# GDMCF/GDMCF

Hardware: AMD Instinct MI355X
Metric: training users/sec (higher is better)
Workload: dtype f32; 1 GPU; yelp-shape synthetic rows, batch=400/GPU, dims=[1000], T=5, noise_scale=0.01, linear-var, mean_type=x0, reweight, AdamW lr=1e-5 (BASELINE configs[1]); n_items=34395, global_batch=400, parallelism=dp1, batch_rows=device CSR rows (CsrBatch)

## Files before the change

### gdmcf_amd/_lib.py

```python
import ctypes
import os
import re
from ctypes import c_char_p, c_double, c_float, c_int, c_int64, c_size_t, c_uint64, c_void_p

_HERE = os.path.dirname(os.path.abspath(__file__))
LIB_PATH = os.path.join(_HERE, "csrc", "libgdmcf_hip.so")
HEADER_PATH = os.path.normpath(os.path.join(_HERE, "..", "include", "gdmcf_hip.h"))

P = c_void_p
_CTYPES = {"int": c_int, "int64_t": c_int64, "uint64_t": c_uint64, "size_t": c_size_t, "float": c_float, "double": c_double}


def _uncomment(text):
    return re.sub(r"/\*.*?\*/", " ", text, flags=re.S)


def _code(text):
    return re.sub(r'^[ \t]*(#.*|extern\s+"C"\s*\{|\})[ \t]*$', "", _uncomment(text), flags=re.M)


def _ctype(ctype, where):
    words = re.sub(r"\bconst\b", " ", ctype).replace("*", " * ").split()
    if "*" in words:
        return c_char_p if words == ["char", "*"] else c_void_p
    if " ".join(words) not in _CTYPES:
        raise ImportError(f"gdmcf_hip.h: no ctypes type for '{' '.join(ctype.split())}' in the declaration of {where}")
    return _CTYPES[" ".join(words)]


def _declarator(decl, where):
    m = re.fullmatch(r"\s*(.*[\s*])(\w+)\s*", decl, flags=re.S)
    if not m:
        raise ImportError(f"gdmcf_hip.h: cannot read '{decl.strip()}' in the declaration of {where}")
    return m.groups()


def parse_functions(text):
    code = _code(text)
    out = {}
    for ret, name, params in re.findall(r"([\w\s*]+?)\b(gdmcf_\w+)\s*\(([^()]*)\)\s*;", code):
        params = [] if params.strip() in ("", "void") else params.split(",")
        out[name] = (_ctype(ret, name), [_ctype(_declarator(p, name)[0], name) for p in params])
    mentioned = re.findall(r"(gdmcf_\w+)\s*\(", code)
    if len(mentioned) != len(out):
        raise ImportError(f"gdmcf_hip.h: {len(mentioned)} gdmcf_*( but {len(out)} declarations read; unreadable: "
                          f"{sorted(set(mentioned) - set(out)) or 'none, a name is repeated'}")
    return out


def parse_constants(text):
    text = _uncomment(text)
    out = {n: int(v) for n, v in re.findall(r"^\s*#\s*define\s+(GDMCF_\w+)\s+\(?\s*(-?\d+)\s*\)?\s*$", text, flags=re.M)}
    for body in re.findall(r"\benum\s*\{([^}]*)\}", text):
        for member in filter(str.strip, body.split(",")):
            m = re.fullmatch(r"\s*(\w+)\s*=\s*(-?\d+)\s*", member)
            if not m:
                raise ImportError(f"gdmcf_hip.h: enum member '{member.strip()}' is not `NAME = integer`")
            out[m.group(1)] = int(m.group(2))
    return out


def parse_structs(text):
    out = {}
    for name, body in re.findall(r"\btypedef\s+struct\s+(\w+)\s*\{([^}]*)\}\s*\1\s*;", _code(text)):
        out[name] = []
        for line in filter(str.strip, body.split(";")):
            first, *more = line.split(",")
            ctype, member = _declarator(first, "struct " + name)
            if more and "*" in line:
                raise ImportError(f"gdmcf_hip.h: struct {name}: '{line.strip()}' must declare one pointer member per line")
            out[name] += [(m.strip(), _ctype(ctype, "struct " + name)) for m in [member] + more]
    return out


try:
    with open(HEADER_PATH) as _f:
        _HEADER = _f.read()
except OSError as e:
    raise ImportError(f"{HEADER_PATH} is missing: gdmcf_amd._lib derives its ctypes binding from the C header, which sits "
                      "beside the package in the source tree.") from e
_SIGNATURES = parse_functions(_HEADER)
EXPORTED_SYMBOLS = tuple(_SIGNATURES)
CONSTANTS = parse_constants(_HEADER)
GDMCF_OK, E_SHAPE, E_ARG, E_UNSUPPORTED, E_HIP, E_WORKSPACE, N_TABLES = (
    CONSTANTS["GDMCF_" + n] for n in ("OK", "E_SHAPE", "E_ARG", "E_UNSUPPORTED", "E_HIP", "E_WORKSPACE", "N_TABLES"))
TABLE_NAMES = (
    "betas", "alphas_cumprod", "alphas_cumprod_prev", "alphas_cumprod_next", "sqrt_alphas_cumprod",
    "sqrt_one_minus_alphas_cumprod", "log_one_minus_alphas_cumprod", "sqrt_recip_alphas_cumprod",
    "sqrt_recipm1_alphas_cumprod", "posterior_variance", "posterior_log_variance_clipped",
    "posterior_mean_coef1", "posterior_mean_coef2",
)


class GdDwAdamw(ctypes.Structure):
    _fields_ = parse_structs(_HEADER)["GdDwAdamw"]


class GdKnTail(ctypes.Structure):
    _fields_ = parse_structs(_HEADER)["GdKnTail"]


_lib = None


def load():
    global _lib
    if _lib is not None:
        return _lib
    if not os.path.exists(LIB_PATH):
        raise ImportError(
            f"{LIB_PATH} is missing: build it with `python -m gdmcf_amd.build` (hipcc, gfx950). "
            "gdmcf_amd has no CPU / PyTorch fallback.")
    lib = ctypes.CDLL(LIB_PATH)
    for name, (res, args) in _SIGNATURES.items():
        fn = getattr(lib, name)
        fn.restype = res
        fn.argtypes = args
    if lib.gdmcf_version() != 1:
        raise ImportError("libgdmcf_hip.so ABI version mismatch; rebuild with `python -m gdmcf_amd.build --force`")
    _lib = lib
    return lib


_EXC = {E_SHAPE: AssertionError, E_ARG: ValueError, E_UNSUPPORTED: NotImplementedError, E_HIP: RuntimeError,
        E_WORKSPACE: RuntimeError}


def check(rc):
    if rc != GDMCF_OK:
        msg = load().gdmcf_last_error().decode(errors="replace")
        raise _EXC.get(rc, RuntimeError)(msg or f"gdmcf error {rc}")


def ptr(t):
    return None if t is None else t.data_ptr()


def require_gpu(t, what):
    if not t.is_cuda:
        raise RuntimeError(f"gdmcf_amd: {what} must live on the MI355X (got device '{t.device}'); "
                           "the HIP path has no CPU fallback")


def shadow_info(data_ptr):
    p16 = ctypes.c_void_p()
    rows, cols, ld = ctypes.c_int64(), ctypes.c_int64(), ctypes.c_int64()
    if not load().gdmcf_bf16_shadow_info(data_ptr, ctypes.byref(p16), ctypes.byref(rows), ctypes.byref(cols), ctypes.byref(ld)):
        return None
    return int(p16.value), int(rows.value), int(cols.value), int(ld.value)


def stream_ptr():
    import torch
    return torch.cuda.current_stream().cuda_stream


def philox_randn(shape, device, seed, offset, stream_id=4, out=None):
    import torch
    rows, cols = int(shape[0]), int(shape[1])
    if out is None:
        out = torch.empty(rows, cols, dtype=torch.float32, device=device)
    require_gpu(out, "philox_randn output")
    check(load().gdmcf_randn_f32(out.data_ptr(), out.stride(0), rows, cols, int(stream_id), int(seed) & (2 ** 64 - 1),
                                 int(offset) & (2 ** 64 - 1), stream_ptr()))
    return out


def schedule_tables(kind, noise_scale, noise_min, noise_max, steps, beta_fixed=True):
    import numpy as np
    out = np.zeros((N_TABLES, steps), dtype=np.float64)
    rc = load().gdmcf_schedule_build(kind, float(noise_scale), float(noise_min), float(noise_max), int(steps),
                                     int(bool(beta_fixed)), out.ctypes.data_as(c_void_p))
    check(rc)
    return out


class Bf16Shadow:

    def __init__(self, t, sync=True):
        import weakref

        import torch
        require_gpu(t, "bf16 shadow source")
        if t.dim() != 2 or t.dtype != torch.float32 or t.stride(1) != 1:
            raise RuntimeError("gdmcf_amd: a bf16 shadow needs a 2-D float32 tensor with unit column stride")
        self.rows, self.cols = t.shape
        self.ptr = t.data_ptr()
        self.ld = t.stride(0)
        self.buf = torch.zeros((self.rows + 63) // 64 * 64, (self.cols + 63) // 64 * 64, dtype=torch.bfloat16,
                               device=t.device)
        self._lib = load()
        self._fin = weakref.finalize(self, self._lib.gdmcf_bf16_shadow_clear, self.ptr)
        self.register()
        if sync:
            self.sync()

    def register(self):
        check(self._lib.gdmcf_bf16_shadow_set(self.ptr, self.buf.data_ptr(), self.rows, self.cols, self.buf.stride(0)))

    def unregister(self):
        self._lib.gdmcf_bf16_shadow_clear(self.ptr)

    def sync(self):
        check(self._lib.gdmcf_bf16_shadow_sync(self.ptr, self.ld, stream_ptr()))

    def close(self):
        self._fin()
```

### gdmcf_amd/csrc/gemm_dr_kn.hip

```cpp
#include <stdlib.h>

#include "gemm_dr.h"
#include "tail_job.h"

namespace {

#ifndef GD_KN_EVERY
#define GD_KN_EVERY 4
#endif
template <int NL>
__global__ __launch_bounds__(256, 1) void dr_kn_kernel(const DrArgs d, const GdTailJob job) {
    constexpr int TMB = 5;
    const GdGemm& g = d.g;
    const int lane = threadIdx.x & 63;
    const int wave = __builtin_amdgcn_readfirstlane(threadIdx.x >> 6);
    const int r = lane & 15, q = lane >> 4;
    const int nblk = gridDim.x, per = nblk >> 3;
    const int slot = (nblk & 7) == 0 ? ((int)(blockIdx.x & 7) * per + (int)(blockIdx.x >> 3)) : (int)blockIdx.x;
    const int wl = slot * 4 + wave;
    const int n_waves = nblk * 4;
    const int ntiles = d.tiles_m * d.tiles_n;
    const int CPS = d.ksp;
    const int total_chunks = (g.K + 15) >> 4;
    const int ntasks = ntiles * g.splits;
    if (job.on && slot == (ntasks + 3) >> 2) {
        extern __shared__ __attribute__((aligned(16))) unsigned char kn_lds[];
        gd_tail_job_run(job, kn_lds);
        return;
    }
    const __amdgpu_buffer_rsrc_t srdA = __builtin_amdgcn_make_buffer_rsrc(const_cast<float*>(g.A), 0, (int)(((int64_t)(g.M - 1) * g.lda + g.K) * 4), 0x00020000);
    const __amdgpu_buffer_rsrc_t srdB = __builtin_amdgcn_make_buffer_rsrc(const_cast<float*>(g.B), 0, (int)(((int64_t)(g.K - 1) * g.ldb + g.N) * 4), 0x00020000);
    const uint32_t ldb16 = (uint32_t)g.ldb * 64u;
    for (int task = wl; task < ntasks; task += n_waves) {
        const int split = task / ntiles, tile = task - split * ntiles;
        const int tm = tile % d.tiles_m, tn = tile / d.tiles_m;
        const int m0 = tm * (16 * TMB), n0 = tn * (64 * NL);
        const int c_lo = split * CPS;
        uint32_t offA[TMB], offB[4][NL];
#pragma unroll
        for (int a = 0; a < TMB; ++a) offA[a] = (uint32_t)(((int64_t)min(m0 + 16 * a + r, g.M - 1) * g.lda + 4 * q) * 4);
#pragma unroll
        for (int s = 0; s < 4; ++s)
#pragma unroll
            for (int l = 0; l < NL; ++l) {
                const int n = n0 + 64 * l + 4 * r;
                offB[s][l] = n < g.N ? (uint32_t)(((int64_t)(4 * q + s) * g.ldb + n) * 4) : 0x80000000u;
            }
        f32x4 acc[TMB][NL][4];
#pragma unroll
        for (int a = 0; a < TMB; ++a)
#pragma unroll
            for (int l = 0; l < NL; ++l)
#pragma unroll
                for (int e = 0; e < 4; ++e) acc[a][l][e] = f32x4{0.f, 0.f, 0.f, 0.f};
        f32x4 xa[2][TMB], xb[2][4][NL];
        {
            const uint32_t ka = (uint32_t)c_lo * 64u, kb = (uint32_t)c_lo * ldb16;
#pragma unroll
            for (int a = 0; a < TMB; ++a) xa[0][a] = __builtin_bit_cast(f32x4, __builtin_amdgcn_raw_buffer_load_b128(srdA, offA[a], ka, 0));
#pragma unroll
            for (int s = 0; s < 4; ++s)
#pragma unroll
                for (int l = 0; l < NL; ++l)
                    xb[0][s][l] = __builtin_bit_cast(f32x4, __builtin_amdgcn_raw_buffer_load_b128(srdB, offB[s][l], kb, 0));
        }
#define GD_KN_CHUNK(PAR, c)                                                                                            \
        {                                                                                                              \
            const bool more = (c) + 1 < c_lo + CPS && (c) + 1 < total_chunks;                                          \
            const uint32_t ka = more ? (uint32_t)((c) + 1) * 64u : 0x80000000u;                                        \
            const uint32_t kb = more ? (uint32_t)((c) + 1) * ldb16 : 0x80000000u;                                      \
            if ((c) * 16 + 15 >= g.K) {  \
                _Pragma("unroll") for (int e = 0; e < 4; ++e) {                                                        \
                    const bool keep = (c) * 16 + 4 * q + e < g.K;                                                      \
                    _Pragma("unroll") for (int a = 0; a < TMB; ++a) xa[PAR][a][e] = keep ? xa[PAR][a][e] : 0.f;        \
                }                                                                                                      \
            }                                                                                                          \
                    \
            _Pragma("unroll") for (int a = 0; a < TMB; ++a) asm volatile("" : "+v"(xa[PAR][a]));                       \
            _Pragma("unroll") for (int s = 0; s < 4; ++s)                                                              \
                _Pragma("unroll") for (int l = 0; l < NL; ++l) asm volatile("" : "+v"(xb[PAR][s][l]));                 \
            __builtin_amdgcn_sched_barrier(0);                                                                         \
            _Pragma("unroll") for (int s = 0; s < 4; ++s) {                                                            \
                _Pragma("unroll") for (int n = 0; n < TMB * NL * 4; ++n) {                                             \
                    const int a = n / (NL * 4), l = (n / 4) % NL, e = n % 4;                                           \
                    acc[a][l][e] = __builtin_amdgcn_mfma_f32_16x16x4f32(xa[PAR][a][s], xb[PAR][s][l][e], acc[a][l][e], 0, 0, 0); \
                    const int idx = s * (TMB * NL * 4) + n;                                                            \
                    if (idx % GD_KN_EVERY == 2 && idx / GD_KN_EVERY < TMB + 4 * NL) {                                  \
                        const int ld = idx / GD_KN_EVERY;                                                              \
                        __builtin_amdgcn_sched_barrier(0);                                                             \
                        if (ld < TMB)                                                                                  \
                            xa[(PAR) ^ 1][ld] = __builtin_bit_cast(f32x4, __builtin_amdgcn_raw_buffer_load_b128(srdA, offA[ld], ka, 0)); \
                        else                                                                                           \
                            xb[(PAR) ^ 1][(ld - TMB) / NL][(ld - TMB) % NL] = __builtin_bit_cast(                      \
                                f32x4, __builtin_amdgcn_raw_buffer_load_b128(srdB, offB[(ld - TMB) / NL][(ld - TMB) % NL], kb, 0)); \
                        __builtin_amdgcn_sched_barrier(0);                                                             \
                    }                                                                                                  \
                }                                                                                                      \
                __builtin_amdgcn_sched_barrier(0);                                                                     \
            }                                                                                                          \
        }
        for (int c = c_lo; c < c_lo + CPS && c < total_chunks; c += 2) {
            GD_KN_CHUNK(0, c);
            GD_KN_CHUNK(1, c + 1);
        }
#undef GD_KN_CHUNK
        float* __restrict__ slab = g.C + (int64_t)split * g.slab_stride;
#pragma unroll
        for (int a = 0; a < TMB; ++a)
#pragma unroll
            for (int t = 0; t < 4; ++t) {
                const int m = m0 + 16 * a + 4 * q + t;
                if (m >= g.M) continue;
#pragma unroll
                for (int l = 0; l < NL; ++l) {
                    const int n = n0 + 64 * l + 4 * r;
                    const f32x4 v = {acc[a][l][0][t], acc[a][l][1][t], acc[a][l][2][t], acc[a][l][3][t]};
                    if (n + 3 < g.ldc) {
                        *reinterpret_cast<f32x4*>(slab + (int64_t)m * g.ldc + n) = v;
                    } else {
                        for (int e = 0; e < 4; ++e)
                            if (n + e < g.N) slab[(int64_t)m * g.ldc + n + e] = v[e];
                    }
                }
            }
    }
}

}

int gd_dr_kn_splits(int M, int N, int K) {
    if (!dr_routes().kn || M < 16 || N < 64 || K < 4096) return 0;
    const long tiles = (long)gd_cdiv(M, 80) * gd_cdiv(N, 128);
    if ((long)gd_cdiv(M, 80) * 80 * 100 > (long)M * 112) return 0;
    if ((long)gd_cdiv(N, 128) * 128 * 100 > (long)N * 112) return 0;
    const long slots = 4L * dr_cu_count();
    if (tiles > slots) return 0;
    int splits = (int)(slots / tiles);
    const int total_chunks = gd_cdiv(K, 16);
    if (splits > total_chunks / 8) splits = total_chunks / 8;
    if (splits < 2 || splits > 64) return splits > 64 ? 64 : 0;
    return splits;
}

static bool kn_idle_workgroup(int ntasks, int n_cu) { return gd_cdiv(ntasks, 4) < n_cu; }

#ifndef GD_KN_TAIL_DEFAULT
#define GD_KN_TAIL_DEFAULT 1
#endif

static int kn_launch(GdGemm& g, const GdTailJob* job, hipStream_t s) {
    if (!dr_routes().kn) return GD_DR_NOT_TAKEN;
    const int splits = gd_dr_kn_splits(g.M, g.N, g.K);
    const size_t need = (size_t)splits * g.M * g.ldc * sizeof(float);
    const bool ok = splits > 0 && g.ldc >= g.N && (g.ldc & 3) == 0 && g.ws_cap >= need && g.slab_stride >= (int64_t)g.M * g.ldc &&
                (int64_t)g.M * g.lda * 4 < ((int64_t)1 << 31) && (int64_t)g.K * g.ldb * 4 < ((int64_t)1 << 31) && g.lda >= g.K && g.ldb >= g.N &&
                (reinterpret_cast<uintptr_t>(g.B) & 15) == 0 && (g.ldb & 3) == 0 && (reinterpret_cast<uintptr_t>(g.C) & 15) == 0;
    if (!ok) return GD_DR_NOT_TAKEN;
    DrArgs d = {};
    const int n_cu = dr_cu_count();
    const int total_chunks = gd_cdiv(g.K, 16);
    const int cps = (gd_cdiv(total_chunks, splits) + 1) & ~1;
    const int real_splits = gd_cdiv(total_chunks, cps);
    d.tiles_m = gd_cdiv(g.M, 80);
    d.tiles_n = gd_cdiv(g.N, 128);
    d.ksp = cps;
    GdTailJob none = {};
    size_t lds = 0;
    if (job) {
        const char* env = getenv("GDMCF_KN_TAIL");
        const bool tail_on = env ? atoi(env) != 0 : GD_KN_TAIL_DEFAULT != 0;
        lds = lt_lds_bytes(job->T, job->H, job->B);
        if (!tail_on || !job->on || !kn_idle_workgroup(d.tiles_m * d.tiles_n * real_splits, n_cu) || lds > GD_LT_LDS_MAX)
            return GD_DR_NOT_TAKEN;
        static bool attr_set = false;
        if (!gd_allow_big_lds(dr_kn_kernel<2>, lds, &attr_set, "gemm_dr_kn")) return GDMCF_E_HIP;
    }
    g.splits = real_splits;
    g.kchunk = cps * 16;
    g.tiles_m = d.tiles_m;
    g.tiles_n = d.tiles_n;
    d.g = g;
    {
        GdProfScope prof(g.prof_tag, 2.0 * g.M * g.N * g.K, s);
        hipLaunchKernelGGL((dr_kn_kernel<2>), dim3(n_cu), dim3(256), lds, s, d, job ? *job : none);
    }
    t_gd_last_gemm = 5;
    return gd_launch_status("gemm_dr_kn");
}

int gd_dr_kn_launch(GdGemm& g, hipStream_t s) { return kn_launch(g, nullptr, s); }
int gd_dr_kn_launch_tail(GdGemm& g, const GdTailJob& job, hipStream_t s) { return kn_launch(g, &job, s); }

int gdmcf_debug_kn_tail_rides(int M, int N, int K) {
    const int splits = gd_dr_kn_splits(M, N, K);
    if (splits <= 0) return 0;
    const int total_chunks = gd_cdiv(K, 16);
    const int cps = (gd_cdiv(total_chunks, splits) + 1) & ~1;
    return kn_idle_workgroup(gd_cdiv(M, 80) * gd_cdiv(N, 128) * gd_cdiv(total_chunks, cps), dr_cu_count()) ? 1 : 0;
}
```

### gdmcf_amd/csrc/linear.hip

```cpp
#include <stdlib.h>

#include "common.h"
#include "tail_job.h"

int gd_splitk_reduce(const float* slabs, int64_t slab_stride, int splits, int64_t ld_slab, int M, int N, int mode,
                     const float* bias, const float* rowscale, const float* aact, int64_t ldact, int act, float* out,
                     int64_t ldo, hipStream_t s);
int gd_colsum(const float* dZ, int64_t ld, const float* rs, int M, int N, float* db, hipStream_t s);
int gd_rowpart_reduce(const float* rowpart, int ld, int M, int nt, float* rowsum, hipStream_t s);

namespace {

static const int TARGET_WGS = getenv("GDMCF_TARGET_WGS") ? atoi(getenv("GDMCF_TARGET_WGS")) : 760;

thread_local int t_gemm_prec = GDMCF_GEMM_F32;
thread_local int t_loss_parts = 0;

int pick_class(int M, int N, bool fused, int prec) {
    if (prec == GDMCF_GEMM_BF16 && M > 128) {
        const long pad = (long)gd_cdiv(M, 208) * 208;
        const long tiles = (pad / 208) * gd_cdiv(N, 256);
        const long rounds = (tiles + 255) / 256;
        if (pad * 10 <= (long)M * 11 && pad / 208 <= 2 && (!fused || tiles * 100 >= rounds * 256 * 85)) return 3;
    }
    if (prec == GDMCF_GEMM_F32X3 && M > 128 && N >= 128) {
        const long pad = (long)gd_cdiv(M, 208) * 208;
        if (pad * 10 <= (long)M * 11) return 4;
    }
    return gd_pick_shape_class(M, N);
}

int pick_class_dw(int M, int N, int prec, bool fused_adamw = false) {
    static const int forced = getenv("GDMCF_BF16_DW_CLASS") ? atoi(getenv("GDMCF_BF16_DW_CLASS")) : -1;
    if (prec == GDMCF_GEMM_BF16 && forced >= 0) return forced;
    if (prec == GDMCF_GEMM_BF16 && fused_adamw && M >= 160 && N >= 256) return 0;
    if (prec == GDMCF_GEMM_BF16 && M >= 416 && N >= 512) {
        const long tiles = (long)gd_cdiv(M, 208) * gd_cdiv(N, 256);
        const long rounds = (tiles + 255) / 256;
        if (tiles * 100 >= rounds * 256 * 85) return 3;
    }
    return gd_pick_shape_class(M, N);
}

void attach_result_shadow(GdGemm& g) {
    GdShadow c;
    if (g.bf16 == 1 && gd_shadow_lookup(g.C, &c) && c.rows == g.M && c.cols >= g.N) {
        g.C16 = c.p16;
        g.ldc16 = c.ld16;
    }
}

void attach_shadows(GdGemm& g, int layA, int layB) {
    if (g.bf16 != 1) return;
    GdShadow a, b;
    if (!gd_shadow_lookup(g.A, &a) || !gd_shadow_lookup(g.B, &b)) return;
    const bool okA = layA == GD_LAY_KC ? (a.rows == g.M && a.cols == g.K) : (a.rows == g.K && a.cols == g.M);
    const bool okB = layB == GD_LAY_KC ? (b.rows == g.N && b.cols == g.K) : (b.rows == g.K && b.cols == g.N);
    if (!okA || !okB) return;
    g.A16 = a.p16; g.lda16 = a.ld16;
    g.B16 = b.p16; g.ldb16 = b.ld16;
}

int pick_splits(int M, int N, int K, int cls, int prec) {
    const int bk = prec == GDMCF_GEMM_BF16 ? 64 : 32;
    const int tiles = gd_cdiv(M, gd_gemm_tile_m(cls)) * gd_cdiv(N, gd_gemm_tile_n(cls));
    int s = (cls >= 3 ? 256 : TARGET_WGS) / tiles;
    const int max_by_k = K / (8 * bk);
    if (s > max_by_k) s = max_by_k;
    if (s < 1) s = 1;
    if (s > 64) s = 64;
    return s;
}

inline int64_t round4(int64_t x) { return (x + 3) & ~(int64_t)3; }

float* bias_col_request(int a_scale_col, int64_t lda, const float* rowscale, int K, float* db) {
    static const int on = getenv("GDMCF_BIAS_COL") ? atoi(getenv("GDMCF_BIAS_COL")) : 1;
    if (!on || !a_scale_col || db == nullptr || t_gemm_prec != GDMCF_GEMM_F32 || lda <= K) return nullptr;
    return db;
}

int dw_adamw_setup(const GdDwAdamw& e, GdGemm& g, int& cls) {
    GD_CHECK_SHAPE(e.M > 0 && e.N > 0 && e.K > 0 && e.lddz >= e.N && e.lda >= e.K && e.ldw >= e.K, "linear_bwd_weight_adamw: bad shape");
    GD_CHECK_ARG(e.W && e.exp_avg && e.exp_avg_sq && e.step >= 1, "linear_bwd_weight_adamw: optimizer state missing");
    const int M = e.M, N = e.N, K = e.K;
    cls = pick_class_dw(N, K, t_gemm_prec, true);
    g = GdGemm{};
    g.bf16 = t_gemm_prec;
    g.A = e.dZ; g.lda = e.lddz; g.B = e.A; g.ldb = e.lda; g.M = N; g.N = K; g.K = M; g.splits = 1;
    g.m_fastest = gd_cdiv(N, gd_gemm_tile_m(cls)) <= gd_cdiv(K, gd_gemm_tile_n(cls));
    g.C = e.W; g.ldc = e.ldw; g.aux = e.exp_avg; g.aux2 = e.exp_avg_sq; g.prof_tag = 5;
    g.adam = gd_adam_hyper(e.lr, e.beta1, e.beta2, e.eps, e.weight_decay, e.step, e.grad_scale);
    g.adam_dev = t_gd_step_state ? &t_gd_step_state->hyper : nullptr;
    attach_result_shadow(g);
    attach_shadows(g, GD_LAY_MC, GD_LAY_MC);
    g.out2 = bias_col_request(e.a_scale_col, e.lda, e.rowscale, K, e.db);
    return GDMCF_OK;
}

int dw_adamw_finish(const GdDwAdamw& e, bool asked, const GdGemm& g, hipStream_t s) {
    if (asked && g.out2 == nullptr) return GDMCF_OK;
    if (e.db) return gd_colsum(e.dZ, e.lddz, e.rowscale, e.M, e.N, e.db, s);
    return GDMCF_OK;
}

}

extern "C" {

int gdmcf_gemm_precision(int mode) {
    const int prev = t_gemm_prec;
    if (mode == GDMCF_GEMM_F32 || mode == GDMCF_GEMM_BF16 || mode == GDMCF_GEMM_F32X3) t_gemm_prec = mode;
    return prev;
}

size_t gdmcf_linear_ws_bytes(int M, int N, int K) {
    if (M <= 0 || N <= 0 || K <= 0) return 0;
    size_t need = 0;
    for (int prec = GDMCF_GEMM_F32; prec <= GDMCF_GEMM_F32X3; ++prec) {
        const int cf = pick_class(M, N, false, prec), cb = pick_class(M, K, false, prec);
        size_t f = (size_t)pick_splits(M, N, K, cf, prec) * M * round4(N);
        if (prec == GDMCF_GEMM_F32) {
            const size_t fk = (size_t)gd_dr_kn_splits(M, N, K) * M * round4(N);
            f = f > fk ? f : fk;
            const size_t ff = (size_t)gd_dr_fat_slab_plan(M, N, K, nullptr, nullptr) * M * round4(N);
            f = f > ff ? f : ff;
        }
        size_t b = (size_t)pick_splits(M, K, N, cb, prec) * M * round4(K);
        if (prec == GDMCF_GEMM_F32) {
            const size_t bk = (size_t)gd_dr_kn_splits(M, K, N) * M * round4(K);
            b = b > bk ? b : bk;
        }
        need = need > f ? need : f;
        need = need > b ? need : b;
    }
    return need * sizeof(float) + 256;
}

int gdmcf_debug_fat_slab_plan(int M, int N, int K, int* nb, int* splits, int* cps) {
    int nb_ = 0, cps_ = 0;
    const int sp = (t_gemm_prec == GDMCF_GEMM_F32 && M > 0 && N > 0 && K > 0) ? gd_dr_fat_slab_plan(M, N, K, &nb_, &cps_) : 0;
    if (nb) *nb = nb_;
    if (splits) *splits = sp;
    if (cps) *cps = cps_;
    return sp > 0;
}

int gdmcf_loss_tiles(int N) { return gd_cdiv(N, 16); }

int gdmcf_linear_fwd_f32(const float* A, int64_t lda, const float* W, int64_t ldw, const float* bias, int act, int M,
                         int N, int K, float* C, int64_t ldc, void* ws, size_t ws_bytes, void* stream) {
    GD_CHECK_SHAPE(M > 0 && N > 0 && K > 0 && lda >= K && ldw >= K && ldc >= N, "linear_fwd: bad shape");
    GD_CHECK_ARG(act == 0 || act == 1, "linear_fwd: bad activation");
    hipStream_t s = (hipStream_t)stream;
    const int cls = pick_class(M, N, false, t_gemm_prec);
    const int splits = pick_splits(M, N, K, cls, t_gemm_prec);
    GdGemm g = {};
    g.bf16 = t_gemm_prec;
    g.A = A; g.lda = lda; g.B = W; g.ldb = ldw; g.M = M; g.N = N; g.K = K;
    g.m_fastest = gd_cdiv(M, gd_gemm_tile_m(cls)) <= gd_cdiv(N, gd_gemm_tile_n(cls));
    g.bias = bias; g.act = act; g.prof_tag = 1;
    if (splits == 1) {
        g.splits = 1; g.C = C; g.ldc = ldc;
        attach_result_shadow(g);
        attach_shadows(g, GD_LAY_KC, GD_LAY_KC);
        return gd_gemm_launch(GD_LAY_KC, GD_LAY_KC, GD_EPI_BIAS_ACT, cls, g, s);
    }
    const int64_t lds_ = round4(N);
    const size_t need = (size_t)splits * M * lds_ * sizeof(float);
    if (ws == nullptr || ws_bytes < need) {
        gdmcf_set_error("linear_fwd: workspace %zu < %zu bytes", ws_bytes, need);
        return GDMCF_E_WORKSPACE;
    }
    g.splits = splits; g.C = (float*)ws; g.ldc = lds_; g.slab_stride = (int64_t)M * lds_;
    g.ws_cap = ws_bytes;
    attach_shadows(g, GD_LAY_KC, GD_LAY_KC);
    int rc = gd_gemm_launch(GD_LAY_KC, GD_LAY_KC, GD_EPI_SLAB, cls, g, s);
    if (rc) return rc;
    const int real_splits = gd_cdiv(K, g.kchunk);
    return gd_splitk_reduce((const float*)ws, g.slab_stride, real_splits, lds_, M, N, 0, bias, nullptr, nullptr, 0,
                            act, C, ldc, s);
}

int gdmcf_linear_fwd_wt_f32(const float* A, int64_t lda, const float* Wt, int64_t ldwt, const float* bias, int act, int M, int N,
                            int K, float* C, int64_t ldc, void* ws, size_t ws_bytes, void* stream) {
    GD_CHECK_SHAPE(M > 0 && N > 0 && K > 0 && lda >= K && ldwt >= N && ldc >= N, "linear_fwd_wt: bad shape");
    GD_CHECK_ARG(act == 0 || act == 1, "linear_fwd_wt: bad activation");
    if (t_gemm_prec != GDMCF_GEMM_F32) {
        gdmcf_set_error("linear_fwd_wt: float32 GEMM mode only (the bf16 / f32x3 modes keep the weight in its own orientation)");
        return GDMCF_E_UNSUPPORTED;
    }
    hipStream_t s = (hipStream_t)stream;
    const int cls = pick_class(M, N, false, t_gemm_prec);
    const int splits = pick_splits(M, N, K, cls, t_gemm_prec);
    const int64_t lds_ = round4(N);
    const size_t need = (size_t)splits * M * lds_ * sizeof(float);
    if (ws == nullptr || ws_bytes < need) {
        gdmcf_set_error("linear_fwd_wt: workspace %zu < %zu bytes", ws_bytes, need);
        return GDMCF_E_WORKSPACE;
    }
    GdGemm g = {};
    g.A = A; g.lda = lda; g.B = Wt; g.ldb = ldwt; g.M = M; g.N = N; g.K = K;
    g.m_fastest = gd_cdiv(M, gd_gemm_tile_m(cls)) <= gd_cdiv(N, gd_gemm_tile_n(cls));
    g.splits = splits; g.C = (float*)ws; g.ldc = lds_; g.slab_stride = (int64_t)M * lds_; g.prof_tag = 1;
    g.ws_cap = ws_bytes;
    int rc = gd_gemm_launch(GD_LAY_KC, GD_LAY_MC, GD_EPI_SLAB, cls, g, s);
    if (rc) return rc;
    const int real_splits = gd_cdiv(K, g.kchunk);
    return gd_splitk_reduce((const float*)ws, g.slab_stride, real_splits, lds_, M, N, 0, bias, nullptr, nullptr, 0, act, C, ldc, s);
}

int gdmcf_linear_loss_fwd_f32(const float* A, int64_t lda, const float* W, int64_t ldw, const float* bias,
                              const float* target, int64_t ldt, const float* alpha, int M, int N, int K, float* out,
                              int64_t ldo, float* diff, int64_t ldd, float* rowpart, float* rowsum, void* stream) {
    GD_CHECK_SHAPE(M > 0 && N > 0 && K > 0 && lda >= K && ldw >= K && ldt >= N && ldd >= N, "linear_loss_fwd: bad shape");
    GD_CHECK_SHAPE(out == nullptr || ldo >= N, "linear_loss_fwd: ldo < N");
    hipStream_t s = (hipStream_t)stream;
    const int cls = pick_class(M, N, true, t_gemm_prec);
    GdGemm g = {};
    g.bf16 = t_gemm_prec;
    g.A = A; g.lda = lda; g.B = W; g.ldb = ldw; g.M = M; g.N = N; g.K = K; g.splits = 1;
    g.m_fastest = gd_cdiv(M, gd_gemm_tile_m(cls)) <= gd_cdiv(N, gd_gemm_tile_n(cls));
    g.bias = bias; g.aux = target; g.ldaux = ldt; g.r0 = alpha; g.out2 = out; g.ldout2 = ldo;
    g.prof_tag = 2;
    g.C = diff; g.ldc = ldd; g.rowpart = rowpart; g.ld_rowpart = gdmcf_loss_tiles(N);
    attach_result_shadow(g);
    attach_shadows(g, GD_LAY_KC, GD_LAY_KC);
    int rc = gd_gemm_launch(GD_LAY_KC, GD_LAY_KC, GD_EPI_LOSS, cls, g, s);
    if (rc) return rc;
    t_loss_parts = g.tiles_n;
    if (rowsum == nullptr) return GDMCF_OK;
    return gd_rowpart_reduce(rowpart, g.ld_rowpart, M, g.tiles_n, rowsum, s);
}

int gdmcf_linear_loss_fwd_bits_f32(const float* A, int64_t lda, const float* W, int64_t ldw, const float* bias,
                                   const uint32_t* target_bits, int64_t ldbits, const float* alpha, int M, int N, int K,
                                   float* out, int64_t ldo, float* diff, int64_t ldd, float* rowpart, float* rowsum,
                                   void* stream) {
    GD_CHECK_SHAPE(M > 0 && N > 0 && K > 0 && lda >= K && ldw >= K && ldd >= N, "linear_loss_fwd_bits: bad shape");
    GD_CHECK_SHAPE(out == nullptr || ldo >= N, "linear_loss_fwd_bits: ldo < N");
    GD_CHECK_ARG(target_bits && ldbits >= (N + 31) / 32, "linear_loss_fwd_bits: target bitmap missing / ldbits < ceil(N/32)");
    hipStream_t s = (hipStream_t)stream;
    const int cls = pick_class(M, N, true, t_gemm_prec);
    GdGemm g = {};
    g.bf16 = t_gemm_prec;
    g.A = A; g.lda = lda; g.B = W; g.ldb = ldw; g.M = M; g.N = N; g.K = K; g.splits = 1;
    g.m_fastest = gd_cdiv(M, gd_gemm_tile_m(cls)) <= gd_cdiv(N, gd_gemm_tile_n(cls));
    g.bias = bias; g.aux = nullptr; g.ldaux = 0; g.aux_bits = target_bits; g.ldbits = ldbits; g.r0 = alpha; g.out2 = out;
    g.ldout2 = ldo; g.prof_tag = 2;
    g.C = diff; g.ldc = ldd; g.rowpart = rowpart; g.ld_rowpart = gdmcf_loss_tiles(N);
    attach_result_shadow(g);
    attach_shadows(g, GD_LAY_KC, GD_LAY_KC);
    int rc = gd_gemm_launch(GD_LAY_KC, GD_LAY_KC, GD_EPI_LOSS, cls, g, s);
    if (rc) return rc;
    t_loss_parts = g.tiles_n;
    if (rowsum == nullptr) return GDMCF_OK;
    return gd_rowpart_reduce(rowpart, g.ld_rowpart, M, g.tiles_n, rowsum, s);
}

int gdmcf_linear_posterior_fwd_f32(const float* A, int64_t lda, const float* W, int64_t ldw, const float* bias,
                                   const float* x_t, int64_t ldxt, const float* c1, const float* c2, const float* r1,
                                   const float* r2, const float* sigma, const float* z, int64_t ldz, int M, int N,
                                   int K, float* x_next, int64_t ldxn, float* pred_out, int64_t ldp, void* stream) {
    GD_CHECK_SHAPE(M > 0 && N > 0 && K > 0 && lda >= K && ldw >= K && ldxt >= N && ldxn >= N, "linear_posterior_fwd: bad shape");
    GD_CHECK_ARG(c1 && c2, "linear_posterior_fwd: c1/c2 missing");
    GD_CHECK_ARG((r1 == nullptr) == (r2 == nullptr), "linear_posterior_fwd: r1/r2 must both be set or both NULL");
    GD_CHECK_ARG(z == nullptr || (sigma != nullptr && ldz >= N), "linear_posterior_fwd: sigma missing");
    hipStream_t s = (hipStream_t)stream;
    const int cls = pick_class(M, N, true, t_gemm_prec);
    GdGemm g = {};
    g.bf16 = t_gemm_prec;
    g.A = A; g.lda = lda; g.B = W; g.ldb = ldw; g.M = M; g.N = N; g.K = K; g.splits = 1;
    g.m_fastest = gd_cdiv(M, gd_gemm_tile_m(cls)) <= gd_cdiv(N, gd_gemm_tile_n(cls));
    g.bias = bias; g.aux = x_t; g.ldaux = ldxt; g.aux2 = z; g.ldaux2 = ldz;
    g.r0 = c1; g.r1 = c2; g.r2 = r1; g.r3 = r2; g.r4 = sigma;
    g.out2 = pred_out; g.ldout2 = ldp; g.C = x_next; g.ldc = ldxn; g.prof_tag = 3;
    attach_result_shadow(g);
    attach_shadows(g, GD_LAY_KC, GD_LAY_KC);
    return gd_gemm_launch(GD_LAY_KC, GD_LAY_KC, GD_EPI_POST, cls, g, s);
}

int gdmcf_linear_bwd_input_f32(const float* dZ, int64_t lddz, const float* W, int64_t ldw, const float* rowscale,
                               const float* Aact, int64_t ldact, int act, int M, int N, int K, float* dA,
                               int64_t ldda, void* ws, size_t ws_bytes, void* stream) {
    GD_CHECK_SHAPE(M > 0 && N > 0 && K > 0 && lddz >= N && ldw >= K && ldda >= K, "linear_bwd_input: bad shape");
    GD_CHECK_ARG(act == 0 || (act == 1 && Aact && ldact >= K), "linear_bwd_input: activation output missing");
    hipStream_t s = (hipStream_t)stream;
    const int cls = pick_class(M, K, false, t_gemm_prec);
    const int splits = pick_splits(M, K, N, cls, t_gemm_prec);
    const int64_t lds_ = round4(K);
    const size_t need = (size_t)splits * M * lds_ * sizeof(float);
    if (ws == nullptr || ws_bytes < need) {
        gdmcf_set_error("linear_bwd_input: workspace %zu < %zu bytes", ws_bytes, need);
        return GDMCF_E_WORKSPACE;
    }
    GdGemm g = {};
    g.bf16 = t_gemm_prec;
    g.A = dZ; g.lda = lddz; g.B = W; g.ldb = ldw; g.M = M; g.N = K; g.K = N;
    g.m_fastest = gd_cdiv(M, gd_gemm_tile_m(cls)) <= gd_cdiv(K, gd_gemm_tile_n(cls));
    g.splits = splits; g.C = (float*)ws; g.ldc = lds_; g.slab_stride = (int64_t)M * lds_; g.prof_tag = 4;
    g.ws_cap = ws_bytes;
    attach_shadows(g, GD_LAY_KC, GD_LAY_MC);
    int rc = gd_gemm_launch(GD_LAY_KC, GD_LAY_MC, GD_EPI_SLAB, cls, g, s);
    if (rc) return rc;
    const int real_splits = gd_cdiv(N, g.kchunk);
    return gd_splitk_reduce((const float*)ws, g.slab_stride, real_splits, lds_, M, K, 1, nullptr, rowscale, Aact,
                            ldact, act, dA, ldda, s);
}

int gdmcf_loss_parts_last(void) { return t_loss_parts; }

int gdmcf_kn_tail_run(const GdKnTail* tail, int M, void* stream) {
    GD_CHECK_ARG(tail != nullptr, "kn_tail_run: tail missing");
    const GdKnTail& t = *tail;
    GD_CHECK_SHAPE(M > 0 && t.nt > 0 && t.ld_rowpart >= t.nt, "kn_tail_run: bad shape");
    GD_CHECK_ARG(t.rowpart && t.rowsum, "kn_tail_run: null pointer");
    int rc = gd_rowpart_reduce(t.rowpart, t.ld_rowpart, M, t.nt, t.rowsum, (hipStream_t)stream);
    if (rc) return rc;
    rc = gdmcf_row_loss_finish_mean_f64(t.rowsum, t.rowdiv, t.alpha, t.ts, t.weight_t, t.pt, M, t.T, t.H, t.Lt_history, t.Lt_count,
                                        t.update_history, t.loss_unscaled, t.loss, t.gradcoef, t.loss_mean, t.rowscale_mean, stream);
    if (rc) return rc;
    return gdmcf_rowscale_f32(t.A, t.lda, t.rowscale, M, t.Ka, t.out, t.ldo, stream);
}

int gdmcf_linear_bwd_input_tail_f32(const float* dZ, int64_t lddz, const float* W, int64_t ldw, const float* rowscale,
                                    const float* Aact, int64_t ldact, int act, int M, int N, int K, float* dA, int64_t ldda,
                                    void* ws, size_t ws_bytes, const GdKnTail* tail, void* stream) {
    GD_CHECK_SHAPE(M > 0 && N > 0 && K > 0 && lddz >= N && ldw >= K && ldda >= K, "linear_bwd_input_tail: bad shape");
    GD_CHECK_ARG(act == 0 || (act == 1 && Aact && ldact >= K), "linear_bwd_input_tail: activation output missing");
    GD_CHECK_ARG(tail != nullptr, "linear_bwd_input_tail: tail missing");
    const GdKnTail& t = *tail;
    GD_CHECK_SHAPE(t.nt > 0 && t.ld_rowpart >= t.nt && t.T > 0 && t.H > 0 && t.Ka > 0 && t.lda >= t.Ka && t.ldo >= t.Ka,
                   "linear_bwd_input_tail: bad tail shape");
    GD_CHECK_ARG(t.rowpart && t.rowsum && t.rowdiv && t.ts && t.weight_t && t.pt && t.loss_unscaled && t.loss && t.A && t.rowscale && t.out,
                 "linear_bwd_input_tail: null pointer");
    GD_CHECK_ARG(!t.update_history || (t.Lt_history && t.Lt_count), "linear_bwd_input_tail: update_history without the history");
    GD_CHECK_ARG(!t.rowscale_mean || t.gradcoef, "linear_bwd_input_tail: rowscale_mean needs gradcoef");
    GD_CHECK_ARG(lt_lds_bytes(t.T, t.H, M) <= GD_LT_LDS_MAX, "linear_bwd_input_tail: T*H and B too large for the LDS-resident FIFO update (150 KiB)");
    hipStream_t s = (hipStream_t)stream;
    const int64_t lds_ = round4(K);
    if (t_gemm_prec == GDMCF_GEMM_F32 && ws != nullptr) {
        GdGemm g = {};
        g.A = dZ; g.lda = lddz; g.B = W; g.ldb = ldw; g.M = M; g.N = K; g.K = N;
        g.C = (float*)ws; g.ldc = lds_; g.slab_stride = (int64_t)M * lds_; g.prof_tag = 4;
        g.ws_cap = ws_bytes;
        GdShadow sh;
        const bool has16 = gd_shadow_lookup(t.out, &sh) && sh.rows == M && sh.cols == t.Ka;
        GdTailJob j = {};
        j.on = 1; j.B = M;
        j.rowpart = t.rowpart; j.ld_rowpart = t.ld_rowpart; j.nt = t.nt; j.rowsum = t.rowsum;
        j.rowdiv = t.rowdiv; j.alpha = t.alpha; j.gradcoef = t.gradcoef; j.ts = t.ts; j.weight_t = t.weight_t; j.pt = t.pt;
        j.T = t.T; j.H = t.H; j.update = t.update_history; j.hist = t.Lt_history; j.cnt = t.Lt_count; j.lu = t.loss_unscaled;
        j.loss = t.loss; j.loss_mean = t.loss_mean; j.rowscale_mean = t.rowscale_mean; j.inv_b = 1.0f / (float)M;
        j.K = t.Ka; j.A = t.A; j.lda = t.lda; j.rs = t.rowscale; j.out = t.out; j.ldo = t.ldo;
        j.out16 = has16 ? (unsigned short*)sh.p16 : nullptr; j.ldo16 = has16 ? sh.ld16 : 0; j.bias_col = t.ldo > t.Ka;
        const int rc = gd_dr_kn_launch_tail(g, j, s);
        if (rc != GD_DR_NOT_TAKEN) {
            if (rc) return rc;
            return gd_splitk_reduce((const float*)ws, g.slab_stride, gd_cdiv(N, g.kchunk), lds_, M, K, 1, nullptr, rowscale, Aact, ldact,
                                    act, dA, ldda, s);
        }
    }
    const int rc = gdmcf_kn_tail_run(tail, M, stream);
    if (rc) return rc;
    return gdmcf_linear_bwd_input_f32(dZ, lddz, W, ldw, rowscale, Aact, ldact, act, M, N, K, dA, ldda, ws, ws_bytes, stream);
}

int gdmcf_linear_bwd_weight_f32(const float* dZ, int64_t lddz, const float* A, int64_t lda, const float* rowscale,
                                int a_scale_col, int M, int N, int K, float* dW, int64_t lddw, float* db, int accumulate,
                                void* stream) {
    GD_CHECK_SHAPE(M > 0 && N > 0 && K > 0 && lddz >= N && lda >= K && lddw >= K, "linear_bwd_weight: bad shape");
    hipStream_t s = (hipStream_t)stream;
    const int cls = pick_class_dw(N, K, t_gemm_prec);
    GdGemm g = {};
    g.bf16 = t_gemm_prec;
    g.A = dZ; g.lda = lddz; g.B = A; g.ldb = lda; g.M = N; g.N = K; g.K = M; g.splits = 1;
    g.m_fastest = gd_cdiv(N, gd_gemm_tile_m(cls)) <= gd_cdiv(K, gd_gemm_tile_n(cls));
    g.C = dW; g.ldc = lddw; g.accumulate = accumulate; g.prof_tag = 5;
    attach_shadows(g, GD_LAY_MC, GD_LAY_MC);
    g.out2 = bias_col_request(a_scale_col, lda, rowscale, K, db);
    const bool asked = g.out2 != nullptr;
    int rc = gd_gemm_launch(GD_LAY_MC, GD_LAY_MC, GD_EPI_STORE, cls, g, s);
    if (rc) return rc;
    if (asked && g.out2 == nullptr) return GDMCF_OK;
    if (db) return gd_colsum(dZ, lddz, rowscale, M, N, db, s);
    return GDMCF_OK;
}

int gdmcf_linear_bwd_weight_adamw_f32(const float* dZ, int64_t lddz, const float* A, int64_t lda, const float* rowscale,
                                      int a_scale_col, int M, int N, int K, float* W, int64_t ldw, float* exp_avg, float* exp_avg_sq,
                                      float* db, float lr, float beta1, float beta2, float eps, float weight_decay,
                                      int step, float grad_scale, void* stream) {
    const GdDwAdamw e = {dZ, lddz, A, lda, rowscale, a_scale_col, M, N, K, W, ldw, exp_avg, exp_avg_sq, db,
                         lr, beta1, beta2, eps, weight_decay, step, grad_scale};
    GdGemm g;
    int cls;
    int rc = dw_adamw_setup(e, g, cls);
    if (rc) return rc;
    const bool asked = g.out2 != nullptr;
    rc = gd_gemm_launch(GD_LAY_MC, GD_LAY_MC, GD_EPI_ADAMW, cls, g, (hipStream_t)stream);
    if (rc) return rc;
    return dw_adamw_finish(e, asked, g, (hipStream_t)stream);
}

int gdmcf_linear_bwd_weight_adamw_multi_f32(const GdDwAdamw* list, int n, void* stream) {
    GD_CHECK_ARG(n >= 0 && (n == 0 || list), "linear_bwd_weight_adamw_multi: bad list");
    hipStream_t s = (hipStream_t)stream;
    constexpr int MAXN = 4;
    for (int i0 = 0; i0 < n; i0 += MAXN) {
        const int k = n - i0 < MAXN ? n - i0 : MAXN;
        GdGemm g[MAXN];
        bool asked[MAXN];
        int cls;
        for (int j = 0; j < k; ++j) {
            const int rc = dw_adamw_setup(list[i0 + j], g[j], cls);
            if (rc) return rc;
            asked[j] = g[j].out2 != nullptr;
        }
        int rc = gd_gemm_dr_adamw_multi(g, k, s);
        if (rc == GD_DR_NOT_TAKEN) {
            for (int j = 0; j < k; ++j) {
                const GdDwAdamw& e = list[i0 + j];
                rc = gdmcf_linear_bwd_weight_adamw_f32(e.dZ, e.lddz, e.A, e.lda, e.rowscale, e.a_scale_col, e.M, e.N, e.K, e.W,
                                                       e.ldw, e.exp_avg, e.exp_avg_sq, e.db, e.lr, e.beta1, e.beta2, e.eps,
                                                       e.weight_decay, e.step, e.grad_scale, stream);
                if (rc) return rc;
            }
            continue;
        }
        if (rc) return rc;
        for (int j = 0; j < k; ++j) {
            rc = dw_adamw_finish(list[i0 + j], asked[j], g[j], s);
            if (rc) return rc;
        }
    }
    return GDMCF_OK;
}

}
```

### gdmcf_amd/csrc/reduce.hip

```cpp
#include "tail_job.h"

namespace {

__global__ __launch_bounds__(256) void splitk_reduce_kernel(const float* __restrict__ slabs, int64_t slab_stride,
                                                            int splits, int64_t ld_slab, int M, int N, int mode,
                                                            const float* __restrict__ bias,
                                                            const float* __restrict__ rowscale,
                                                            const float* __restrict__ aact, int64_t ldact, int act,
                                                            float* __restrict__ out, int64_t ldo,
                                                            unsigned short* __restrict__ out16, int64_t ldo16, int vec) {
    const int m = blockIdx.y;
    const int n0 = (blockIdx.x * 256 + threadIdx.x) * 4;
    if (n0 >= N) return;
    float sv[4] = {0.f, 0.f, 0.f, 0.f};
    const float* p = slabs + (int64_t)m * ld_slab + n0;
    if (vec && n0 + 3 < N) {
        for (int k0 = 0; k0 < splits; k0 += 8) {
            f32x4 t[8];
#pragma unroll
            for (int u = 0; u < 8; ++u)
                t[u] = (k0 + u < splits) ? *reinterpret_cast<const f32x4*>(p + (int64_t)(k0 + u) * slab_stride)
                                         : f32x4{0.f, 0.f, 0.f, 0.f};
#pragma unroll
            for (int u = 0; u < 8; ++u)
                if (k0 + u < splits) { sv[0] += t[u].x; sv[1] += t[u].y; sv[2] += t[u].z; sv[3] += t[u].w; }
        }
    } else {
        for (int k = 0; k < splits; ++k)
            for (int j = 0; j < 4; ++j)
                if (n0 + j < N) sv[j] += p[(int64_t)k * slab_stride + j];
    }
    const float rs = (mode != 0 && rowscale) ? rowscale[m] : 1.f;
#pragma unroll
    for (int j = 0; j < 4; ++j) {
        const int n = n0 + j;
        if (n >= N) break;
        float s = sv[j];
        if (mode == 0) {
            if (bias) s += bias[n];
            if (act == 1) s = tanhf(s);
        } else {
            if (rowscale) s *= rs;
            if (act == 1) {
                const float h = aact[(int64_t)m * ldact + n];
                s *= (1.f - h * h);
            }
        }
        out[(int64_t)m * ldo + n] = s;
        if (out16) out16[(int64_t)m * ldo16 + n] = gd_bf16_bits(s);
    }
}

__global__ __launch_bounds__(256) void rowscale_kernel(const float* __restrict__ A, int64_t lda,
                                                       const float* __restrict__ rs, int M, int K,
                                                       float* __restrict__ out, int64_t ldo,
                                                       unsigned short* __restrict__ out16, int64_t ldo16, int bias_col) {
    gd_rowscale_rows<1>(A, lda, rs, M, K, out, ldo, out16, ldo16, bias_col, blockIdx.x, gridDim.x, blockIdx.y, gridDim.y);
}

__global__ __launch_bounds__(256) void colsum_kernel(const float* __restrict__ dZ, int64_t ld,
                                                     const float* __restrict__ rs, int M, int N,
                                                     float* __restrict__ db) {
    __shared__ float part[4][64];
    const int lane = threadIdx.x & 63, wave = threadIdx.x >> 6;
    const int n = blockIdx.x * 64 + lane;
    const int nc = min(n, N - 1);
    float s = 0.f;
    int m = wave;
    for (; m + 28 < M; m += 32) {
        float v[8];
#pragma unroll
        for (int j = 0; j < 8; ++j) v[j] = dZ[(int64_t)(m + 4 * j) * ld + nc] * (rs ? rs[m + 4 * j] : 1.f);
#pragma unroll
        for (int j = 0; j < 8; ++j) s += v[j];
    }
    for (; m < M; m += 4) s += dZ[(int64_t)m * ld + nc] * (rs ? rs[m] : 1.f);
    part[wave][lane] = s;
    __syncthreads();
    if (wave == 0 && n < N) db[n] = ((part[0][lane] + part[1][lane]) + part[2][lane]) + part[3][lane];
}

__global__ __launch_bounds__(256) void rowpart_reduce_kernel(const float* __restrict__ rowpart, int ld, int M, int nt,
                                                             float* __restrict__ rowsum) {
    gd_rowpart_reduce_rows<1>(rowpart, ld, M, nt, rowsum, blockIdx.x, gridDim.x);
}

typedef __bf16 gd_bf16x2 __attribute__((ext_vector_type(2)));
__device__ __forceinline__ unsigned gd_pack_bf16(float lo, float hi) {
    gd_bf16x2 v;
    v[0] = (__bf16)lo;
    v[1] = (__bf16)hi;
    return __builtin_bit_cast(unsigned, v);
}
typedef unsigned int gd_u32x4 __attribute__((ext_vector_type(4)));

__global__ __launch_bounds__(256) void cast_bf16_kernel(const float* __restrict__ src, int64_t ld, unsigned short* __restrict__ dst,
                                                        int64_t ld16, int64_t rows, int64_t cols) {
    const int64_t groups = (cols + 7) / 8;
    const int64_t total = rows * groups;
    for (int64_t u = (int64_t)blockIdx.x * blockDim.x + threadIdx.x; u < total; u += (int64_t)gridDim.x * blockDim.x) {
        const int64_t r = u / groups, c = (u - r * groups) * 8;
        const float* p = src + r * ld + c;
        float e[8];
#pragma unroll
        for (int i = 0; i < 8; ++i) e[i] = (c + i < cols) ? p[i] : 0.f;
        gd_u32x4 w;
        w.x = gd_pack_bf16(e[0], e[1]);
        w.y = gd_pack_bf16(e[2], e[3]);
        w.z = gd_pack_bf16(e[4], e[5]);
        w.w = gd_pack_bf16(e[6], e[7]);
        *reinterpret_cast<gd_u32x4*>(dst + r * ld16 + c) = w;
    }
}
}

extern "C" {

int gdmcf_rowscale_f32(const float* A, int64_t lda, const float* rowscale, int M, int K, float* out, int64_t ldo,
                       void* stream) {
    GD_CHECK_SHAPE(M > 0 && K > 0 && lda >= K && ldo >= K, "rowscale: bad shape");
    GdShadow sh;
    const bool has16 = gd_shadow_lookup(out, &sh) && sh.rows == M && sh.cols == K;
    const int bias_col = ldo > K;
    hipLaunchKernelGGL(rowscale_kernel, dim3(gd_cdiv(K, 1024), M), dim3(256), 0, (hipStream_t)stream, A, lda,
                       rowscale, M, K, out, ldo, has16 ? (unsigned short*)sh.p16 : nullptr, has16 ? sh.ld16 : 0, bias_col);
    return gd_launch_status("rowscale");
}

}

int gd_splitk_reduce(const float* slabs, int64_t slab_stride, int splits, int64_t ld_slab, int M, int N, int mode,
                     const float* bias, const float* rowscale, const float* aact, int64_t ldact, int act, float* out,
                     int64_t ldo, hipStream_t s) {
    GdShadow sh;
    const bool has16 = gd_shadow_lookup(out, &sh) && sh.rows == M && sh.cols == N;
    const int vec = (ld_slab % 4 == 0) && (slab_stride % 4 == 0) && gd_aligned16(slabs);
    hipLaunchKernelGGL(splitk_reduce_kernel, dim3(gd_cdiv(N, 1024), M), dim3(256), 0, s, slabs, slab_stride,
                       splits, ld_slab, M, N, mode, bias, rowscale, aact, ldact, act, out, ldo,
                       has16 ? (unsigned short*)sh.p16 : nullptr, has16 ? sh.ld16 : 0, vec);
    return gd_launch_status("splitk_reduce");
}

int gd_colsum(const float* dZ, int64_t ld, const float* rs, int M, int N, float* db, hipStream_t s) {
    hipLaunchKernelGGL(colsum_kernel, dim3(gd_cdiv(N, 64)), dim3(256), 0, s, dZ, ld, rs, M, N, db);
    return gd_launch_status("colsum");
}

int gd_rowpart_reduce(const float* rowpart, int ld, int M, int nt, float* rowsum, hipStream_t s) {
    hipLaunchKernelGGL(rowpart_reduce_kernel, dim3(gd_cdiv(M, 4)), dim3(256), 0, s, rowpart, ld, M, nt, rowsum);
    return gd_launch_status("rowpart_reduce");
}

int gd_cast_bf16(const float* src, int64_t ld, void* dst, int64_t ld16, int64_t rows, int64_t cols, hipStream_t s) {
    const int64_t total = rows * ((cols + 7) / 8);
    const int64_t blocks = (total + 255) / 256;
    hipLaunchKernelGGL(cast_bf16_kernel, dim3((unsigned)(blocks < 16384 ? blocks : 16384)), dim3(256), 0, s, src, ld,
                       (unsigned short*)dst, ld16, rows, cols);
    return gd_launch_status("cast_bf16");
}
```

### gdmcf_amd/csrc/rows.hip

```cpp
#include "common.h"

namespace {

__device__ __forceinline__ float block_sum_256(float v, float* red) {
#pragma unroll
    for (int o = 32; o > 0; o >>= 1) v += __shfl_down(v, o, 64);
    __syncthreads();
    if ((threadIdx.x & 63) == 0) red[threadIdx.x >> 6] = v;
    __syncthreads();
    return red[0] + red[1] + red[2] + red[3];
}

__global__ __launch_bounds__(256) void row_norms_kernel(const float* __restrict__ X, int64_t ld, int cols,
                                                       float* __restrict__ norm, float* __restrict__ inv_norm) {
    __shared__ float red[4];
    const float* x = X + (int64_t)blockIdx.x * ld;
    float ss = 0.f;
    const int c4 = cols & ~3;
    for (int c = threadIdx.x * 4; c < c4; c += 1024) {
        const f32x4 t = *reinterpret_cast<const f32x4_u4*>(x + c);
        ss += t.x * t.x + t.y * t.y + t.z * t.z + t.w * t.w;
    }
    if (threadIdx.x < cols - c4) ss += x[c4 + threadIdx.x] * x[c4 + threadIdx.x];
    const float n = sqrtf(block_sum_256(ss, red));
    if (threadIdx.x == 0) {
        if (norm) norm[blockIdx.x] = n;
        if (inv_norm) inv_norm[blockIdx.x] = 1.f / n;
    }
}

template <bool ADAM_>
__global__ __launch_bounds__(256) void normalize_rows_bwd_kernel(const float* __restrict__ dY, int64_t lddy,
                                                                const float* __restrict__ Y, int64_t ldy,
                                                                const float* __restrict__ inv_norm, int cols,
                                                                float* __restrict__ dX, int64_t lddx,
                                                                float* __restrict__ exp_avg, float* __restrict__ exp_avg_sq,
                                                                GdAdamHyper h, const GdStepState* step_state) {
    __shared__ float red[4];
    if (ADAM_ && step_state) h = step_state->hyper;
    const float* dy = dY + (int64_t)blockIdx.x * lddy;
    const float* y = Y + (int64_t)blockIdx.x * ldy;
    float* dx = dX + (int64_t)blockIdx.x * lddx;
    float* mr = ADAM_ ? exp_avg + (int64_t)blockIdx.x * lddx : nullptr;
    float* vr = ADAM_ ? exp_avg_sq + (int64_t)blockIdx.x * lddx : nullptr;
    const float rn = inv_norm[blockIdx.x];
    if (cols <= 4096 && (cols & 3) == 0) {
        f32x4 a[4], b[4];
        float dot = 0.f;
#pragma unroll
        for (int k = 0; k < 4; ++k) {
            const int c = (threadIdx.x + 256 * k) * 4;
            a[k] = b[k] = f32x4{0.f, 0.f, 0.f, 0.f};
            if (c < cols) {
                a[k] = *reinterpret_cast<const f32x4_u4*>(dy + c);
                b[k] = *reinterpret_cast<const f32x4_u4*>(y + c);
            }
            dot += a[k].x * b[k].x + a[k].y * b[k].y + a[k].z * b[k].z + a[k].w * b[k].w;
        }
        dot = block_sum_256(dot, red);
#pragma unroll
        for (int k = 0; k < 4; ++k) {
            const int c = (threadIdx.x + 256 * k) * 4;
            if (c >= cols) continue;
            const f32x4 g = (a[k] - b[k] * dot) * rn;
            if (!ADAM_) {
                *reinterpret_cast<f32x4_u4*>(dx + c) = g;
                continue;
            }
            f32x4 pp = *reinterpret_cast<const f32x4_u4*>(dx + c);
            f32x4 mm = *reinterpret_cast<const f32x4_u4*>(mr + c);
            f32x4 vv = *reinterpret_cast<const f32x4_u4*>(vr + c);
#pragma unroll
            for (int j = 0; j < 4; ++j) {
                float pj = pp[j], mj = mm[j], vj = vv[j];
                gd_adam_elem(pj, g[j], mj, vj, h);
                pp[j] = pj;
                mm[j] = mj;
                vv[j] = vj;
            }
            *reinterpret_cast<f32x4_u4*>(dx + c) = pp;
            *reinterpret_cast<f32x4_u4*>(mr + c) = mm;
            *reinterpret_cast<f32x4_u4*>(vr + c) = vv;
        }
        return;
    }
    float dot = 0.f;
    for (int c = threadIdx.x; c < cols; c += 256) dot += dy[c] * y[c];
    dot = block_sum_256(dot, red);
    for (int c = threadIdx.x; c < cols; c += 256) {
        const float g = (dy[c] - y[c] * dot) * rn;
        if (ADAM_)
            gd_adam_elem(dx[c], g, mr[c], vr[c], h);
        else
            dx[c] = g;
    }
}

__global__ __launch_bounds__(256) void tanh_bwd_kernel(const float* __restrict__ dA, int64_t ldd, const float* __restrict__ A,
                                                      int64_t lda, const float* __restrict__ extra, int64_t lde,
                                                      const float* __restrict__ scale, int N, float* __restrict__ out,
                                                      int64_t ldo) {
    const int m = blockIdx.y, n = blockIdx.x * 256 + threadIdx.x;
    if (n >= N) return;
    float g = dA[(int64_t)m * ldd + n];
    if (extra) g += scale[0] * extra[(int64_t)m * lde + n];
    const float a = A[(int64_t)m * lda + n];
    out[(int64_t)m * ldo + n] = g * (1.f - a * a);
}

__global__ __launch_bounds__(256) void gather_rows_kernel(const float* __restrict__ src, int64_t lds,
                                                         const int64_t* __restrict__ index, int cols,
                                                         float* __restrict__ dst, int64_t ldd) {
    const float* s = src + index[blockIdx.x] * lds;
    float* d = dst + (int64_t)blockIdx.x * ldd;
    for (int c = threadIdx.x; c < cols; c += 256) d[c] = s[c];
}

__global__ __launch_bounds__(256) void scatter_add_rows_kernel(const float* __restrict__ src, int64_t lds,
                                                              const int64_t* __restrict__ index, int cols,
                                                              float* __restrict__ dst, int64_t ldd) {
    const float* s = src + (int64_t)blockIdx.x * lds;
    float* d = dst + index[blockIdx.x] * ldd;
    for (int c = threadIdx.x; c < cols; c += 256) atomicAdd(d + c, s[c]);
}

constexpr int SCATTER_ADAM_ROWS = 16;

__global__ __launch_bounds__(256) void scatter_rows_adamw_kernel(const float* __restrict__ src, int64_t lds,
                                                                const int64_t* __restrict__ index, int n, int rows, int cols,
                                                                float* __restrict__ W, int64_t ldw, float* __restrict__ exp_avg,
                                                                float* __restrict__ exp_avg_sq, GdAdamHyper h,
                                                                const GdStepState* step_state) {
    __shared__ int slot[SCATTER_ADAM_ROWS];
    if (step_state) h = step_state->hyper;
    const int64_t r0 = (int64_t)blockIdx.x * SCATTER_ADAM_ROWS;
    if (threadIdx.x < SCATTER_ADAM_ROWS) slot[threadIdx.x] = -1;
    __syncthreads();
    for (int j = threadIdx.x; j < n; j += 256) {
        const int64_t r = index[j] - r0;
        if (r >= 0 && r < SCATTER_ADAM_ROWS) slot[r] = j;
    }
    __syncthreads();
    const int nr = (int)min((int64_t)SCATTER_ADAM_ROWS, rows - r0);
    const bool vec = ((cols | ldw | lds) & 3) == 0 &&
                     ((reinterpret_cast<uintptr_t>(W) | reinterpret_cast<uintptr_t>(exp_avg) |
                       reinterpret_cast<uintptr_t>(exp_avg_sq) | reinterpret_cast<uintptr_t>(src)) & 15u) == 0;
    if (vec) {
        const int c4 = cols >> 2;
        for (int it = threadIdx.x; it < nr * c4; it += 256) {
            const int rr = it / c4, c = (it - rr * c4) * 4;
            const int j = slot[rr];
            const int64_t o = (r0 + rr) * ldw + c;
            f32x4 gg = {0.f, 0.f, 0.f, 0.f};
            if (j >= 0) gg = gg + *reinterpret_cast<const f32x4*>(src + (int64_t)j * lds + c);
            f32x4 pp = __builtin_nontemporal_load(reinterpret_cast<f32x4*>(W + o));
            f32x4 mm = __builtin_nontemporal_load(reinterpret_cast<f32x4*>(exp_avg + o));
            f32x4 vv = __builtin_nontemporal_load(reinterpret_cast<f32x4*>(exp_avg_sq + o));
#pragma unroll
            for (int q = 0; q < 4; ++q) {
                float pq = pp[q], mq = mm[q], vq = vv[q];
                gd_adam_elem(pq, gg[q], mq, vq, h);
                pp[q] = pq;
                mm[q] = mq;
                vv[q] = vq;
            }
            __builtin_nontemporal_store(pp, reinterpret_cast<f32x4*>(W + o));
            __builtin_nontemporal_store(mm, reinterpret_cast<f32x4*>(exp_avg + o));
            __builtin_nontemporal_store(vv, reinterpret_cast<f32x4*>(exp_avg_sq + o));
        }
        return;
    }
    for (int it = threadIdx.x; it < nr * cols; it += 256) {
        const int rr = it / cols, c = it - rr * cols;
        const int j = slot[rr];
        const int64_t o = (r0 + rr) * ldw + c;
        float g = 0.f;
        if (j >= 0) g = g + src[(int64_t)j * lds + c];
        gd_adam_elem(W[o], g, exp_avg[o], exp_avg_sq[o], h);
    }
}

__global__ __launch_bounds__(256) void emb_gather_w_kernel(const float* __restrict__ W1, int64_t ldw, int I, int E, int N,
                                                           float* __restrict__ W1e) {
    const int idx = blockIdx.x * 256 + threadIdx.x;
    if (idx < N * E) W1e[idx] = W1[(int64_t)(idx / E) * ldw + I + (idx % E)];
}

__global__ __launch_bounds__(256) void emb_bwd_demb_kernel(const float* __restrict__ dZ1, int64_t lddz,
                                                           const float* __restrict__ W1e, int E, int N,
                                                           float* __restrict__ demb) {
    const int m = blockIdx.x;
    const int lane = threadIdx.x & 63, wave = threadIdx.x >> 6;
    for (int e = wave; e < E; e += 4) {
        float s = 0.f;
        for (int n = lane; n < N; n += 64) s += dZ1[(int64_t)m * lddz + n] * W1e[(int64_t)n * E + e];
        for (int o = 32; o > 0; o >>= 1) s += __shfl_xor(s, o);
        if (lane == 0) demb[(int64_t)m * E + e] = s;
    }
}

__global__ __launch_bounds__(64) void emb_bwd_w_kernel(const float* __restrict__ demb, const float* __restrict__ temb,
                                                       int M, int E, float* __restrict__ dWe,
                                                       float* __restrict__ dbe) {
    const int idx = blockIdx.x, lane = threadIdx.x;
    float s = 0.f;
    if (idx < E * E) {
        const int e = idx / E, f = idx % E;
        for (int m = lane; m < M; m += 64) s += demb[(int64_t)m * E + e] * temb[(int64_t)m * E + f];
    } else {
        const int e = idx - E * E;
        for (int m = lane; m < M; m += 64) s += demb[(int64_t)m * E + e];
    }
    for (int o = 32; o > 0; o >>= 1) s += __shfl_xor(s, o);
    if (lane == 0) {
        if (idx < E * E) dWe[idx] = s;
        else dbe[idx - E * E] = s;
    }
}

__global__ __launch_bounds__(256) void densify_rows_kernel(const int64_t* __restrict__ indptr,
                                                           const int32_t* __restrict__ indices,
                                                           const float* __restrict__ values,
                                                           const int64_t* __restrict__ row_ids, int I,
                                                           float* __restrict__ out, int64_t ldo) {
    const int b = blockIdx.x;
    float* row = out + (int64_t)b * ldo;
    const bool al = ((reinterpret_cast<uintptr_t>(row) & 15u) == 0);
    if (al) {
        for (int i = threadIdx.x * 4; i + 3 < I; i += 1024) *reinterpret_cast<f32x4*>(row + i) = f32x4{0.f, 0.f, 0.f, 0.f};
        for (int i = (I & ~3) + threadIdx.x; i < I; i += 256) row[i] = 0.f;
    } else {
        for (int i = threadIdx.x; i < I; i += 256) row[i] = 0.f;
    }
    __syncthreads();
    const int64_t u = row_ids ? row_ids[b] : b;
    for (int64_t j = indptr[u] + threadIdx.x; j < indptr[u + 1]; j += 256) {
        const int c = indices[j];
        if (c >= 0 && c < I) row[c] = values ? values[j] : 1.f;
    }
}

__global__ __launch_bounds__(256) void scale_kernel(const float* __restrict__ a, int64_t n, float s,
                                                    float* __restrict__ out) {
    const int64_t i = (int64_t)blockIdx.x * 256 + threadIdx.x;
    if (i < n) out[i] = a[i] * s;
}

}

extern "C" {

int gdmcf_row_norms_f32(const float* X, int64_t ld, int rows, int cols, float* norm, float* inv_norm, void* stream) {
    GD_CHECK_SHAPE(rows > 0 && cols > 0 && ld >= cols, "row_norms: bad shape");
    GD_CHECK_ARG(X && (norm || inv_norm), "row_norms: null pointer");
    hipLaunchKernelGGL(row_norms_kernel, dim3(rows), dim3(256), 0, (hipStream_t)stream, X, ld, cols, norm, inv_norm);
    return gd_launch_status("row_norms");
}

int gdmcf_normalize_rows_bwd_f32(const float* dY, int64_t lddy, const float* Y, int64_t ldy, const float* inv_norm, int rows,
                                 int cols, float* dX, int64_t lddx, void* stream) {
    GD_CHECK_SHAPE(rows > 0 && cols > 0 && lddy >= cols && ldy >= cols && lddx >= cols, "normalize_rows_bwd: bad shape");
    GD_CHECK_ARG(dY && Y && inv_norm && dX, "normalize_rows_bwd: null pointer");
    hipLaunchKernelGGL(normalize_rows_bwd_kernel<false>, dim3(rows), dim3(256), 0, (hipStream_t)stream, dY, lddy, Y, ldy,
                       inv_norm, cols, dX, lddx, nullptr, nullptr, GdAdamHyper{}, nullptr);
    return gd_launch_status("normalize_rows_bwd");
}

int gdmcf_normalize_rows_bwd_adamw_f32(const float* dY, int64_t lddy, const float* Y, int64_t ldy, const float* inv_norm,
                                       int rows, int cols, float* X, int64_t ldx, float* exp_avg, float* exp_avg_sq, float lr,
                                       float beta1, float beta2, float eps, float weight_decay, int step, float grad_scale,
                                       void* stream) {
    GD_CHECK_SHAPE(rows > 0 && cols > 0 && lddy >= cols && ldy >= cols && ldx >= cols, "normalize_rows_bwd_adamw: bad shape");
    GD_CHECK_ARG(dY && Y && inv_norm && X && exp_avg && exp_avg_sq && step >= 1, "normalize_rows_bwd_adamw: null pointer");
    const GdAdamHyper h = gd_adam_hyper(lr, beta1, beta2, eps, weight_decay, step, grad_scale);
    {
        GdProfScope prof(6, 32.0 * (double)rows * cols, (hipStream_t)stream);
        hipLaunchKernelGGL(normalize_rows_bwd_kernel<true>, dim3(rows), dim3(256), 0, (hipStream_t)stream, dY, lddy, Y, ldy,
                           inv_norm, cols, X, ldx, exp_avg, exp_avg_sq, h, t_gd_step_state);
    }
    return gd_launch_status("normalize_rows_bwd_adamw");
}

int gdmcf_tanh_bwd_f32(const float* dA, int64_t ldd, const float* A, int64_t lda, const float* extra, int64_t lde,
                       const float* scale, int M, int N, float* out, int64_t ldo, void* stream) {
    GD_CHECK_SHAPE(M > 0 && N > 0 && ldd >= N && lda >= N && ldo >= N && (!extra || lde >= N), "tanh_bwd: bad shape");
    GD_CHECK_ARG(dA && A && out && (!extra || scale), "tanh_bwd: null pointer");
    hipLaunchKernelGGL(tanh_bwd_kernel, dim3(gd_cdiv(N, 256), M), dim3(256), 0, (hipStream_t)stream, dA, ldd, A, lda, extra, lde,
                       scale, N, out, ldo);
    return gd_launch_status("tanh_bwd");
}

int gdmcf_gather_rows_f32(const float* src, int64_t lds, const int64_t* index, int n, int cols, float* dst, int64_t ldd,
                          void* stream) {
    GD_CHECK_SHAPE(n > 0 && cols > 0 && lds >= cols && ldd >= cols, "gather_rows: bad shape");
    GD_CHECK_ARG(src && index && dst, "gather_rows: null pointer");
    hipLaunchKernelGGL(gather_rows_kernel, dim3(n), dim3(256), 0, (hipStream_t)stream, src, lds, index, cols, dst, ldd);
    return gd_launch_status("gather_rows");
}

int gdmcf_scatter_add_rows_f32(const float* src, int64_t lds, const int64_t* index, int n, int cols, float* dst, int64_t ldd,
                               void* stream) {
    GD_CHECK_SHAPE(n > 0 && cols > 0 && lds >= cols && ldd >= cols, "scatter_add_rows: bad shape");
    GD_CHECK_ARG(src && index && dst, "scatter_add_rows: null pointer");
    hipLaunchKernelGGL(scatter_add_rows_kernel, dim3(n), dim3(256), 0, (hipStream_t)stream, src, lds, index, cols, dst, ldd);
    return gd_launch_status("scatter_add_rows");
}

int gdmcf_scatter_rows_adamw_f32(const float* src, int64_t lds, const int64_t* index, int n, int rows, int cols, float* W,
                                 int64_t ldw, float* exp_avg, float* exp_avg_sq, float lr, float beta1, float beta2, float eps,
                                 float weight_decay, int step, float grad_scale, void* stream) {
    GD_CHECK_SHAPE(n >= 0 && rows > 0 && cols > 0 && ldw >= cols && (n == 0 || lds >= cols), "scatter_rows_adamw: bad shape");
    GD_CHECK_ARG(W && exp_avg && exp_avg_sq && (n == 0 || (src && index)) && step >= 1, "scatter_rows_adamw: null pointer");
    const GdAdamHyper h = gd_adam_hyper(lr, beta1, beta2, eps, weight_decay, step, grad_scale);
    {
        GdProfScope prof(6, 24.0 * (double)rows * cols, (hipStream_t)stream);
        hipLaunchKernelGGL(scatter_rows_adamw_kernel, dim3(gd_cdiv(rows, SCATTER_ADAM_ROWS)), dim3(256), 0, (hipStream_t)stream,
                           src, lds, index, n, rows, cols, W, ldw, exp_avg, exp_avg_sq, h, t_gd_step_state);
    }
    return gd_launch_status("scatter_rows_adamw");
}

int gdmcf_emb_bwd_f32(const float* dZ1, int64_t lddz, const float* W1, int64_t ldw, int I, int E, const float* temb,
                      int M, int N, float* demb_ws, float* dWe, float* dbe, void* stream) {
    GD_CHECK_SHAPE(M > 0 && N > 0 && E > 0 && I >= 0 && ldw >= I + E && lddz >= N, "emb_bwd: bad shape");
    GD_CHECK_ARG(dZ1 && W1 && temb && demb_ws && dWe && dbe, "emb_bwd: null pointer");
    hipStream_t s = (hipStream_t)stream;
    float* W1e = demb_ws + (size_t)M * E;
    hipLaunchKernelGGL(emb_gather_w_kernel, dim3(gd_cdiv(N * E, 256)), dim3(256), 0, s, W1, ldw, I, E, N, W1e);
    hipLaunchKernelGGL(emb_bwd_demb_kernel, dim3(M), dim3(256), 0, s, dZ1, lddz, W1e, E, N, demb_ws);
    hipLaunchKernelGGL(emb_bwd_w_kernel, dim3(E * E + E), dim3(64), 0, s, demb_ws, temb, M, E, dWe, dbe);
    return gd_launch_status("emb_bwd");
}

int gdmcf_densify_rows_f32(const int64_t* indptr, const int32_t* indices, const float* values, const int64_t* row_ids,
                           int B, int I, float* out, int64_t ldo, void* stream) {
    GD_CHECK_SHAPE(B > 0 && I > 0 && ldo >= I, "densify_rows: bad shape");
    GD_CHECK_ARG(indptr && indices && out, "densify_rows: null pointer");
    hipLaunchKernelGGL(densify_rows_kernel, dim3(B), dim3(256), 0, (hipStream_t)stream, indptr, indices, values, row_ids,
                       I, out, ldo);
    return gd_launch_status("densify_rows");
}

int gdmcf_scale_f32(const float* acc, int64_t n, float scale, float* out, void* stream) {
    GD_CHECK_SHAPE(n > 0, "scale: empty");
    GD_CHECK_ARG(acc && out, "scale: null pointer");
    hipLaunchKernelGGL(scale_kernel, dim3((unsigned)((n + 255) / 256)), dim3(256), 0, (hipStream_t)stream, acc, n,
                       scale, out);
    return gd_launch_status("scale");
}

}
```

### gdmcf_amd/csrc/tail_job.h

```cpp
#pragma once

#include "common.h"

namespace {

template <int U>
__device__ __forceinline__ void gd_rowpart_reduce_rows(const float* __restrict__ rowpart, int ld, int M, int nt,
                                                       float* __restrict__ rowsum, int blk, int nblk) {
    const int lane = threadIdx.x & 63, step = nblk * 4;
    for (int m0 = blk * 4 + (int)(threadIdx.x >> 6); m0 < M; m0 += step * U) {
        float s[U];
#pragma unroll
        for (int u = 0; u < U; ++u) s[u] = 0.f;
        for (int j = lane; j < nt; j += 64) {
#pragma unroll
            for (int u = 0; u < U; ++u) s[u] += rowpart[(int64_t)min(m0 + u * step, M - 1) * ld + j];
        }
#pragma unroll
        for (int u = 0; u < U; ++u) {
            for (int o = 32; o > 0; o >>= 1) s[u] += __shfl_xor(s[u], o);
            if (lane == 0 && m0 + u * step < M) rowsum[m0 + u * step] = s[u];
        }
    }
}

template <int U>
__device__ __forceinline__ void gd_rowscale_rows(const float* __restrict__ A, int64_t lda, const float* __restrict__ rs, int M, int K,
                                                 float* __restrict__ out, int64_t ldo, unsigned short* __restrict__ out16,
                                                 int64_t ldo16, int bias_col, int bx, int nbx, int by, int nby) {
    for (int kb = bx; kb * 1024 < K; kb += nbx) {
        const int k = (kb * 256 + (int)threadIdx.x) * 4;
        for (int m0 = by; m0 < M; m0 += nby * U) {
            float r[U];
            f32x4 t[U];
#pragma unroll
            for (int u = 0; u < U; ++u) {
                const int m = min(m0 + u * nby, M - 1);
                r[u] = rs[m];
                const float* a = A + (int64_t)m * lda + k;
                if (k + 3 < K) {
                    t[u] = *reinterpret_cast<const f32x4_u4*>(a);
                } else {
                    for (int j = 0; j < 4; ++j) t[u][j] = k + j < K ? a[j] : 0.f;
                }
            }
#pragma unroll
            for (int u = 0; u < U; ++u) {
                const int m = m0 + u * nby;
                if (m >= M) break;
                if (bias_col && kb == 0 && threadIdx.x == 0) out[(int64_t)m * ldo + K] = r[u];
                if (k >= K) continue;
                float* o = out + (int64_t)m * ldo + k;
                const float v[4] = {t[u].x * r[u], t[u].y * r[u], t[u].z * r[u], t[u].w * r[u]};
                if (k + 3 < K) {
                    *reinterpret_cast<f32x4_u4*>(o) = f32x4{v[0], v[1], v[2], v[3]};
                } else {
                    for (int j = 0; j < 4; ++j)
                        if (k + j < K) o[j] = v[j];
                }
                if (out16)
                    for (int j = 0; j < 4; ++j)
                        if (k + j < K) out16[(int64_t)m * ldo16 + k + j] = gd_bf16_bits(v[j]);
            }
        }
    }
}

__device__ __forceinline__ void lt_history_parallel(const int64_t* __restrict__ ts, const double* __restrict__ lu, int B, int T, int H,
                                                    double* hist, int64_t* cnt, unsigned char* lds_raw) {
    double* old = reinterpret_cast<double*>(lds_raw);
    int* n_t = reinterpret_cast<int*>(old + (size_t)T * H);
    int* c0 = n_t + T;
    int* tsl = c0 + T;
    const int tid = threadIdx.x, nth = blockDim.x;
    for (int i = tid; i < T * H; i += nth) old[i] = hist[i];
    for (int t = tid; t < T; t += nth) {
        n_t[t] = 0;
        c0[t] = (int)cnt[t];
    }
    for (int b = tid; b < B; b += nth) tsl[b] = (int)ts[b];
    __syncthreads();
    for (int b = tid; b < B; b += nth) atomicAdd(&n_t[tsl[b]], 1);
    __syncthreads();
    for (int i = tid; i < T * H; i += nth) {
        const int t = i / H, j = i % H;
        const int drop = max(0, c0[t] + n_t[t] - H);
        if (j < c0[t] && j - drop >= 0) hist[(int64_t)t * H + (j - drop)] = old[i];
    }
    for (int b = tid; b < B; b += nth) {
        const int t = tsl[b];
        int rank = 0;
        for (int p = 0; p < b; ++p) rank += (tsl[p] == t);
        const int drop = max(0, c0[t] + n_t[t] - H);
        const int pos = c0[t] + rank - drop;
        if (pos >= 0) hist[(int64_t)t * H + pos] = lu[b];
    }
    for (int t = tid; t < T; t += nth) cnt[t] = (int64_t)min(H, c0[t] + n_t[t]);
}

__device__ __forceinline__ void gd_row_loss_finish_block(const float* __restrict__ rowsum, const float* __restrict__ rowdiv,
                                                         const float* __restrict__ alpha, float* __restrict__ gradcoef,
                                                         const int64_t* __restrict__ ts, const double* __restrict__ weight_t,
                                                         const double* __restrict__ pt, int B, int T, int H, double* hist,
                                                         int64_t* cnt, int update, double* __restrict__ lu, double* __restrict__ loss,
                                                         double* __restrict__ loss_mean, float* __restrict__ rowscale_mean,
                                                         float inv_b, unsigned char* fin_lds) {
    double part = 0.0;
    for (int b = threadIdx.x; b < B; b += 256) {
        const float mse = rowsum[b] / rowdiv[b];
        const double l = weight_t[ts[b]] * (double)mse;
        lu[b] = l;
        const double lb = l / pt[b];
        loss[b] = lb;
        part += lb;
        if (gradcoef) {
            const float gc = (float)(2.0 * (alpha ? (double)alpha[b] : 1.0) * weight_t[ts[b]] / (pt[b] * (double)rowdiv[b]));
            gradcoef[b] = gc;
            if (rowscale_mean) rowscale_mean[b] = gc * inv_b;
        }
    }
    if (loss_mean) {
        double* s_part = reinterpret_cast<double*>(fin_lds);
        for (int o = 32; o > 0; o >>= 1) part += __shfl_xor(part, o);
        if ((threadIdx.x & 63) == 0) s_part[threadIdx.x >> 6] = part;
        __syncthreads();
        if (threadIdx.x == 0) *loss_mean = (((s_part[0] + s_part[1]) + s_part[2]) + s_part[3]) / (double)B;
    }
    __syncthreads();
    if (update) lt_history_parallel(ts, lu, B, T, H, hist, cnt, fin_lds);
}

}

struct GdTailJob {
    int on;
    int B;
    const float* rowpart;
    int ld_rowpart, nt;
    float* rowsum;
    const float* rowdiv;
    const float* alpha;
    float* gradcoef;
    const int64_t* ts;
    const double* weight_t;
    const double* pt;
    int T, H, update;
    double* hist;
    int64_t* cnt;
    double* lu;
    double* loss;
    double* loss_mean;
    float* rowscale_mean;
    float inv_b;
    int K;
    const float* A;
    int64_t lda;
    const float* rs;
    float* out;
    int64_t ldo;
    unsigned short* out16;
    int64_t ldo16;
    int bias_col;
};

namespace {

__device__ __forceinline__ void gd_tail_job_run(const GdTailJob& j, unsigned char* lds) {
    gd_rowpart_reduce_rows<8>(j.rowpart, j.ld_rowpart, j.B, j.nt, j.rowsum, 0, 1);
    __syncthreads();
    gd_row_loss_finish_block(j.rowsum, j.rowdiv, j.alpha, j.gradcoef, j.ts, j.weight_t, j.pt, j.B, j.T, j.H, j.hist, j.cnt, j.update,
                             j.lu, j.loss, j.loss_mean, j.rowscale_mean, j.inv_b, lds);
    __syncthreads();
    gd_rowscale_rows<8>(j.A, j.lda, j.rs, j.B, j.K, j.out, j.ldo, j.out16, j.ldo16, j.bias_col, 0, 1, 0, 1);
}

inline size_t lt_lds_bytes(int T, int H, int B) { return (size_t)T * H * 8 + (size_t)T * 8 + (size_t)B * 4 + 16; }
constexpr size_t GD_LT_LDS_MAX = 150 * 1024;

template <class K>
bool gd_allow_big_lds(K* kernel, size_t lds, bool* done, const char* who) {
    if (*done || lds <= 48 * 1024) return true;
    *done = hipFuncSetAttribute(reinterpret_cast<const void*>(kernel), hipFuncAttributeMaxDynamicSharedMemorySize, 160 * 1024) == hipSuccess;
    if (!*done) gdmcf_set_error("%s: hipFuncSetAttribute failed", who);
    return *done;
}

}

int gd_dr_kn_launch_tail(GdGemm& g, const GdTailJob& job, hipStream_t s);
```

### gdmcf_amd/engine.py

```python

import ctypes
import os

import torch

from . import _lib
from . import engine_core as core
from .engine_core import EngineBase, _Bufs, _ceil64, with_precision


class DenoiserEngine(EngineBase):
    def __init__(self, model):
        super().__init__(model)
        self._wshadow = {}
        self.input_grad_first = False
        self.weight_waiters = {}
        self.static_grads = False
        self._grad_bufs = {}
        self._gemm_side = os.environ.get("GDMCF_GEMM_SIDE", "0") == "1"
        self._side2 = None
        self._side2_used = False
        self._wt_on = os.environ.get("GDMCF_FWD_WT", "1") == "1"
        self.defer_tail = False
        self._pending_tail = None

    def _grad_like(self, p):
        if not self.static_grads:
            return torch.empty_like(p)
        g = self._grad_bufs.get(id(p))
        if g is None or g.shape != p.shape or g.device != p.device:
            g = self._grad_bufs[id(p)] = torch.empty_like(p)
        return g

    def _use_weight(self, w):
        fn = self.weight_waiters.pop(id(w), None) if self.weight_waiters else None
        if fn is not None:
            fn()
            rec = self._wshadow.get(id(w))
            if rec is not None and rec[1] != w._version:
                rec[0].sync()
                rec[1] = w._version

    def flush_weight_waiters(self):
        self._flush_tail()
        while self.weight_waiters:
            self.weight_waiters.popitem()[1]()

    def _defers_tail(self, spec, layers, B):
        if not self.defer_tail or type(self) is not DenoiserEngine or self.gemm_dtype != "f32" or spec["eps_mode"]:
            return False
        if (self.grad_sink is not None and not self.input_grad_first) or len(layers) < 2:
            return False
        n, k = layers[-1][0].shape
        return bool(self.lib.gdmcf_debug_kn_tail_rides(B, k, n))

    def _flush_tail(self):
        pend, self._pending_tail = self._pending_tail, None
        if pend is not None:
            core.tail_job_run(self.lib, pend[0], pend[1], _lib.stream_ptr())

    def _shadows_on(self, bufs, layers):
        if self.gemm_dtype != "bf16":
            if bufs.shadows is not None:
                for sh in bufs.shadows:
                    sh.close()
                bufs.shadows = None
                bufs.sh_xin2 = None
            for sh, _ in self._wshadow.values():
                sh.close()
            self._wshadow = {}
            return
        if bufs.shadows is None:
            I, E = self.I, self.E
            mk = lambda t, cols: _lib.Bf16Shadow(t[:, :cols], sync=False)
            sh = [mk(bufs.xin, I + E), mk(bufs.diff, I)]
            for (w, _, _), a, d in zip(layers[:-1], bufs.acts, bufs.dzs):
                sh += [mk(a, w.shape[0]), mk(d, w.shape[0])]
            sh.append(mk(bufs.hs, layers[-1][0].shape[1]))
            bufs.shadows = sh
            bufs.sh_xin = sh[0]
        live = {id(w) for w, _, _ in layers}
        for key in [k for k in self._wshadow if k not in live]:
            self._wshadow.pop(key)[0].close()
        for w, _, _ in layers:
            rec = self._wshadow.get(id(w))
            if rec is None or rec[0].ptr != w.data_ptr():
                self._use_weight(w)
                if rec is not None:
                    rec[0].close()
                self._wshadow[id(w)] = [_lib.Bf16Shadow(w.detach()), w._version]
            elif id(w) in self.weight_waiters:
                continue
            elif rec[1] != w._version:
                rec[0].sync()
                rec[1] = w._version

    def _layers(self):
        layers = self.model.layer_list()
        self._check_params(layers)
        return layers

    def buffers(self, B, device):
        key = (B, str(device))
        b = self._bufs.get(key)
        if b is not None:
            return b
        layers = self.model.layer_list()
        f32 = dict(dtype=torch.float32, device=device)
        b = _Bufs()
        b.ldk = _ceil64(self.I + self.E)
        b.xin = torch.zeros(B, b.ldk, **f32)
        b.xin2 = None
        b.acts = [torch.zeros(B, _ceil64(w.shape[0]), **f32) for (w, _, _) in layers[:-1]]
        b.dzs = [torch.zeros(B, _ceil64(w.shape[0]), **f32) for (w, _, _) in layers[:-1]]
        b.hs = torch.zeros(B, _ceil64(layers[-1][0].shape[1]), **f32)
        b.shadows = None
        self._shared_buffers(b, B, device, layers[-1][0].shape[0], layers[0][0].shape[0], [w for w, _, _ in layers])
        self._bufs[key] = b
        return b

    def _prep(self, bufs, x, ts, ca, cb, noise, drop_mask, training, xt_out=None, xin=None):
        xin = bufs.xin if xin is None else xin
        keepalive = self._prep_input(bufs, x, self.I, xin, ts, ca, cb, noise, drop_mask, training, xt_out=xt_out)
        if xin is bufs.xin:
            bufs.xin_ones = True
        return keepalive

    def _train_input(self, bufs, spec, xt_out):
        return self._prep(bufs, spec["x_start"], spec["ts"], spec["ca"], spec["cb"], spec["noise"], spec["drop_mask"],
                          self.model.training, xt_out=xt_out)

    def _prep_csr(self, bufs, batch, ts, ca, cb, noise, drop_mask, training):
        m = self.model
        B, I = batch.shape
        if getattr(bufs, "x0bits", None) is None:
            bufs.x0bits = torch.zeros(B, (I + 31) // 32, dtype=torch.int32, device=batch.device)
        self.offset += 1
        keepalive = core.prep_input_csr(self.lib, batch, ts, ca, cb, noise, drop_mask, float(m.drop.p), training, self.seed,
                                        self.offset, m.emb_layer, self.E, bufs.xin, bufs.temb, bufs.x0bits, _lib.stream_ptr())
        bufs.xin_ones = True
        return keepalive

    def _train_input_csr(self, bufs, spec):
        return self._prep_csr(bufs, spec["csr"], spec["ts"], spec["ca"], spec["cb"], spec["noise"], spec["drop_mask"],
                              self.model.training)

    def _hidden_forward(self, bufs, layers, B, xin=None, frozen=False, csr=None):
        lib, st = self.lib, _lib.stream_ptr()
        A = bufs.xin if xin is None else xin
        for li, (w, bias, act) in enumerate(layers[:-1]):
            N, K = w.shape
            out = bufs.acts[li]
            self._use_weight(w)
            if li == 0 and csr is not None:
                self._gather_first_layer(bufs, csr, w, bias, act, A, B, out, st)
            elif frozen and self._wt_on and self.gemm_dtype == "f32" and K >= 4096 and w.numel() >= (1 << 20):
                wt = self._transposed(w)
                _lib.check(lib.gdmcf_linear_fwd_wt_f32(A.data_ptr(), A.stride(0), wt.data_ptr(), wt.stride(0), bias.data_ptr(), act, B, N, K,
                                                       out.data_ptr(), out.stride(0), bufs.ws.data_ptr(), bufs.ws_bytes, st))
            else:
                core.linear_fwd(lib, bufs, A, w, bias, act, B, N, K, out, st)
            A = out
        return A

    @with_precision
    def train_forward(self, spec):
        self._flush_tail()
        x0, ts = spec["x_start"], spec["ts"]
        csr = spec.get("csr")
        B, dev = (csr.shape[0], csr.device) if csr is not None else (x0.shape[0], x0.device)
        layers = self._layers()
        bufs = self.buffers(B, dev)
        self._shadows_on(bufs, layers)
        lib, st = self.lib, _lib.stream_ptr()
        self.version += 1
        eps_mode = spec["eps_mode"]
        xt_out = None
        if eps_mode:
            if bufs.xt is None:
                bufs.xt = torch.zeros(B, bufs.ldi, dtype=torch.float32, device=dev)
            xt_out = bufs.xt
        if csr is not None:
            keepalive = self._train_input_csr(bufs, spec)
        else:
            keepalive = self._train_input(bufs, spec, xt_out)
        x0c = keepalive[0]
        alpha = None
        if eps_mode:
            target, alpha, rowdiv = self._eps_target(bufs, spec, ts, x0c, keepalive[1])
        else:
            target = x0c
            rowdiv = bufs.rowdiv_mse
        A = self._hidden_forward(bufs, layers, B)
        w, bias, _ = layers[-1]
        N, K = w.shape
        self._use_weight(w)
        defer = self._defers_tail(spec, layers, B)
        if csr is not None:
            nt = core.loss_layer_bits(lib, bufs, A, w, bias, bufs.x0bits, None, B, N, K, st, reduce=not defer)
        else:
            nt = core.loss_layer(lib, bufs, A, w, bias, target, alpha, B, N, K, st, reduce=not defer)
        tail = None
        if defer:
            loss, self.last_loss_mean, tail = core.loss_tail_job(lib, bufs, spec, B, rowdiv, alpha, nt, A, K)
            self._pending_tail = (tail, B)
        else:
            loss, self.last_loss_mean = core.loss_tail(lib, bufs, spec, B, rowdiv, alpha, st, mean=True)
        self._saved = dict(kind="train", B=B, bufs=bufs, layers=layers, tail=tail,
                           keepalive=(keepalive, target, alpha, rowdiv, spec["pt"]))
        return loss

    @with_precision
    def train_backward(self, gloss):
        sv = self._saved
        if sv is None or sv.get("kind") != "train":
            raise RuntimeError("gdmcf_amd: train_backward without a preceding training_losses")
        bufs = sv["bufs"]
        tail = sv.get("tail")
        if tail is not None and self._pending_tail is not None and self._pending_tail[0] is tail:
            if isinstance(gloss, float) and gloss == 1.0 / sv["B"]:
                self._pending_tail = None
                return self._backward(sv, bufs.diff, bufs.rowscale_mean, tail=tail)
            self._flush_tail()
        if isinstance(gloss, float) and gloss == 1.0 / sv["B"] and getattr(bufs, "rowscale_mean", None) is not None:
            rowscale = bufs.rowscale_mean
        else:
            rowscale = self._rowscale_of(bufs, gloss)
        return self._backward(sv, bufs.diff, rowscale)

    @with_precision
    def forward_plain(self, x, timesteps, training, drop_mask=None):
        self.flush_weight_waiters()
        B, dev = x.shape[0], x.device
        layers = self._layers()
        bufs = self.buffers(B, dev)
        self._shadows_on(bufs, layers)
        lib, st = self.lib, _lib.stream_ptr()
        self.version += 1
        ts = timesteps.to(device=dev, dtype=torch.int64).contiguous()
        keepalive = self._prep(bufs, x, ts, None, None, None, drop_mask, training)
        A = self._hidden_forward(bufs, layers, B)
        w, bias, act = layers[-1]
        N, K = w.shape
        out = torch.empty(B, N, dtype=torch.float32, device=dev)
        core.linear_fwd(lib, bufs, A, w, bias, act, B, N, K, out, st)
        self._saved = dict(kind="plain", B=B, bufs=bufs, layers=layers, keepalive=(keepalive, ts))
        return out

    @with_precision
    def backward_plain(self, gout):
        sv = self._saved
        g = gout.to(torch.float32)
        if g.stride(-1) != 1:
            g = g.contiguous()
        return self._backward(sv, g, None)

    def _backward(self, sv, dz_last, rowscale, tail=None):
        lib, st = self.lib, _lib.stream_ptr()
        bufs, layers, B = sv["bufs"], sv["layers"], sv["B"]
        m = self.model
        L = len(layers)
        grads_w = [None] * L
        grads_b = [None] * L
        dWe = dbe = None
        fused = self.fused_opt if self.grad_sink is None else None
        dz, rs = dz_last, rowscale
        dw_queue = [] if (fused is not None and self.gemm_dtype == "f32" and os.environ.get("GDMCF_DW_MULTI", "1") != "0") else None

        def input_grad(li, w, A_prev):
            nonlocal dWe, dbe
            N, K = w.shape
            if li > 0:
                dprev = bufs.dzs[li - 1]
                if tail is not None and li == L - 1:
                    core.linear_bwd_input_tail(lib, bufs, dz, w, rs, A_prev, layers[li - 1][2], B, N, K, dprev, tail, st)
                else:
                    self._input_grad(bufs, B, w, N, K, dz, rs, A_prev, layers[li - 1][2], dprev, st)
                return dprev
            dWe = self._grad_like(m.emb_layer.weight)
            dbe = self._grad_like(m.emb_layer.bias)
            core.emb_bwd(lib, bufs, dz, w, self.I, self.E, B, N, dWe, dbe, st)
            return None

        def weight_grad(li, w, bias, A_prev):
            db = self._grad_like(bias)
            scol = int(rs is None and li == 0 and getattr(bufs, "xin_ones", False) and A_prev.stride(0) > w.shape[1])
            if tail is not None and li == L - 1:
                A_use, scol = bufs.hs, int(bufs.hs.stride(0) > w.shape[1])
            else:
                A_use, scol = self._row_scaled(bufs, B, w.shape[1], A_prev, rs, scol, st)
            fs = fused.fused_state(w) if fused is not None else None
            dW = self._grad_like(w) if fs is None else None
            if fs is None and self._gemm_side and self.grad_sink is None and li == L - 1 and L > 1:
                if self._side2 is None:
                    self._side2 = torch.cuda.Stream()
                self._side2.wait_stream(torch.cuda.current_stream())
                with torch.cuda.stream(self._side2):
                    self._weight_grad(bufs, B, w, dz, rs, A_use, scol, dW, db, None, _lib.stream_ptr())
                self._side2_used = True
            else:
                self._weight_grad(bufs, B, w, dz, rs, A_use, scol, dW, db, fs, st, queue=dw_queue)
            grads_w[li], grads_b[li] = dW, db
            if self.grad_sink is not None:
                self.grad_sink(w, dW)
                self.grad_sink(bias, db)
                grads_w[li] = grads_b[li] = None

        for li in range(L - 1, -1, -1):
            w, bias, _ = layers[li]
            A_prev = bufs.acts[li - 1] if li > 0 else bufs.xin
            if fused is not None or self.input_grad_first or (tail is not None and li == L - 1):
                nxt = input_grad(li, w, A_prev)
                weight_grad(li, w, bias, A_prev)
            else:
                weight_grad(li, w, bias, A_prev)
                nxt = input_grad(li, w, A_prev)
            dz, rs = nxt, None
        if dw_queue:
            arr = (_lib.GdDwAdamw * len(dw_queue))(*[e for e, _ in dw_queue])
            _lib.check(lib.gdmcf_linear_bwd_weight_adamw_multi_f32(ctypes.addressof(arr), len(dw_queue), st))
            for _, w in dw_queue:
                torch.autograd.graph.increment_version(w)
        if self._side2_used:
            torch.cuda.current_stream().wait_stream(self._side2)
            self._side2_used = False
        if self.grad_sink is not None:
            self.grad_sink(m.emb_layer.weight, dWe)
            self.grad_sink(m.emb_layer.bias, dbe)
            dWe = dbe = None
        out = [dWe, dbe]
        for li in range(L):
            out += [grads_w[li], grads_b[li]]
        return out

    @with_precision
    def p_sample_loop(self, x_start, steps, T, tabs32, eps_mode, sampling_noise, noise0=None, step_noise=None,
                      capture=None, draw_noise=None, latent=False, stop=False, eps=None):
        m, lib = self.model, self.lib
        if draw_noise is None:
            def draw_noise(like):
                self.offset += 1
                return _lib.philox_randn(like.shape, like.device, self.seed, self.offset, 7)
        self.flush_weight_waiters()
        B, dev, I = x_start.shape[0], x_start.device, self.I
        from .data_utils import CsrBatch
        csr = x_start if isinstance(x_start, CsrBatch) else None
        if csr is not None and (steps != 0 or m.norm or self.gemm_dtype != "f32" or csr.csr.values is not None):
            raise RuntimeError("gdmcf_amd: the reverse loop takes CSR rows only for steps == 0, binary rows, norm=False and "
                               "float32 products (GaussianDiffusion.p_sample densifies the rest)")
        layers = self._layers()
        bufs = self.buffers(B, dev)
        self._shadows_on(bufs, layers)
        st = _lib.stream_ptr()
        self.version += 1
        if latent:
            if (eps_mode and eps is None) or sampling_noise or capture is not None or m.norm or self.gemm_dtype != "f32":
                raise RuntimeError("gdmcf_amd: the latent reverse loop takes the x0 target without sampling noise, capture or "
                                   "F.normalize, in float32 products (GaussianDiffusion._latent_reverse_ok)")
            return self._latent_loop(bufs, layers, x_start, csr, steps, T, tabs32, noise0, stop=stop, eps=eps if eps_mode else None)
        if bufs.xin2 is None:
            bufs.xin2 = torch.zeros_like(bufs.xin)
        if self.gemm_dtype == "bf16" and getattr(bufs, "sh_xin2", None) is None:
            bufs.sh_xin2 = _lib.Bf16Shadow(bufs.xin2[:, : I + self.E], sync=False)
            bufs.shadows.append(bufs.sh_xin2)
        norm = bool(m.norm)
        keep = []
        t_vec = torch.full((B,), max(steps - 1, 0), dtype=torch.int64, device=dev)
        ca = cb = None
        if steps > 0:
            ca, cb = tabs32["sqrt_ab"], tabs32["sqrt_1mab"]
        w, bias, _ = layers[-1]
        N, K = w.shape
        out = None

        stabs = core.step_tables(tabs32, T, B, ("c1", "c2", "r1", "r2", "sigma"), bufs.tab_cache)
        if getattr(bufs, "step_ts", None) is None or bufs.step_ts.shape[0] != T:
            bufs.step_ts = torch.arange(T, dtype=torch.int64, device=dev)[:, None].expand(T, B).contiguous()
        step_ts = bufs.step_ts

        def posterior(i, n, A, xt, xn):
            c1, c2 = stabs["c1"][i], stabs["c2"][i]
            r1 = r2 = sg = z = None
            if eps_mode:
                r1, r2 = stabs["r1"][i], stabs["r2"][i]
            if sampling_noise and i != 0:
                sg = stabs["sigma"][i]
                z = step_noise[n] if step_noise is not None else draw_noise(xt[:, :I])
                z = z.contiguous()
            pred = torch.empty(B, I, dtype=torch.float32, device=dev) if capture is not None else None
            core.posterior_fwd(lib, A, w, bias, xt, c1, c2, r1, r2, sg, z, B, N, K, xn, pred, st)
            keep.append((c1, c2, r1, r2, sg, z))
            if capture is not None:
                capture.setdefault("pred_xstart", []).append(pred)
                capture.setdefault("mean", []).append(xn[:, :I].clone())

        if not norm:
            cur, nxt = bufs.xin, bufs.xin2
            if csr is not None:
                keep.append(self._prep_csr(bufs, csr, t_vec, None, None, None, None, False))
            else:
                keep.append(self._prep(bufs, x_start, t_vec, ca, cb, noise0, None, False, xin=cur))
            bufs.xin_ones = False
            for n, i in enumerate(range(T - 1, -1, -1)):
                ts = step_ts[i]
                _lib.check(lib.gdmcf_dnn_emb_cols_f32(ts.data_ptr(), m.emb_layer.weight.data_ptr(),
                                                      m.emb_layer.bias.data_ptr(), self.E, B, I, cur.data_ptr(),
                                                      cur.stride(0), bufs.temb.data_ptr(), st))
                keep.append(ts)
                A = self._hidden_forward(bufs, layers, B, xin=cur, frozen=True, csr=csr if n == 0 else None)
                out = torch.empty(B, I, dtype=torch.float32, device=dev) if i == 0 else None
                posterior(i, n, A, cur, out if out is not None else nxt)
                cur, nxt = nxt, cur
        else:
            if bufs.xt is None:
                bufs.xt = torch.zeros(B, bufs.ldi, dtype=torch.float32, device=dev)
            xt = bufs.xt
            keep.append(self._prep(bufs, x_start, t_vec, ca, cb, noise0, None, False, xt_out=xt, xin=bufs.xin2))
            for n, i in enumerate(range(T - 1, -1, -1)):
                ts = step_ts[i]
                keep.append(self._prep(bufs, xt[:, :I], ts, None, None, None, None, False, xin=bufs.xin))
                A = self._hidden_forward(bufs, layers, B, xin=bufs.xin, frozen=True)
                out = torch.empty(B, I, dtype=torch.float32, device=dev) if i == 0 else None
                xn = out if out is not None else (bufs.diff if xt is bufs.xt else bufs.xt)
                posterior(i, n, A, xt, xn)
                xt = xn
        self._saved = None
        del keep
        return out

    def _latent_begin(self, bufs, layers, T, B, tabs32):
        for wl, _, _ in layers:
            self._use_weight(wl)
        (w1, b1, _), (w, bias, _), emb = layers[0], layers[-1], self.model.emb_layer
        ops = self._latent_operands(w1, b1, w, w.shape[1], bias, T, (w1, b1, w, bias, emb.weight, emb.bias))
        ld = _ceil64(w1.shape[0])
        if getattr(bufs, "lat_p", None) is None:
            bufs.lat_p = torch.zeros(B, ld, dtype=torch.float32, device=w1.device)
            bufs.lat_h = torch.zeros_like(bufs.lat_p)
        return ops, core.step_tables(tabs32, T, B, ("c1", "c2"), bufs.tab_cache), bufs.lat_p, ld

    def _latent_run(self, bufs, layers, ops, tabs, T, B, pre, p, e, x_T, **kw):
        (_, _, act1), (w, bias, _), lib, st = layers[0], layers[-1], self.lib, _lib.stream_ptr()

        def middle(n, i, A):
            for li in range(1, len(layers) - 1):
                wl, bl, al = layers[li]
                core.linear_fwd(lib, bufs, A, wl, bl, al, B, wl.shape[0], wl.shape[1], bufs.acts[li], st)
                A = bufs.acts[li]
            return A

        return self._latent_reverse(bufs, ops, T, B, w.shape[1], act1, pre, p, (bufs.acts[0], bufs.lat_h),
                                    middle if len(layers) > 2 else None, e, tabs["c1"], tabs["c2"], w, bias, x_T, **kw)

    def _latent_loop(self, bufs, layers, x_start, csr, steps, T, tabs32, noise0, stop=False, eps=None):
        lib, st, I = self.lib, _lib.stream_ptr(), self.I
        B, dev = x_start.shape[0], x_start.device
        w1 = layers[0][0]
        h1 = w1.shape[0]
        ops, tabs, p, _ = self._latent_begin(bufs, layers, T, B, tabs32)
        t_vec = torch.full((B,), max(steps - 1, 0), dtype=torch.int64, device=dev)
        if csr is not None:
            if stop:
                keep, self.offset = None, self.offset + 1
            else:
                keep = self._prep_csr(bufs, csr, t_vec, None, None, None, None, False)
            wt = self._transposed(w1)
            core.gather_fwd(lib, None, None, csr, wt, I, None, None, 0, None, 0, B, h1, p, st)
        else:
            ca, cb = (tabs32["sqrt_ab"], tabs32["sqrt_1mab"]) if steps > 0 else (None, None)
            keep = self._prep(bufs, x_start, t_vec, ca, cb, noise0, None, False, xin=bufs.xin)
            core.linear_fwd(lib, bufs, (bufs.xin.data_ptr(), bufs.xin.stride(0)), w1, None, 0, B, h1, I, p, st)
        bufs.xin_ones = False
        x0 = self._latent_run(bufs, layers, ops, tabs, T, B, p, p, ops.e, bufs.xin, stop=stop, eps=eps)
        self._saved = None
        del keep
        return x0
```

### gdmcf_amd/engine_core.py

```python
import collections
import ctypes
import functools

import torch

from . import _lib


def _ceil64(n):
    return (int(n) + 63) // 64 * 64


class _Bufs:
    pass


_GEMM_MODES = {k: _lib.CONSTANTS["GDMCF_GEMM_" + k.upper()] for k in ("f32", "bf16", "f32x3")}


def with_precision(fn):
    @functools.wraps(fn)
    def wrapped(self, *a, **kw):
        prev = self.lib.gdmcf_gemm_precision(_GEMM_MODES[self.gemm_dtype])
        try:
            return fn(self, *a, **kw)
        finally:
            self.lib.gdmcf_gemm_precision(prev)
    return wrapped


def _pl(a):
    if type(a) is tuple:
        return a
    return (None, 0) if a is None else (a.data_ptr(), a.stride(0))


def _f32_rows(t):
    return t if t.dtype == torch.float32 and t.stride(-1) == 1 else t.float().contiguous()


def _prep_modes(B, ca, noise, drop_mask, drop_p, training):
    noise_mode = 0
    if ca is not None:
        noise_mode = 1 if noise is not None else 2
        if noise is not None:
            noise = _f32_rows(noise)
    drop_mode, keep = 0, None
    if drop_mask is not None:
        drop_mode = 1
        keep = drop_mask.reshape(B, -1)
        keep = (keep if keep.dtype == torch.uint8 else (keep != 0).to(torch.uint8)).contiguous()
    elif training and drop_p > 0.0:
        drop_mode = 2
    return noise_mode, noise, drop_mode, keep


def prep_input(lib, x, I, ts, ca, cb, noise, drop_mask, drop_p, training, seed, offset, norm, emb, E, xin, xt_out, temb,
               rownorm, st):
    B = x.shape[0]
    x = _f32_rows(x)
    noise_mode, noise, drop_mode, keep = _prep_modes(B, ca, noise, drop_mask, drop_p, training)
    (nz, ldn), (kp, ldkp), (xi, ldx), (xo, ldxo) = _pl(noise), _pl(keep), _pl(xin), _pl(xt_out)
    _lib.check(lib.gdmcf_dnn_prep_input_f32(
        x.data_ptr(), x.stride(0), _lib.ptr(ts), _lib.ptr(ca), _lib.ptr(cb), noise_mode, nz, ldn, drop_mode, kp, ldkp, drop_p,
        seed, offset, int(bool(norm)), emb.weight.data_ptr() if emb is not None else None,
        emb.bias.data_ptr() if emb is not None else None, E, B, I, xi, ldx, xo, ldxo, _lib.ptr(temb), _lib.ptr(rownorm), st))
    return x, noise, keep


def prep_input_csr(lib, batch, ts, ca, cb, noise, drop_mask, drop_p, training, seed, offset, emb, E, xin, temb, x0bits, st):
    B, I = batch.shape
    noise_mode, noise, drop_mode, keep = _prep_modes(B, ca, noise, drop_mask, drop_p, training)
    (nz, ldn), (kp, ldkp) = _pl(noise), _pl(keep)
    c = batch.csr
    _lib.check(lib.gdmcf_dnn_prep_input_csr_f32(
        c.indptr.data_ptr(), c.indices.data_ptr(), batch.row_ids.data_ptr(), _lib.ptr(ts), _lib.ptr(ca), _lib.ptr(cb),
        noise_mode, nz, ldn, drop_mode, kp, ldkp, drop_p, seed, offset, emb.weight.data_ptr(), emb.bias.data_ptr(), E, B, I,
        xin.data_ptr(), xin.stride(0), temb.data_ptr(), x0bits.data_ptr(), x0bits.stride(0), st))
    return batch, noise, keep


def onehot_prep_input_csr(lib, batch, ts_U, discrete, sampled, seed, offset_noise, ts, drop_mask, drop_p, training,
                          offset_prep, emb, E, xin, temb, st, sampled_out=None, x0bits=None):
    B, I = batch.shape
    _, _, drop_mode, keep = _prep_modes(B, None, None, drop_mask, drop_p, training)
    (sp, lds), (kp, ldkp), (so, ldso), (xb, ldb) = _pl(sampled), _pl(keep), _pl(sampled_out), _pl(x0bits)
    c = batch.csr
    _lib.check(lib.gdmcf_onehot_prep_input_csr_f32(
        c.indptr.data_ptr(), c.indices.data_ptr(), batch.row_ids.data_ptr(), _lib.ptr(ts_U), float(discrete), sp, lds, seed,
        offset_noise, so, ldso, _lib.ptr(ts), drop_mode, kp, ldkp, drop_p, offset_prep,
        emb.weight.data_ptr() if emb is not None else None, emb.bias.data_ptr() if emb is not None else None, E, B, I,
        xin.data_ptr(), xin.stride(0), _lib.ptr(temb), xb, ldb, st))
    return batch, sampled, keep


def cat_prep_input_csr(lib, batch, ts_U, discrete, sampled, seed, offset_noise, ts, ca, cb, noise, drop_mask, drop_p, training,
                       offset_prep, cat, emb, E, xin, xt, temb, x0bits, clsbits, st):
    B, I = batch.shape
    noise_mode, noise, drop_mode, keep = _prep_modes(B, ca, noise, drop_mask, drop_p, training)
    (sp, lds), (nz, ldn), (kp, ldkp) = _pl(sampled), _pl(noise), _pl(keep)
    c = batch.csr
    _lib.check(lib.gdmcf_cat_prep_input_csr_f32(
        c.indptr.data_ptr(), c.indices.data_ptr(), batch.row_ids.data_ptr(), _lib.ptr(ts_U), float(discrete), sp, lds,
        offset_noise, ts.data_ptr(), _lib.ptr(ca), _lib.ptr(cb), noise_mode, nz, ldn, drop_mode, kp, ldkp, drop_p, seed,
        offset_prep, cat.weight.data_ptr(), cat.bias.data_ptr(), emb.weight.data_ptr(), emb.bias.data_ptr(), E, B, I,
        xin.data_ptr(), xin.stride(0), xt.data_ptr(), xt.stride(0), temb.data_ptr(), x0bits.data_ptr(), x0bits.stride(0),
        clsbits.data_ptr(), clsbits.stride(0), st))
    return batch, noise, keep, drop_mode


def cat_grad_bits(lib, dxin, xt, x0bits, clsbits, drop_mode, keep, drop_p, seed, offset, B, I, ws, ws_bytes, gw, gb, st):
    (kp, ldkp) = _pl(keep)
    _lib.check(lib.gdmcf_cat_grad_bits_f32(
        dxin.data_ptr(), dxin.stride(0), xt.data_ptr(), xt.stride(0), x0bits.data_ptr(), x0bits.stride(0), clsbits.data_ptr(),
        clsbits.stride(0), drop_mode, kp, ldkp, drop_p, seed, offset, B, I, ws.data_ptr(), ws_bytes, gw.data_ptr(), gb.data_ptr(),
        st))


def linear_fwd(lib, bufs, A, W, bias, act, B, N, K, out, st):
    (a, lda), (w, ldw), (o, ldo) = _pl(A), _pl(W), _pl(out)
    _lib.check(lib.gdmcf_linear_fwd_f32(a, lda, w, ldw, _lib.ptr(bias), act, B, N, K, o, ldo, bufs.ws.data_ptr(),
                                        bufs.ws_bytes, st))


def gather_fwd(lib, pre, base, batch, table, I, a, tblE, E, bias, act, B, N, out, st):
    (p, ldp), (tb, ldt), (ap, lda), (te, ldte), (o, ldo) = _pl(pre), _pl(table), _pl(a), _pl(tblE), _pl(out)
    c = batch.csr if batch is not None else None
    if c is None:
        tb, ldt = None, 0
    if E == 0:
        ap, lda, te, ldte = None, 0, None, 0
    _lib.check(lib.gdmcf_gather_fwd_f32(
        p, ldp, _lib.ptr(base), c.indptr.data_ptr() if c is not None else None, c.indices.data_ptr() if c is not None else None,
        batch.row_ids.data_ptr() if c is not None else None, tb, ldt, I, ap, lda, te, ldte, E, _lib.ptr(bias), act, B, N, o, ldo, st))


def latent_step(lib, A, M, v, p_cur, c1, c2, e, act, B, N, K, p_next, h_next, st):
    (a, lda), (m, ldm), (pc, ldpc), (pn, ldpn), (h, ldh) = _pl(A), _pl(M), _pl(p_cur), _pl(p_next), _pl(h_next)
    _lib.check(lib.gdmcf_latent_step_f32(a, lda, m, ldm, _lib.ptr(v), pc, ldpc, c1.data_ptr(), c2.data_ptr(), _lib.ptr(e), act,
                                         B, N, K, pn, ldpn, h, ldh, None, 0, st))


def latent_step_ex(lib, A, M, v, p_cur, c1, c2, r, e, act, B, N, K, p_next, h_next, acc, st):
    (a, lda), (m, ldm), (pc, ldpc), (pn, ldpn), (h, ldh), (rp, ldr) = _pl(A), _pl(M), _pl(p_cur), _pl(p_next), _pl(h_next), _pl(r)
    (qc, ldqc), (qn, ldqn) = (_pl(acc[0]), _pl(acc[3])) if acc is not None else ((None, 0), (None, 0))
    qa, qb = (acc[1].data_ptr(), acc[2].data_ptr()) if acc is not None else (None, None)
    _lib.check(lib.gdmcf_latent_step_ex_f32(a, lda, m, ldm, _lib.ptr(v), pc, ldpc, c1.data_ptr(), c2.data_ptr(), rp, ldr, _lib.ptr(e),
                                            act, B, N, K, pn, ldpn, h, ldh, qc, ldqc, qa, qb, qn, ldqn, None, 0, st))


def latent_acc(lib, q_cur, qa, A, qb, B, K, q_next, st):
    (qc, ldqc), (a, lda), (qn, ldqn) = _pl(q_cur), _pl(A), _pl(q_next)
    _lib.check(lib.gdmcf_latent_acc_f32(qc, ldqc, qa.data_ptr(), a, lda, qb.data_ptr(), B, K, qn, ldqn, st))


def cand_scores(lib, A, W, I, K, bias, scale, cand, ldcand, B, C, mask_ptrs, rows, out, st):
    (a, lda), (w, ldw), (o, ldo) = _pl(A), _pl(W), _pl(out)
    _lib.check(lib.gdmcf_cand_scores_f32(a, lda, w, ldw, I, K, _lib.ptr(bias), _lib.ptr(scale), cand.data_ptr(), ldcand, B, C,
                                         *mask_ptrs, _lib.ptr(rows), o, ldo, st))


def cand_pick(lib, dense, B, I, scale, cand, ldcand, C, mask_ptrs, rows, out, st):
    (d, ldd), (o, ldo) = _pl(dense), _pl(out)
    _lib.check(lib.gdmcf_cand_pick_f32(d, ldd, B, I, _lib.ptr(scale), cand.data_ptr(), ldcand, C, *mask_ptrs, _lib.ptr(rows), o,
                                       ldo, st))


def step_tables(tabs32, T, B, names, cache=None):
    key = (id(tabs32), int(T), int(B))
    rec = cache.get(names) if cache is not None else None
    if rec is None or rec[0] != key:
        rec = (key, {k: tabs32[k][:T, None].expand(T, B).contiguous() for k in names if k in tabs32})
        if cache is not None:
            cache[names] = rec
    return rec[1]


LatentProduct = collections.namedtuple("LatentProduct", "A second K bias scale")


class EpsTables:

    def __init__(self, c1, c2, r1, r2, T):
        import numpy as np
        c1, c2, r1, r2 = (np.asarray(t, dtype=np.float64)[:T] for t in (c1, c2, r1, r2))
        g, d = c1 * r1 + c2, c1 * r2
        G, D = 1.0, 0.0
        with np.errstate(all="ignore"):
            for t in range(T - 1, -1, -1):
                G, D = g[t] * G, g[t] * D + d[t]
            qa, qb = g.copy(), d.copy()
            qa[T - 1] = 0.0
            qa[0], qb[0] = qa[0] / D, qb[0] / D
        self.g, self.d, self.qa, self.qb = (t.astype(np.float32) for t in (g, d, qa, qb))
        self.G, self.D = float(np.float32(G)), float(np.float32(D))
        self.ok = bool(all(np.isfinite(t).all() for t in (self.g, self.d, self.qa, self.qb)) and np.isfinite(self.G)
                       and np.isfinite(self.D) and self.D > 0)
        self._dev = {}

    def on(self, device, B):
        rec, key = self._dev, (str(device), int(B))
        if key not in rec:
            def tab(a):
                return torch.from_numpy(a).to(device)[:, None].expand(len(a), B).contiguous()
            f = dict(dtype=torch.float32, device=device)
            rec[key] = dict(neg_d=tab(-self.d), g=tab(self.g), qa=tab(self.qa), qb=tab(self.qb), G=torch.full((B,), self.G, **f),
                            D=torch.full((B,), self.D, **f), one=torch.ones(B, **f), zero=torch.zeros(B, **f))
            rec[key]["qa0_neg"], rec[key]["qb0_neg"] = -rec[key]["qa"][0], -rec[key]["qb"][0]
        return rec[key]


def linear_bwd_input(lib, bufs, dz, W, rs, A_prev, act_prev, B, N, K, d_prev, st):
    (z, ldz), (w, ldw), (a, lda), (d, ldd) = _pl(dz), _pl(W), _pl(A_prev), _pl(d_prev)
    _lib.check(lib.gdmcf_linear_bwd_input_f32(z, ldz, w, ldw, _lib.ptr(rs), a, lda, act_prev, B, N, K, d, ldd,
                                              bufs.ws.data_ptr(), bufs.ws_bytes, st))


def linear_bwd_weight(lib, dz, A, rs, scol, B, N, K, dW, db, st):
    (z, ldz), (a, lda) = _pl(dz), _pl(A)
    _lib.check(lib.gdmcf_linear_bwd_weight_f32(z, ldz, a, lda, _lib.ptr(rs), scol, B, N, K, dW.data_ptr(), dW.stride(0),
                                               _lib.ptr(db), 0, st))


def adamw_args(fs, w):
    if fs["exp_avg"].stride() != w.stride() or fs["exp_avg_sq"].stride() != w.stride():
        raise RuntimeError("gdmcf_amd: the moments of a fused weight must share its leading dimension")
    return (fs["exp_avg"].data_ptr(), fs["exp_avg_sq"].data_ptr(), fs["lr"], fs["beta1"], fs["beta2"], fs["eps"],
            fs["weight_decay"], fs["step"], fs["grad_scale"])


def dw_adamw_args(dz, A, rs, scol, B, N, K, w, db, fs):
    (z, ldz), (a, lda) = _pl(dz), _pl(A)
    ad = adamw_args(fs, w)
    return (z, ldz, a, lda, _lib.ptr(rs), scol, B, N, K, w.data_ptr(), w.stride(0), ad[0], ad[1], _lib.ptr(db)) + ad[2:]


def linear_bwd_weight_adamw(lib, args, st):
    _lib.check(lib.gdmcf_linear_bwd_weight_adamw_f32(*args, st))


def rowscale(lib, A, rs, B, K, out, st):
    (a, lda), (o, ldo) = _pl(A), _pl(out)
    _lib.check(lib.gdmcf_rowscale_f32(a, lda, rs.data_ptr(), B, K, o, ldo, st))


def emb_bwd(lib, bufs, dz, W, I_cols, E, B, N, dWe, dbe, st):
    (z, ldz), (w, ldw) = _pl(dz), _pl(W)
    _lib.check(lib.gdmcf_emb_bwd_f32(z, ldz, w, ldw, I_cols, E, bufs.temb.data_ptr(), B, N, bufs.demb.data_ptr(),
                                     dWe.data_ptr(), dbe.data_ptr(), st))


def loss_layer(lib, bufs, A, W, bias, target, alpha, B, N, K, st, reduce=True):
    (a, lda), (w, ldw) = _pl(A), _pl(W)
    _lib.check(lib.gdmcf_linear_loss_fwd_f32(a, lda, w, ldw, _lib.ptr(bias), target.data_ptr(), target.stride(0),
                                             _lib.ptr(alpha), B, N, K, None, 0, bufs.diff.data_ptr(), bufs.ldi,
                                             bufs.rowpart.data_ptr(), bufs.rowsum.data_ptr() if reduce else None, st))
    return int(lib.gdmcf_loss_parts_last())


def loss_layer_bits(lib, bufs, A, W, bias, x0bits, alpha, B, N, K, st, reduce=True):
    (a, lda), (w, ldw) = _pl(A), _pl(W)
    _lib.check(lib.gdmcf_linear_loss_fwd_bits_f32(a, lda, w, ldw, _lib.ptr(bias), x0bits.data_ptr(), x0bits.stride(0),
                                                  _lib.ptr(alpha), B, N, K, None, 0, bufs.diff.data_ptr(), bufs.ldi,
                                                  bufs.rowpart.data_ptr(), bufs.rowsum.data_ptr() if reduce else None, st))
    return int(lib.gdmcf_loss_parts_last())


def loss_tail(lib, bufs, spec, B, rowdiv, alpha, st, mean=False):
    ts = spec["ts"]
    loss = torch.empty(B, dtype=torch.float64, device=ts.device)
    args = (bufs.rowsum.data_ptr(), rowdiv.data_ptr(), _lib.ptr(alpha), ts.data_ptr(), spec["weight_t"].data_ptr(),
            spec["pt"].data_ptr(), B, spec["T"], spec["H"], spec["Lt_history"].data_ptr(), spec["Lt_count"].data_ptr(),
            int(spec["update_history"]), bufs.lu.data_ptr(), loss.data_ptr(), bufs.gradcoef.data_ptr())
    if not mean:
        _lib.check(lib.gdmcf_row_loss_finish_f64(*args, st))
        return loss
    loss_mean = torch.empty((), dtype=torch.float64, device=ts.device)
    if getattr(bufs, "rowscale_mean", None) is None:
        bufs.rowscale_mean = torch.zeros(B, dtype=torch.float32, device=ts.device)
    _lib.check(lib.gdmcf_row_loss_finish_mean_f64(*args, loss_mean.data_ptr(), bufs.rowscale_mean.data_ptr(), st))
    return loss, loss_mean


def loss_tail_job(lib, bufs, spec, B, rowdiv, alpha, nt, A, K):
    ts = spec["ts"]
    loss = torch.empty(B, dtype=torch.float64, device=ts.device)
    loss_mean = torch.empty((), dtype=torch.float64, device=ts.device)
    if getattr(bufs, "rowscale_mean", None) is None:
        bufs.rowscale_mean = torch.zeros(B, dtype=torch.float32, device=ts.device)
    (a, lda) = _pl(A)
    job = _lib.GdKnTail(bufs.rowpart.data_ptr(), bufs.rowpart.stride(0), nt, bufs.rowsum.data_ptr(), rowdiv.data_ptr(),
                        _lib.ptr(alpha), ts.data_ptr(), spec["weight_t"].data_ptr(), spec["pt"].data_ptr(), spec["T"], spec["H"],
                        spec["Lt_history"].data_ptr(), spec["Lt_count"].data_ptr(), int(spec["update_history"]),
                        bufs.lu.data_ptr(), loss.data_ptr(), bufs.gradcoef.data_ptr(), loss_mean.data_ptr(),
                        bufs.rowscale_mean.data_ptr(), a, lda, bufs.rowscale_mean.data_ptr(), K, bufs.hs.data_ptr(),
                        bufs.hs.stride(0))
    job.refs = (loss, loss_mean, rowdiv, alpha, ts, spec["weight_t"], spec["pt"], spec["Lt_history"], spec["Lt_count"], A)
    return loss, loss_mean, job


def tail_job_run(lib, job, B, st):
    _lib.check(lib.gdmcf_kn_tail_run(ctypes.byref(job), B, st))


def linear_bwd_input_tail(lib, bufs, dz, W, rs, A_prev, act_prev, B, N, K, d_prev, job, st):
    (z, ldz), (w, ldw), (a, lda), (d, ldd) = _pl(dz), _pl(W), _pl(A_prev), _pl(d_prev)
    _lib.check(lib.gdmcf_linear_bwd_input_tail_f32(z, ldz, w, ldw, _lib.ptr(rs), a, lda, act_prev, B, N, K, d, ldd,
                                                   bufs.ws.data_ptr(), bufs.ws_bytes, ctypes.byref(job), st))


def posterior_fwd(lib, A, W, bias, x_t, c1, c2, r1, r2, sigma, z, B, N, K, x_next, pred, st):
    (a, lda), (w, ldw), (zp, ldz), (pp, ldp) = _pl(A), _pl(W), _pl(z), _pl(pred)
    _lib.check(lib.gdmcf_linear_posterior_fwd_f32(
        a, lda, w, ldw, _lib.ptr(bias), x_t.data_ptr(), x_t.stride(0), c1.data_ptr(), c2.data_ptr(), _lib.ptr(r1),
        _lib.ptr(r2), _lib.ptr(sigma), zp, ldz, B, N, K, x_next.data_ptr(), x_next.stride(0), pp, ldp, st))


class TrainLoss(torch.autograd.Function):

    @staticmethod
    def forward(ctx, eng, spec, *params):
        loss = eng.train_forward(spec)
        ctx.eng, ctx.version = eng, eng.version
        return loss

    @staticmethod
    def backward(ctx, gloss):
        eng = ctx.eng
        if ctx.version != eng.version:
            raise RuntimeError("gdmcf_amd: activations were overwritten by a later forward; "
                               "call backward before the next training_losses/forward")
        return (None, None, *eng.train_backward(gloss))


class EngineBase:
    supports_grad_sink = True

    def __init__(self, model):
        self.model = model
        self.lib = _lib.load()
        self.E = int(model.time_emb_dim)
        self.I = int(model.in_dims[0])
        self.version = 0
        self.seed = int(torch.initial_seed()) & 0xFFFFFFFFFFFFFFFF
        self.offset = 0
        self._bufs = {}
        self._saved = None
        self._wt = {}
        self._latent = None
        self.grad_sink = None
        self.fused_opt = None

    @property
    def gemm_dtype(self):
        return getattr(self.model, "gemm_dtype", "f32")

    def manual_seed(self, seed):
        self.seed = int(seed) & 0xFFFFFFFFFFFFFFFF
        self.offset = 0

    def _check_params(self, layers):
        what = type(self.model).__name__ + " parameters"
        for w, b, _ in layers:
            _lib.require_gpu(w, what)
            if not (w.stride(1) == 1 and w.stride(0) >= w.shape[1] and b.is_contiguous() and w.dtype == torch.float32):
                raise RuntimeError(f"gdmcf_amd: {what} must be float32 with unit column stride")

    def _transposed(self, w):
        rec = self._wt.get(id(w))
        if rec is None or rec[0] is not w or rec[1] != w._version or rec[2].device != w.device:
            n, k = w.shape
            buf = torch.zeros(k, (n + 31) // 32 * 32, dtype=torch.float32, device=w.device)
            buf[:, :n].copy_(w.detach().t())
            rec = self._wt[id(w)] = (w, w._version, buf)
        return rec[2]

    def _emb_table(self, w, bias, I_cols, T, st):
        m, lib, E, h, dev = self.model, self.lib, self.E, w.shape[0], w.device
        f32 = dict(dtype=torch.float32, device=dev)
        e = torch.zeros(T, _ceil64(h), **f32)
        if E == 0:
            e[:, :h].copy_(bias.detach()[None, :].expand(T, h))
            return e, None
        ew, eb = m.emb_layer.weight, m.emb_layer.bias
        xs = torch.zeros(T, _ceil64(4 + E), **f32)
        ts = torch.arange(T, dtype=torch.int64, device=dev)
        temb = torch.zeros(T, E, **f32)
        _lib.check(lib.gdmcf_dnn_emb_cols_f32(ts.data_ptr(), ew.data_ptr(), eb.data_ptr(), E, T, 4, xs.data_ptr(), xs.stride(0),
                                              temb.data_ptr(), st))
        we_t = torch.zeros(E, (h + 3) // 4 * 4, **f32)
        we_t[:, :h].copy_(w.detach()[:, I_cols:I_cols + E].t())
        gather_fwd(lib, None, None, None, None, I_cols, (xs.data_ptr() + 16, xs.stride(0)), we_t, E, bias, 0, T, h, e, st)
        return e, (xs, ts, temb, we_t)

    def _latent_operands(self, w1, bias1, second, K, b_out, T, entering, tables=()):
        lib, st = self.lib, _lib.stream_ptr()
        key = tuple((t.data_ptr(), t._version, str(t.device)) for t in entering) + (int(T), int(K), b_out is None)
        if self._latent is not None and self._latent[0] == key:
            return self._latent[1]
        h, I, dev = w1.shape[0], self.I, w1.device
        f32 = dict(dtype=torch.float32, device=dev)
        o, ws = _Bufs(), _Bufs()
        ws.ws_bytes = int(max(lib.gdmcf_linear_ws_bytes(h, I, K), lib.gdmcf_linear_ws_bytes(1, h, I)))
        ws.ws = torch.empty(max(ws.ws_bytes, 256), dtype=torch.uint8, device=dev)
        w1x = (w1.data_ptr(), w1.stride(0))
        o.M = torch.zeros(h, _ceil64(K), **f32)
        linear_bwd_input(lib, ws, w1x, second, None, None, 0, h, I, K, o.M, st)
        o.v = o.neg_b = None
        if b_out is not None:
            o.v = torch.zeros(h, **f32)
            linear_fwd(lib, ws, (b_out.data_ptr(), I), w1x, None, 0, 1, h, I, (o.v.data_ptr(), h), st)
            o.neg_b = -b_out.detach()
        ones = torch.ones(I, **f32)
        o.S = torch.zeros(h, **f32)
        linear_fwd(lib, ws, (ones.data_ptr(), I), w1x, None, 0, 1, h, I, (o.S.data_ptr(), h), st)
        o.keep_S = ones
        o.e, o.keep = self._emb_table(w1, bias1, I, T, st)
        o.tabs = [self._emb_table(w, b, cols, T, st) for w, b, cols in tables]
        self._latent = (key, o)
        return o

    def _latent_reverse(self, bufs, ops, T, B, K, act, pre, p, hpair, small, e, c1, c2, second, b_out, x_T, stop=False, eps=None,
                        r=None, c1_of=None, before_step=None):
        lib, st, I, dev, h = self.lib, _lib.stream_ptr(), self.I, p.device, ops.M.shape[0]
        s1, s2, Q = c1, c2, None
        if eps is not None:
            et = eps.on(dev, B)
            s1, s2, qa, qb = et["neg_d"], et["g"], et["qa"], et["qb"]
            if getattr(bufs, "lat_q", None) is None:
                bufs.lat_q = torch.zeros(B, _ceil64(K), dtype=torch.float32, device=dev)
            Q = bufs.lat_q
        if c1_of is not None:
            s1 = c1_of(s1)
        plain = r is None and Q is None
        hcur, hnxt = hpair
        gather_fwd(lib, pre, None, None, None, I, None, None, 0, e[T - 1], act, B, h, hcur, st)
        for n, i in enumerate(range(T - 1, -1, -1)):
            if before_step is not None:
                before_step(n, i)
            A = small(n, i, hcur) if small is not None else hcur
            if i == 0:
                break
            if plain:
                latent_step(lib, A, ops.M, ops.v, p, s1[i], s2[i], e[i - 1], act, B, h, K, p, hnxt, st)
            else:
                latent_step_ex(lib, A, ops.M, ops.v, p, s1[i], s2[i], r, e[i - 1], act, B, h, K, p, hnxt,
                               (Q, qa[i], qb[i], Q) if Q is not None else None, st)
            hcur, hnxt = hnxt, hcur
        if eps is not None:
            qa0, qb0 = (et["qa0_neg"], et["qb0_neg"]) if stop else (qa[0], qb[0])
            latent_acc(lib, Q, qa0, A, qb0, B, K, Q, st)
            if stop:
                return LatentProduct(Q, second, K, ops.neg_b, et["D"])
        elif stop:
            return LatentProduct(A, second, K, b_out, c1[0])
        x0 = torch.empty(B, I, dtype=torch.float32, device=dev)
        if eps is not None:
            posterior_fwd(lib, Q, second, b_out, x_T, et["one"], et["zero"], et["G"], et["D"], None, None, B, I, K, x0, None, st)
        else:
            posterior_fwd(lib, A, second, b_out, x_T, c1[0], c2[0], None, None, None, None, B, I, K, x0, None, st)
        return x0

    @with_precision
    def score_product(self, A, second, K, b_out, B, device):
        bufs = self.buffers(B, device)
        if getattr(bufs, "scores", None) is None:
            bufs.scores = torch.empty(B, self.I, dtype=torch.float32, device=device)
        self._grow_workspace(bufs, B, device, [(self.I, K)])
        linear_fwd(self.lib, bufs, A, second, b_out, 0, B, self.I, K, bufs.scores, _lib.stream_ptr())
        return bufs.scores

    def _gather_first_layer(self, bufs, batch, w, bias, act, xin, B, out, st):
        N, I, E = w.shape[0], self.I, self.E
        wt = self._transposed(w)
        emb_cols = (xin.data_ptr() + 4 * I, xin.stride(0))
        gather_fwd(self.lib, None, None, batch, wt, I, emb_cols, (wt.data_ptr() + 4 * I * wt.stride(0), wt.stride(0)), E, bias, act,
                   B, N, out, st)

    def _shared_buffers(self, b, B, device, n_loss, n_first, weights):
        lib, I, E = self.lib, self.I, self.E
        f32 = dict(dtype=torch.float32, device=device)
        b.temb = torch.zeros(B, max(E, 1), **f32)
        b.rownorm = torch.zeros(B, **f32)
        b.ldi = _ceil64(I)
        b.diff = torch.zeros(B, b.ldi, **f32)
        b.xt = None
        b.rowpart = torch.zeros(B, lib.gdmcf_loss_tiles(n_loss), **f32)
        b.rowsum = torch.zeros(B, **f32)
        b.gradcoef = torch.zeros(B, **f32)
        b.rowdiv_mse = torch.full((B,), float(I), **f32)
        b.lu = torch.zeros(B, dtype=torch.float64, device=device)
        b.demb = torch.zeros((B + n_first) * max(E, 1), **f32)
        b.ws_bytes = 0
        b.tab_cache = {}
        self._grow_workspace(b, B, device, [w.shape for w in weights])

    def _grow_workspace(self, b, B, device, shapes):
        ws = max([b.ws_bytes] + [self.lib.gdmcf_linear_ws_bytes(B, n, k) for n, k in shapes])
        if ws > b.ws_bytes or getattr(b, "ws", None) is None:
            b.ws_bytes = int(ws)
            b.ws = torch.empty(max(ws, 256), dtype=torch.uint8, device=device)

    def _prep_input(self, bufs, x, I, xin, ts, ca, cb, noise, drop_mask, training, xt_out=None):
        m = self.model
        self.offset += 1
        return prep_input(self.lib, x, I, ts, ca, cb, noise, drop_mask, float(m.drop.p), training, self.seed, self.offset,
                          m.norm, m.emb_layer, self.E, xin, xt_out, bufs.temb, bufs.rownorm, _lib.stream_ptr())

    def _eps_target(self, bufs, spec, ts, x0, noise):
        B, dev = ts.shape[0], ts.device
        x0 = _f32_rows(x0)
        target = noise if spec.get("noise_owned", False) else torch.empty(B, self.I, dtype=torch.float32, device=dev)
        alpha = torch.empty(B, dtype=torch.float32, device=dev)
        rowdiv = torch.empty(B, dtype=torch.float32, device=dev)
        _lib.check(self.lib.gdmcf_eps_target_f32(
            noise.data_ptr(), noise.stride(0), bufs.xt.data_ptr(), bufs.xt.stride(0), x0.data_ptr(), x0.stride(0), ts.data_ptr(),
            spec["r1_0"].data_ptr(), spec["r2_0"].data_ptr(), int(bool(spec.get("t0_likelihood", True))), B, self.I,
            target.data_ptr(), target.stride(0), alpha.data_ptr(), rowdiv.data_ptr(), _lib.stream_ptr()))
        return target, alpha, rowdiv

    def _rowscale_of(self, bufs, gloss):
        if isinstance(gloss, float):
            return bufs.gradcoef * gloss
        return (gloss.to(torch.float32) * bufs.gradcoef).contiguous()

    def _fused_state(self, w):
        fused = self.fused_opt if self.grad_sink is None else None
        return fused.fused_state(w) if fused is not None else None

    def _row_scaled(self, bufs, B, K, A, rs, scol, st):
        if rs is None:
            return A, scol
        rowscale(self.lib, A, rs, B, K, bufs.hs, st)
        return bufs.hs, int(bufs.hs.stride(0) > K)

    def _weight_grad(self, bufs, B, w, dz, rs, A, scol, dW, db, fs, st, queue=None):
        N, K = w.shape
        if fs is None:
            linear_bwd_weight(self.lib, dz, A, rs, scol, B, N, K, dW, db, st)
            return
        args = dw_adamw_args(dz, A, rs, scol, B, N, K, w, db, fs)
        if queue is not None:
            queue.append((_lib.GdDwAdamw(*args), w))
            return
        linear_bwd_weight_adamw(self.lib, args, st)
        if not (self.gemm_dtype == "bf16" and _lib.shadow_info(w.data_ptr()) is not None):
            torch.autograd.graph.increment_version(w)

    def _input_grad(self, bufs, B, W, N, K, dz, rs, A_prev, act_prev, d_prev, st):
        linear_bwd_input(self.lib, bufs, dz, W, rs, A_prev, act_prev, B, N, K, d_prev, st)
```

### include/gdmcf_hip.h

```cpp
#ifndef GDMCF_HIP_H
#define GDMCF_HIP_H
#include <stddef.h>
#include <stdint.h>

#ifdef __cplusplus
extern "C" {
#endif

#define GDMCF_OK 0
#define GDMCF_E_SHAPE (-1)
#define GDMCF_E_ARG (-2)
#define GDMCF_E_UNSUPPORTED (-3)
#define GDMCF_E_HIP (-4)
#define GDMCF_E_WORKSPACE (-5)

int gdmcf_version(void);
const char* gdmcf_last_error(void);
int gdmcf_device_info(int* n_cu, int* wave_size, char* arch_host, int arch_len);
int gdmcf_debug_last_gemm(void);
int gdmcf_debug_fat_slab_plan(int M, int N, int K, int* nb, int* splits, int* cps);
int gdmcf_debug_dr_tn_plan(int M, int N, int K, int64_t lddz, int64_t lda, int64_t ldw, int bias_col, int fused, int* depth,
                           int* ksp, int* tiles_m, int* tiles_n, int* m_fastest, int* has_bias);

int gdmcf_prof_enable(int on);
int gdmcf_prof_collect(int cap, int* tags_host, float* ms_host, double* work_host);

#define GDMCF_N_TABLES 13
int gdmcf_schedule_build(int kind, double noise_scale, double noise_min, double noise_max, int T,
                         int beta_fixed, double* out_tables_host);

int gdmcf_densify_rows_f32(const int64_t* indptr, const int32_t* indices, const float* values,
                           const int64_t* row_ids, int B, int I, float* out, int64_t ldo, void* stream);

int gdmcf_dnn_prep_input_f32(const float* x, int64_t ldx, const int64_t* ts, const float* ca,
                             const float* cb, int noise_mode, const float* noise, int64_t ldn,
                             int drop_mode, const uint8_t* keep, int64_t ldkeep, float drop_p,
                             uint64_t seed, uint64_t offset, int normalize, const float* emb_w,
                             const float* emb_b, int E, int B, int I, float* xin, int64_t ldxin,
                             float* xt_out, int64_t ldxt, float* temb_out, float* rownorm_ws,
                             void* stream);
int gdmcf_dnn_prep_input_csr_f32(const int64_t* indptr, const int32_t* indices, const int64_t* rows, const int64_t* ts,
                                 const float* ca, const float* cb, int noise_mode, const float* noise, int64_t ldn,
                                 int drop_mode, const uint8_t* keep, int64_t ldkeep, float drop_p, uint64_t seed,
                                 uint64_t offset, const float* emb_w, const float* emb_b, int E, int B, int I, float* xin,
                                 int64_t ldxin, float* temb_out, uint32_t* bits_out, int64_t ldbits, void* stream);

int gdmcf_onehot_noise_f32(const float* x0, int64_t ldx, const int64_t* ts, int B, int I, float discrete,
                           const uint8_t* sampled, int64_t lds, uint64_t seed, uint64_t offset,
                           float* xU, int64_t ldu, uint8_t* sampled_out, int64_t ldso, void* stream);
int gdmcf_onehot_prep_input_csr_f32(const int64_t* indptr, const int32_t* indices, const int64_t* rows, const int64_t* ts_U,
                                    float discrete, const uint8_t* sampled, int64_t lds, uint64_t seed, uint64_t offset_noise,
                                    uint8_t* sampled_out, int64_t ldso, const int64_t* ts, int drop_mode, const uint8_t* keep,
                                    int64_t ldkeep, float drop_p, uint64_t offset_prep, const float* emb_w, const float* emb_b,
                                    int E, int B, int I, float* xin, int64_t ldxin, float* temb_out, uint32_t* bits_out,
                                    int64_t ldbits, void* stream);

int gdmcf_randn_f32(float* out, int64_t ld, int rows, int cols, int stream_id, uint64_t seed, uint64_t offset, void* stream);

int gdmcf_eps_target_f32(const float* noise, int64_t ldn, const float* xt, int64_t ldxt, const float* x0, int64_t ldx0,
                         const int64_t* ts, const float* r1, const float* r2, int t0_likelihood, int B, int I, float* target,
                         int64_t ldt, float* alpha, float* rowdiv, void* stream);

int gdmcf_graph_guided_step_u8(uint8_t* graph, int64_t ldg, const int64_t* ts, int B, int I, float discrete,
                               const uint8_t* sampled_in, int64_t lds, const uint8_t* pick_in, const float* degree_prob,
                               int user_guided, uint64_t seed, uint64_t offset, uint8_t* sampled_out, int64_t ldso,
                               uint8_t* pick_out, void* stream);

int gdmcf_dnn_emb_cols_f32(const int64_t* ts, const float* emb_w, const float* emb_b, int E, int B,
                           int I, float* xin, int64_t ldxin, float* temb_out, void* stream);

enum { GDMCF_GEMM_F32 = 0, GDMCF_GEMM_BF16 = 1, GDMCF_GEMM_F32X3 = 2 };
int gdmcf_gemm_precision(int mode);
int gdmcf_bf16_shadow_set(const float* f32, void* bf16, int64_t rows, int64_t cols, int64_t ld_bf16);
int gdmcf_bf16_shadow_clear(const float* f32 );
void* gdmcf_bf16_shadow_get(const float* f32);
int gdmcf_bf16_shadow_info(const float* f32, void** bf16, int64_t* rows, int64_t* cols, int64_t* ld_bf16);
int gdmcf_bf16_shadow_sync(const float* f32, int64_t ld, void* stream);
size_t gdmcf_linear_ws_bytes(int M, int N, int K);
int gdmcf_linear_fwd_f32(const float* A, int64_t lda, const float* W, int64_t ldw,
                         const float* bias, int act, int M, int N, int K, float* C, int64_t ldc,
                         void* ws, size_t ws_bytes, void* stream);
int gdmcf_linear_fwd_wt_f32(const float* A, int64_t lda, const float* Wt, int64_t ldwt,
                            const float* bias, int act, int M, int N, int K, float* C, int64_t ldc,
                            void* ws, size_t ws_bytes, void* stream);
int gdmcf_gather_fwd_f32(const float* pre, int64_t ldpre, const float* base, const int64_t* indptr, const int32_t* indices,
                         const int64_t* rows, const float* table, int64_t ldt, int I, const float* a, int64_t lda,
                         const float* tblE, int64_t ldte, int E, const float* bias, int act, int B, int N, float* out, int64_t ldo,
                         void* stream);
int gdmcf_latent_step_f32(const float* A, int64_t lda, const float* M, int64_t ldm, const float* v,
                          const float* p_cur, int64_t ldpc, const float* c1, const float* c2, const float* e, int act,
                          int B, int N, int K, float* p_next, int64_t ldpn, float* h_next, int64_t ldh,
                          void* ws, size_t ws_bytes, void* stream);
size_t gdmcf_latent_step_ws_bytes(int B, int N, int K);
int gdmcf_latent_step_ex_f32(const float* A, int64_t lda, const float* M, int64_t ldm, const float* v,
                             const float* p_cur, int64_t ldpc, const float* c1, const float* c2, const float* r, int64_t ldr,
                             const float* e, int act, int B, int N, int K, float* p_next, int64_t ldpn, float* h_next,
                             int64_t ldh, const float* q_cur, int64_t ldqc, const float* qa, const float* qb, float* q_next,
                             int64_t ldqn, void* ws, size_t ws_bytes, void* stream);
int gdmcf_latent_acc_f32(const float* q_cur, int64_t ldqc, const float* qa, const float* A, int64_t lda, const float* qb,
                         int B, int K, float* q_next, int64_t ldqn, void* stream);
int gdmcf_loss_tiles(int N);
int gdmcf_linear_loss_fwd_f32(const float* A, int64_t lda, const float* W, int64_t ldw,
                              const float* bias, const float* target, int64_t ldt,
                              const float* alpha, int M, int N, int K, float* out, int64_t ldo,
                              float* diff, int64_t ldd, float* rowpart, float* rowsum,
                              void* stream);
int gdmcf_linear_loss_fwd_bits_f32(const float* A, int64_t lda, const float* W, int64_t ldw, const float* bias,
                                   const uint32_t* target_bits, int64_t ldbits, const float* alpha, int M, int N, int K,
                                   float* out, int64_t ldo, float* diff, int64_t ldd, float* rowpart, float* rowsum,
                                   void* stream);
int gdmcf_linear_posterior_fwd_f32(const float* A, int64_t lda, const float* W, int64_t ldw,
                                   const float* bias, const float* x_t, int64_t ldxt,
                                   const float* c1, const float* c2, const float* r1,
                                   const float* r2, const float* sigma, const float* z,
                                   int64_t ldz, int M, int N, int K, float* x_next,
                                   int64_t ldxn, float* pred_out, int64_t ldp, void* stream);
int gdmcf_linear_bwd_input_f32(const float* dZ, int64_t lddz, const float* W, int64_t ldw,
                               const float* rowscale, const float* Aact, int64_t ldact, int act,
                               int M, int N, int K, float* dA, int64_t ldda, void* ws,
                               size_t ws_bytes, void* stream);
typedef struct GdKnTail {
    const float* rowpart;
    int ld_rowpart, nt;
    float* rowsum;
    const float* rowdiv;
    const float* alpha;
    const int64_t* ts;
    const double* weight_t;
    const double* pt;
    int T, H;
    double* Lt_history;
    int64_t* Lt_count;
    int update_history;
    double* loss_unscaled;
    double* loss;
    float* gradcoef;
    double* loss_mean;
    float* rowscale_mean;
    const float* A;
    int64_t lda;
    const float* rowscale;
    int Ka;
    float* out;
    int64_t ldo;
} GdKnTail;
int gdmcf_linear_bwd_input_tail_f32(const float* dZ, int64_t lddz, const float* W, int64_t ldw, const float* rowscale,
                                    const float* Aact, int64_t ldact, int act, int M, int N, int K, float* dA, int64_t ldda,
                                    void* ws, size_t ws_bytes, const GdKnTail* tail, void* stream);
int gdmcf_kn_tail_run(const GdKnTail* tail, int M, void* stream);
int gdmcf_loss_parts_last(void);
int gdmcf_debug_kn_tail_rides(int M, int N, int K);
int gdmcf_linear_bwd_weight_f32(const float* dZ, int64_t lddz, const float* A, int64_t lda,
                                const float* rowscale, int a_scale_col, int M, int N, int K,
                                float* dW, int64_t lddw, float* db, int accumulate, void* stream);
int gdmcf_linear_bwd_weight_adamw_f32(const float* dZ, int64_t lddz, const float* A, int64_t lda,
                                      const float* rowscale, int a_scale_col, int M, int N, int K, float* W,
                                      int64_t ldw, float* exp_avg, float* exp_avg_sq, float* db, float lr,
                                      float beta1, float beta2, float eps, float weight_decay, int step,
                                      float grad_scale, void* stream);
typedef struct GdDwAdamw {
    const float* dZ;
    int64_t lddz;
    const float* A;
    int64_t lda;
    const float* rowscale;
    int a_scale_col, M, N, K;
    float* W;
    int64_t ldw;
    float* exp_avg;
    float* exp_avg_sq;
    float* db;
    float lr, beta1, beta2, eps, weight_decay;
    int step;
    float grad_scale;
} GdDwAdamw;
int gdmcf_linear_bwd_weight_adamw_multi_f32(const GdDwAdamw* list, int n, void* stream);
int gdmcf_rowscale_f32(const float* A, int64_t lda, const float* rowscale, int M, int K, float* out,
                       int64_t ldo, void* stream);
int gdmcf_row_norms_f32(const float* X, int64_t ld, int rows, int cols, float* norm, float* inv_norm,
                        void* stream);
int gdmcf_normalize_rows_bwd_f32(const float* dY, int64_t lddy, const float* Y, int64_t ldy,
                                 const float* inv_norm, int rows, int cols, float* dX, int64_t lddx,
                                 void* stream);
int gdmcf_tanh_bwd_f32(const float* dA, int64_t ldd, const float* A, int64_t lda, const float* extra,
                       int64_t lde, const float* scale, int M, int N, float* out, int64_t ldo,
                       void* stream);
int gdmcf_gather_rows_f32(const float* src, int64_t lds, const int64_t* index, int n, int cols, float* dst,
                          int64_t ldd, void* stream);
int gdmcf_scatter_add_rows_f32(const float* src, int64_t lds, const int64_t* index, int n, int cols,
                               float* dst, int64_t ldd, void* stream);
int gdmcf_normalize_rows_bwd_adamw_f32(const float* dY, int64_t lddy, const float* Y, int64_t ldy,
                                       const float* inv_norm, int rows, int cols, float* X, int64_t ldx,
                                       float* exp_avg, float* exp_avg_sq, float lr, float beta1, float beta2,
                                       float eps, float weight_decay, int step, float grad_scale, void* stream);
int gdmcf_scatter_rows_adamw_f32(const float* src, int64_t lds, const int64_t* index, int n, int rows, int cols,
                                 float* W, int64_t ldw, float* exp_avg, float* exp_avg_sq, float lr, float beta1,
                                 float beta2, float eps, float weight_decay, int step, float grad_scale,
                                 void* stream);
int gdmcf_emb_bwd_f32(const float* dZ1, int64_t lddz, const float* W1, int64_t ldw, int I, int E,
                      const float* temb, int M, int N, float* demb_ws, float* dWe, float* dbe,
                      void* stream);

int gdmcf_row_loss_finish_f64(const float* rowsum, const float* rowdiv, const float* alpha,
                              const int64_t* ts, const double* weight_t, const double* pt, int B,
                              int T, int H, double* Lt_history, int64_t* Lt_count,
                              int update_history, double* loss_unscaled, double* loss,
                              float* gradcoef, void* stream);
int gdmcf_row_loss_finish_mean_f64(const float* rowsum, const float* rowdiv, const float* alpha, const int64_t* ts,
                                   const double* weight_t, const double* pt, int B, int T, int H, double* Lt_history,
                                   int64_t* Lt_count, int update_history, double* loss_unscaled, double* loss,
                                   float* gradcoef, double* loss_mean, float* rowscale_mean, void* stream);
int gdmcf_lt_history_update(const int64_t* ts, const double* loss_unscaled, int B, int T, int H,
                            double* Lt_history, int64_t* Lt_count, void* stream);

int gdmcf_dp_pack_f64(const float* const* grads, const int64_t* counts, int n, const int64_t* ts,
                      const double* loss_unscaled, int B, int rank, int world, double* flat,
                      void* stream);
int gdmcf_dp_unpack_f64(const double* flat, float* const* grads, const int64_t* counts, int n, int B,
                        int world, int64_t* ts_all, double* loss_unscaled_all, void* stream);

int gdmcf_sample_timesteps(const double* Lt_history, const int64_t* Lt_count, int T, int H, int B,
                           double uniform_prob, uint64_t seed, uint64_t offset, int64_t* ts,
                           double* pt, double* p_out, void* stream);

int gdmcf_adamw_f32(const int64_t* table, int n_tensors, int total_blocks, float lr, float beta1,
                    float beta2, float eps, float weight_decay, int step, float grad_scale,
                    void* stream);
int gdmcf_adamw_bf16s_f32(const int64_t* table, const int64_t* shadow_table, int n_tensors, int total_blocks, float lr,
                          float beta1, float beta2, float eps, float weight_decay, int step, float grad_scale,
                          void* stream);

int gdmcf_topk_masked_f32(const float* pred, int64_t ldp, int B, int I, const int64_t* mask_indptr,
                          const int32_t* mask_indices, int k, int64_t* idx_out, float* val_out,
                          void* stream);
int gdmcf_topk_masked_rows_f32(const float* pred, int64_t ldp, int B, int I, const int64_t* indptr, const int32_t* indices,
                               const int64_t* indptr2, const int32_t* indices2, const int64_t* rows, const float* scale, int k,
                               int64_t* idx_out, float* val_out, void* stream);
int gdmcf_rank_targets_f32(const float* pred, int64_t ldp, int B, int I, const int64_t* indptr, const int32_t* indices,
                           const int64_t* indptr2, const int32_t* indices2, const int64_t* tgt_indptr, const int32_t* tgt_indices,
                           const int64_t* rows, int G, int32_t* rank_out, int64_t ldr, int32_t* n_live_out, void* stream);

int gdmcf_cand_scores_f32(const float* A, int64_t lda, const float* W, int64_t ldw, int I, int K, const float* bias,
                          const float* scale, const int64_t* cand, int64_t ldcand, int B, int C, const int64_t* indptr,
                          const int32_t* indices, const int64_t* indptr2, const int32_t* indices2, const int64_t* rows, float* out,
                          int64_t ldo, void* stream);
int gdmcf_cand_pick_f32(const float* dense, int64_t ldd, int B, int I, const float* scale, const int64_t* cand, int64_t ldcand,
                        int C, const int64_t* indptr, const int32_t* indices, const int64_t* indptr2, const int32_t* indices2,
                        const int64_t* rows, float* out, int64_t ldo, void* stream);

size_t gdmcf_score_topk_ws_bytes(int n_rows, int n_items, int d, int k);
int gdmcf_score_topk_f32(const float* user_emb, int64_t ldu, const int64_t* user_ids, int n_rows, const float* item_emb,
                         int64_t ldi, int n_items, int d, const int64_t* mask_indptr, const int32_t* mask_indices, int k,
                         int64_t* out_idx, float* out_val, void* ws, size_t ws_bytes, void* stream);

int gdmcf_debug_score_rank_plan(int n_rows, int n_items, int G, int* tile_rows, int* pass_targets, int* passes, int* slabs);
size_t gdmcf_score_rank_ws_bytes(int n_rows, int n_items, int d, int G);
int gdmcf_score_rank_f32(const float* user_emb, int64_t ldu, const int64_t* user_ids, int n_rows, const float* item_emb,
                         int64_t ldi, int n_items, int d, const int64_t* mask_indptr, const int32_t* mask_indices,
                         const int64_t* tgt_indptr, const int32_t* tgt_indices, int G, int32_t* rank_out, int64_t ldr,
                         int32_t* n_live_out, void* ws, size_t ws_bytes, void* stream);

int gdmcf_topn_metrics_f64(const int64_t* pred_idx, int64_t ldp, int U, const int64_t* gt_indptr, const int32_t* gt_indices,
                           const int* topN_host, int n_topn, double* out, void* stream);
int gdmcf_rank_metrics_f64(const int32_t* ranks, int64_t ldr, int U, int G, const int* topN_host, int n_topn, double* out,
                           void* stream);

int gdmcf_spmm_csr_f32(const int64_t* vbeg, const int64_t* vend, const int32_t* vrow, const int32_t* vslot,
                       int n_virtual, int n_short, const int32_t* lrow, const int32_t* lptr, int n_long, const int32_t* col,
                       const float* val, int n_rows, const float* X, int64_t ldx, int d, float* Y,
                       int64_t ldy, float* partial_ws, const float* const* addends_host, int n_add,
                       int64_t ld_add, float scale, double alg_bytes, void* stream);
int gdmcf_spmm_bundled_f32(const int32_t* wdesc, int n_waves, const int64_t* lbeg, const int32_t* llen, const int32_t* lrow,
                           const int32_t* lslot, int n_pieces, const int64_t* sbeg, const int32_t* slen, const int32_t* srow,
                           const int32_t* smax, int n_bundles, const int32_t* crow, const int32_t* cptr, int n_cut,
                           const int32_t* col, const float* val, int64_t nnz, int n_rows, int n_x_rows, const float* X,
                           int64_t ldx, int d, float* Y, int64_t ldy, float* partial_ws, const float* const* addends_host, int n_add, int64_t ld_add,
                           float scale, double alg_bytes, void* stream);
int gdmcf_spmm_stream_f32(const int32_t* wdesc, int n_waves, const int32_t* cw, int64_t n_entries, const int32_t* ud, int n_units,
                          const int32_t* crow, const int32_t* cptr, int n_cut, int n_rows, int n_x_rows, const float* X,
                          int64_t ldx, int d, float* Y, int64_t ldy, float* partial_ws, const float* const* addends_host,
                          int n_add, int64_t ld_add, float scale, double alg_bytes, void* stream);
int gdmcf_debug_spmm_stamps(int n_waves, long long* host_out);
int gdmcf_graph_state_bytes(void);
int gdmcf_adam_hyper_bytes(void);
int gdmcf_graph_state_init(void* state_host, uint64_t prep_offset, uint64_t ts_offset, int64_t adam_step, int64_t table_first,
                           int64_t table_len, const void* hyper_table_dev);
int gdmcf_adam_hyper_fill(void* out_host, int n, float lr, float beta1, float beta2, float eps, float weight_decay,
                          int64_t first_step, float grad_scale);
int gdmcf_graph_state_bind(const void* state_dev);
int gdmcf_graph_state_tick(void* state_dev, void* stream);
int gdmcf_scale_f32(const float* acc, int64_t n, float scale, float* out, void* stream);

int gdmcf_bpr_sample_f32(const int64_t* indptr, const int32_t* indices, const int64_t* users, int B, int n_users, int n_items,
                         uint64_t seed, uint64_t offset, int64_t* pos, int64_t* neg, int32_t* flag, void* stream);
int gdmcf_bpr_sample_pool_f32(const int64_t* indptr, const int32_t* indices, const int64_t* users, int B, int n_negs, int pool,
                              int n_users, int n_items, const float* M, int64_t ldm, int d, uint64_t seed, uint64_t offset,
                              int64_t* pos, int64_t* neg, int32_t* flag, void* stream);
int gdmcf_bpr_loss_f32(const float* M, int64_t ldm, const float* E0, int64_t lde, int d, const int64_t* users, const int64_t* pos,
                       const int64_t* neg, int B, int n_users, int n_items, float* coef, float* ws, float* mf, float* reg,
                       int32_t* flag, void* stream);
int gdmcf_bpr_grad_f32(int mode, const int32_t* order, const int64_t* users, const int64_t* pos, const int64_t* neg, int B,
                       int n_users, int n_items, const float* coef, const float* src, int64_t ld_src, int d, float* out,
                       int64_t ld_out, float scale, float* zero_rows, int64_t ld_zero, void* stream);

int gdmcf_cat_prep_input_f32(const float* x, int64_t ldx, const float* xU, int64_t ldu, const int64_t* ts, const float* ca,
                             const float* cb, int noise_mode, const float* noise, int64_t ldn, int drop_mode, const uint8_t* keep,
                             int64_t ldkeep, float drop_p, uint64_t seed, uint64_t offset, const float* cat_w, const float* cat_b,
                             const float* emb_w, const float* emb_b, int E, int B, int I, float* xin, int64_t ldxin, float* xt_out,
                             int64_t ldxt, float* temb_out, void* stream);
size_t gdmcf_cat_grad_ws_bytes(int B, int I);
int gdmcf_cat_grad_f32(const float* dxin, int64_t lddx, const float* xt, int64_t ldxt, const float* xU, int64_t ldu, int drop_mode,
                       const uint8_t* keep, int64_t ldkeep, float drop_p, uint64_t seed, uint64_t offset, int B, int I, void* ws,
                       size_t ws_bytes, float* grad_w, float* grad_b, void* stream);
int gdmcf_cat_prep_input_csr_f32(const int64_t* indptr, const int32_t* indices, const int64_t* rows, const int64_t* ts_U,
                                 float discrete, const uint8_t* sampled, int64_t lds, uint64_t offset_noise, const int64_t* ts,
                                 const float* ca, const float* cb, int noise_mode, const float* noise, int64_t ldn, int drop_mode,
                                 const uint8_t* keep, int64_t ldkeep, float drop_p, uint64_t seed, uint64_t offset_prep,
                                 const float* cat_w, const float* cat_b, const float* emb_w, const float* emb_b, int E, int B, int I,
                                 float* xin, int64_t ldxin, float* xt_out, int64_t ldxt, float* temb_out, uint32_t* x0bits_out,
                                 int64_t ldx0bits, uint32_t* clsbits_out, int64_t ldclsbits, void* stream);
int gdmcf_cat_grad_bits_f32(const float* dxin, int64_t lddx, const float* xt, int64_t ldxt, const uint32_t* x0bits, int64_t ldx0bits,
                            const uint32_t* clsbits, int64_t ldclsbits, int drop_mode, const uint8_t* keep, int64_t ldkeep,
                            float drop_p, uint64_t seed, uint64_t offset, int B, int I, void* ws, size_t ws_bytes, float* grad_w,
                            float* grad_b, void* stream);

size_t gdmcf_ntxent_ws_bytes(int B);
int gdmcf_ntxent_fwd_f32(const float* z1, int64_t ld1, const float* z2, int64_t ld2, int B, int d, float temperature, float eps,
                         void* ws, size_t ws_bytes, float* loss_out, void* stream);
int gdmcf_ntxent_bwd_f32(const float* z1, int64_t ld1, const float* z2, int64_t ld2, int B, int d, const void* ws, size_t ws_bytes,
                         const float* scale, float* dz1, int64_t lddz1, float* dz2, int64_t lddz2, void* stream);

#ifdef __cplusplus
}
#endif
#endif
```

Baseline: 324,700 users/s.

## Fold time-embedding backward into layer-1 input-gradient GEMM and split-K reduce

The time-embedding backward is moved into the layer-1 input-gradient path. Gathering the embedding columns of W1 now runs on an idle workgroup of the register-streaming GEMM, and the demb row products are folded into the split-K reduce kernel through an LDS row buffer. This is meant to remove the separate embedding-backward launches and the extra read of dA. The cost is more complex job dispatch, a templated reduce kernel, and an error path if the GEMM declines a product it had accepted.

```diff
diff --git a/gdmcf_amd/_lib.py b/gdmcf_amd/_lib.py
--- a/gdmcf_amd/_lib.py
+++ b/gdmcf_amd/_lib.py
@@ -100,6 +100,10 @@
     _fields_ = parse_structs(_HEADER)["GdKnTail"]
 
 
+class GdEmbBwd(ctypes.Structure):
+    _fields_ = parse_structs(_HEADER)["GdEmbBwd"]
+
+
 _lib = None
 
 
diff --git a/gdmcf_amd/csrc/gemm_dr_kn.hip b/gdmcf_amd/csrc/gemm_dr_kn.hip
--- a/gdmcf_amd/csrc/gemm_dr_kn.hip
+++ b/gdmcf_amd/csrc/gemm_dr_kn.hip
@@ -26,6 +26,10 @@
     if (job.on && slot == (ntasks + 3) >> 2) {
         extern __shared__ __attribute__((aligned(16))) unsigned char kn_lds[];
         gd_tail_job_run(job, kn_lds);
+        return;
+    }
+    if (job.emb_W1 && slot == ((ntasks + 3) >> 2) + (job.on ? 1 : 0)) {
+        gd_emb_gather_w_cols<8>(job.emb_W1, job.emb_ldw, job.emb_I, job.emb_E, job.emb_N1, job.emb_W1e, 0, 1);
         return;
     }
     const __amdgpu_buffer_rsrc_t srdA = __builtin_amdgcn_make_buffer_rsrc(const_cast<float*>(g.A), 0, (int)(((int64_t)(g.M - 1) * g.lda + g.K) * 4), 0x00020000);
@@ -148,14 +152,36 @@
 #define GD_KN_TAIL_DEFAULT 1
 #endif
 
-static int kn_launch(GdGemm& g, const GdTailJob* job, hipStream_t s) {
-    if (!dr_routes().kn) return GD_DR_NOT_TAKEN;
+bool gd_dr_kn_tail_switch() {
+    const char* env = getenv("GDMCF_KN_TAIL");
+    return env ? atoi(env) != 0 : GD_KN_TAIL_DEFAULT != 0;
+}
+
+static int kn_taken_splits(const GdGemm& g) {
+    if (!dr_routes().kn) return 0;
     const int splits = gd_dr_kn_splits(g.M, g.N, g.K);
     const size_t need = (size_t)splits * g.M * g.ldc * sizeof(float);
     const bool ok = splits > 0 && g.ldc >= g.N && (g.ldc & 3) == 0 && g.ws_cap >= need && g.slab_stride >= (int64_t)g.M * g.ldc &&
                 (int64_t)g.M * g.lda * 4 < ((int64_t)1 << 31) && (int64_t)g.K * g.ldb * 4 < ((int64_t)1 << 31) && g.lda >= g.K && g.ldb >= g.N &&
                 (reinterpret_cast<uintptr_t>(g.B) & 15) == 0 && (g.ldb & 3) == 0 && (reinterpret_cast<uintptr_t>(g.C) & 15) == 0;
-    if (!ok) return GD_DR_NOT_TAKEN;
+    return ok ? splits : 0;
+}
+
+static int kn_idle_count(int M, int N, int K, int splits) {
+    const int total_chunks = gd_cdiv(K, 16);
+    const int cps = (gd_cdiv(total_chunks, splits) + 1) & ~1;
+    const int idle = dr_cu_count() - gd_cdiv(gd_cdiv(M, 80) * gd_cdiv(N, 128) * gd_cdiv(total_chunks, cps), 4);
+    return idle > 0 ? idle : 0;
+}
+
+int gd_dr_kn_idle_workgroups(const GdGemm& g) {
+    const int splits = kn_taken_splits(g);
+    return splits > 0 ? kn_idle_count(g.M, g.N, g.K, splits) : -1;
+}
+
+static int kn_launch(GdGemm& g, const GdTailJob* job, hipStream_t s) {
+    const int splits = kn_taken_splits(g);
+    if (splits <= 0) return GD_DR_NOT_TAKEN;
     DrArgs d = {};
     const int n_cu = dr_cu_count();
     const int total_chunks = gd_cdiv(g.K, 16);
@@ -167,11 +193,12 @@
     GdTailJob none = {};
     size_t lds = 0;
     if (job) {
-        const char* env = getenv("GDMCF_KN_TAIL");
-        const bool tail_on = env ? atoi(env) != 0 : GD_KN_TAIL_DEFAULT != 0;
+        const int idle = n_cu - gd_cdiv(d.tiles_m * d.tiles_n * real_splits, 4);
+        if (idle < (job->on ? 1 : 0) + (job->emb_W1 ? 1 : 0)) return GD_DR_NOT_TAKEN;
+    }
+    if (job && job->on) {
         lds = lt_lds_bytes(job->T, job->H, job->B);
-        if (!tail_on || !job->on || !kn_idle_workgroup(d.tiles_m * d.tiles_n * real_splits, n_cu) || lds > GD_LT_LDS_MAX)
-            return GD_DR_NOT_TAKEN;
+        if (!gd_dr_kn_tail_switch() || lds > GD_LT_LDS_MAX) return GD_DR_NOT_TAKEN;
         static bool attr_set = false;
         if (!gd_allow_big_lds(dr_kn_kernel<2>, lds, &attr_set, "gemm_dr_kn")) return GDMCF_E_HIP;
     }
@@ -189,7 +216,13 @@
 }
 
 int gd_dr_kn_launch(GdGemm& g, hipStream_t s) { return kn_launch(g, nullptr, s); }
-int gd_dr_kn_launch_tail(GdGemm& g, const GdTailJob& job, hipStream_t s) { return kn_launch(g, &job, s); }
+int gd_dr_kn_launch_tail(GdGemm& g, const GdTailJob& job, hipStream_t s) { return job.on ? kn_launch(g, &job, s) : GD_DR_NOT_TAKEN; }
+int gd_dr_kn_launch_jobs(GdGemm& g, const GdTailJob& job, hipStream_t s) { return kn_launch(g, &job, s); }
+
+int gdmcf_debug_kn_idle_workgroups(int M, int N, int K) {
+    const int splits = gd_dr_kn_splits(M, N, K);
+    return splits > 0 ? kn_idle_count(M, N, K, splits) : 0;
+}
 
 int gdmcf_debug_kn_tail_rides(int M, int N, int K) {
     const int splits = gd_dr_kn_splits(M, N, K);
diff --git a/gdmcf_amd/csrc/linear.hip b/gdmcf_amd/csrc/linear.hip
--- a/gdmcf_amd/csrc/linear.hip
+++ b/gdmcf_amd/csrc/linear.hip
@@ -3,9 +3,6 @@
 #include "common.h"
 #include "tail_job.h"
 
-int gd_splitk_reduce(const float* slabs, int64_t slab_stride, int splits, int64_t ld_slab, int M, int N, int mode,
-                     const float* bias, const float* rowscale, const float* aact, int64_t ldact, int act, float* out,
-                     int64_t ldo, hipStream_t s);
 int gd_colsum(const float* dZ, int64_t ld, const float* rs, int M, int N, float* db, hipStream_t s);
 int gd_rowpart_reduce(const float* rowpart, int ld, int M, int nt, float* rowsum, hipStream_t s);
 
@@ -310,26 +307,7 @@
 
 int gdmcf_loss_parts_last(void) { return t_loss_parts; }
 
-int gdmcf_kn_tail_run(const GdKnTail* tail, int M, void* stream) {
-    GD_CHECK_ARG(tail != nullptr, "kn_tail_run: tail missing");
-    const GdKnTail& t = *tail;
-    GD_CHECK_SHAPE(M > 0 && t.nt > 0 && t.ld_rowpart >= t.nt, "kn_tail_run: bad shape");
-    GD_CHECK_ARG(t.rowpart && t.rowsum, "kn_tail_run: null pointer");
-    int rc = gd_rowpart_reduce(t.rowpart, t.ld_rowpart, M, t.nt, t.rowsum, (hipStream_t)stream);
-    if (rc) return rc;
-    rc = gdmcf_row_loss_finish_mean_f64(t.rowsum, t.rowdiv, t.alpha, t.ts, t.weight_t, t.pt, M, t.T, t.H, t.Lt_history, t.Lt_count,
-                                        t.update_history, t.loss_unscaled, t.loss, t.gradcoef, t.loss_mean, t.rowscale_mean, stream);
-    if (rc) return rc;
-    return gdmcf_rowscale_f32(t.A, t.lda, t.rowscale, M, t.Ka, t.out, t.ldo, stream);
-}
-
-int gdmcf_linear_bwd_input_tail_f32(const float* dZ, int64_t lddz, const float* W, int64_t ldw, const float* rowscale,
-                                    const float* Aact, int64_t ldact, int act, int M, int N, int K, float* dA, int64_t ldda,
-                                    void* ws, size_t ws_bytes, const GdKnTail* tail, void* stream) {
-    GD_CHECK_SHAPE(M > 0 && N > 0 && K > 0 && lddz >= N && ldw >= K && ldda >= K, "linear_bwd_input_tail: bad shape");
-    GD_CHECK_ARG(act == 0 || (act == 1 && Aact && ldact >= K), "linear_bwd_input_tail: activation output missing");
-    GD_CHECK_ARG(tail != nullptr, "linear_bwd_input_tail: tail missing");
-    const GdKnTail& t = *tail;
+static int kn_tail_check(const GdKnTail& t, int M) {
     GD_CHECK_SHAPE(t.nt > 0 && t.ld_rowpart >= t.nt && t.T > 0 && t.H > 0 && t.Ka > 0 && t.lda >= t.Ka && t.ldo >= t.Ka,
                    "linear_bwd_input_tail: bad tail shape");
     GD_CHECK_ARG(t.rowpart && t.rowsum && t.rowdiv && t.ts && t.weight_t && t.pt && t.loss_unscaled && t.loss && t.A && t.rowscale && t.out,
@@ -337,23 +315,58 @@
     GD_CHECK_ARG(!t.update_history || (t.Lt_history && t.Lt_count), "linear_bwd_input_tail: update_history without the history");
     GD_CHECK_ARG(!t.rowscale_mean || t.gradcoef, "linear_bwd_input_tail: rowscale_mean needs gradcoef");
     GD_CHECK_ARG(lt_lds_bytes(t.T, t.H, M) <= GD_LT_LDS_MAX, "linear_bwd_input_tail: T*H and B too large for the LDS-resident FIFO update (150 KiB)");
+    return GDMCF_OK;
+}
+
+static GdTailJob kn_tail_job(const GdKnTail& t, int M) {
+    GdShadow sh;
+    const bool has16 = gd_shadow_lookup(t.out, &sh) && sh.rows == M && sh.cols == t.Ka;
+    GdTailJob j = {};
+    j.on = 1; j.B = M;
+    j.rowpart = t.rowpart; j.ld_rowpart = t.ld_rowpart; j.nt = t.nt; j.rowsum = t.rowsum;
+    j.rowdiv = t.rowdiv; j.alpha = t.alpha; j.gradcoef = t.gradcoef; j.ts = t.ts; j.weight_t = t.weight_t; j.pt = t.pt;
+    j.T = t.T; j.H = t.H; j.update = t.update_history; j.hist = t.Lt_history; j.cnt = t.Lt_count; j.lu = t.loss_unscaled;
+    j.loss = t.loss; j.loss_mean = t.loss_mean; j.rowscale_mean = t.rowscale_mean; j.inv_b = 1.0f / (float)M;
+    j.K = t.Ka; j.A = t.A; j.lda = t.lda; j.rs = t.rowscale; j.out = t.out; j.ldo = t.ldo;
+    j.out16 = has16 ? (unsigned short*)sh.p16 : nullptr; j.ldo16 = has16 ? sh.ld16 : 0; j.bias_col = t.ldo > t.Ka;
+    return j;
+}
+
+static GdGemm kn_slab_product(const float* dZ, int64_t lddz, const float* W, int64_t ldw, int M, int N, int K, void* ws, size_t ws_bytes) {
+    const int64_t lds_ = round4(K);
+    GdGemm g = {};
+    g.A = dZ; g.lda = lddz; g.B = W; g.ldb = ldw; g.M = M; g.N = K; g.K = N;
+    g.C = (float*)ws; g.ldc = lds_; g.slab_stride = (int64_t)M * lds_; g.prof_tag = 4;
+    g.ws_cap = ws_bytes;
+    return g;
+}
+
+int gdmcf_kn_tail_run(const GdKnTail* tail, int M, void* stream) {
+    GD_CHECK_ARG(tail != nullptr, "kn_tail_run: tail missing");
+    const GdKnTail& t = *tail;
+    GD_CHECK_SHAPE(M > 0 && t.nt > 0 && t.ld_rowpart >= t.nt, "kn_tail_run: bad shape");
+    GD_CHECK_ARG(t.rowpart && t.rowsum, "kn_tail_run: null pointer");
+    int rc = gd_rowpart_reduce(t.rowpart, t.ld_rowpart, M, t.nt, t.rowsum, (hipStream_t)stream);
+    if (rc) return rc;
+    rc = gdmcf_row_loss_finish_mean_f64(t.rowsum, t.rowdiv, t.alpha, t.ts, t.weight_t, t.pt, M, t.T, t.H, t.Lt_history, t.Lt_count,
+                                        t.update_history, t.loss_unscaled, t.loss, t.gradcoef, t.loss_mean, t.rowscale_mean, stream);
+    if (rc) return rc;
+    return gdmcf_rowscale_f32(t.A, t.lda, t.rowscale, M, t.Ka, t.out, t.ldo, stream);
+}
+
+int gdmcf_linear_bwd_input_tail_f32(const float* dZ, int64_t lddz, const float* W, int64_t ldw, const float* rowscale,
+                                    const float* Aact, int64_t ldact, int act, int M, int N, int K, float* dA, int64_t ldda,
+                                    void* ws, size_t ws_bytes, const GdKnTail* tail, void* stream) {
+    GD_CHECK_SHAPE(M > 0 && N > 0 && K > 0 && lddz >= N && ldw >= K && ldda >= K, "linear_bwd_input_tail: bad shape");
+    GD_CHECK_ARG(act == 0 || (act == 1 && Aact && ldact >= K), "linear_bwd_input_tail: activation output missing");
+    GD_CHECK_ARG(tail != nullptr, "linear_bwd_input_tail: tail missing");
+    int rc0 = kn_tail_check(*tail, M);
+    if (rc0) return rc0;
     hipStream_t s = (hipStream_t)stream;
     const int64_t lds_ = round4(K);
     if (t_gemm_prec == GDMCF_GEMM_F32 && ws != nullptr) {
-        GdGemm g = {};
-        g.A = dZ; g.lda = lddz; g.B = W; g.ldb = ldw; g.M = M; g.N = K; g.K = N;
-        g.C = (float*)ws; g.ldc = lds_; g.slab_stride = (int64_t)M * lds_; g.prof_tag = 4;
-        g.ws_cap = ws_bytes;
-        GdShadow sh;
-        const bool has16 = gd_shadow_lookup(t.out, &sh) && sh.rows == M && sh.cols == t.Ka;
-        GdTailJob j = {};
-        j.on = 1; j.B = M;
-        j.rowpart = t.rowpart; j.ld_rowpart = t.ld_rowpart; j.nt = t.nt; j.rowsum = t.rowsum;
-        j.rowdiv = t.rowdiv; j.alpha = t.alpha; j.gradcoef = t.gradcoef; j.ts = t.ts; j.weight_t = t.weight_t; j.pt = t.pt;
-        j.T = t.T; j.H = t.H; j.update = t.update_history; j.hist = t.Lt_history; j.cnt = t.Lt_count; j.lu = t.loss_unscaled;
-        j.loss = t.loss; j.loss_mean = t.loss_mean; j.rowscale_mean = t.rowscale_mean; j.inv_b = 1.0f / (float)M;
-        j.K = t.Ka; j.A = t.A; j.lda = t.lda; j.rs = t.rowscale; j.out = t.out; j.ldo = t.ldo;
-        j.out16 = has16 ? (unsigned short*)sh.p16 : nullptr; j.ldo16 = has16 ? sh.ld16 : 0; j.bias_col = t.ldo > t.Ka;
+        GdGemm g = kn_slab_product(dZ, lddz, W, ldw, M, N, K, ws, ws_bytes);
+        const GdTailJob j = kn_tail_job(*tail, M);
         const int rc = gd_dr_kn_launch_tail(g, j, s);
         if (rc != GD_DR_NOT_TAKEN) {
             if (rc) return rc;
@@ -364,6 +377,64 @@
     const int rc = gdmcf_kn_tail_run(tail, M, stream);
     if (rc) return rc;
     return gdmcf_linear_bwd_input_f32(dZ, lddz, W, ldw, rowscale, Aact, ldact, act, M, N, K, dA, ldda, ws, ws_bytes, stream);
+}
+
+int gdmcf_linear_bwd_input_jobs_f32(const float* dZ, int64_t lddz, const float* W, int64_t ldw, const float* rowscale,
+                                    const float* Aact, int64_t ldact, int act, int M, int N, int K, float* dA, int64_t ldda,
+                                    void* ws, size_t ws_bytes, const GdKnTail* tail, const GdEmbBwd* emb, void* stream) {
+    GD_CHECK_SHAPE(M > 0 && N > 0 && K > 0 && lddz >= N && ldw >= K && ldda >= K, "linear_bwd_input_jobs: bad shape");
+    GD_CHECK_ARG(act == 0 || (act == 1 && Aact && ldact >= K), "linear_bwd_input_jobs: activation output missing");
+    if (tail) {
+        const int rc = kn_tail_check(*tail, M);
+        if (rc) return rc;
+    }
+    if (emb) {
+        GD_CHECK_SHAPE(emb->E > 0 && emb->I >= 0 && emb->ldw >= emb->I + emb->E && emb->N1 == K, "linear_bwd_input_jobs: bad embedding shape");
+        GD_CHECK_ARG(emb->W1 && emb->temb && emb->demb_ws && emb->dWe && emb->dbe, "linear_bwd_input_jobs: null pointer");
+    }
+    hipStream_t s = (hipStream_t)stream;
+    const char* env = getenv("GDMCF_EMB_RIDE");
+    const int ride = env ? atoi(env) : 1;
+    if (ride != 0 && t_gemm_prec == GDMCF_GEMM_F32 && ws != nullptr) {
+        GdGemm g = kn_slab_product(dZ, lddz, W, ldw, M, N, K, ws, ws_bytes);
+        int idle = gd_dr_kn_idle_workgroups(g);
+        if (idle >= 0) {
+            GdTailJob j = {};
+            if (tail && idle > 0 && gd_dr_kn_tail_switch()) {
+                j = kn_tail_job(*tail, M);
+                --idle;
+            } else if (tail) {
+                const int rc = gdmcf_kn_tail_run(tail, M, stream);
+                if (rc) return rc;
+            }
+            float* W1e = emb ? emb->demb_ws + (size_t)M * emb->E : nullptr;
+            if (emb && (ride & 1) && idle > 0) {
+                j.emb_W1 = emb->W1; j.emb_ldw = emb->ldw; j.emb_I = emb->I; j.emb_E = emb->E; j.emb_N1 = emb->N1; j.emb_W1e = W1e;
+            } else if (emb) {
+                const int rc = gd_emb_gather_w(emb->W1, emb->ldw, emb->I, emb->E, emb->N1, W1e, s);
+                if (rc) return rc;
+            }
+            int rc = gd_dr_kn_launch_jobs(g, j, s);
+            if (rc == GD_DR_NOT_TAKEN) {
+                gdmcf_set_error("linear_bwd_input_jobs: the register-streaming kernel declined a product it had accepted");
+                return GDMCF_E_UNSUPPORTED;
+            }
+            if (rc) return rc;
+            const bool fold = emb && (ride & 2) && K <= GD_REDUCE_DEMB_MAX_N;
+            rc = gd_splitk_reduce((const float*)ws, g.slab_stride, gd_cdiv(N, g.kchunk), round4(K), M, K, 1, nullptr, rowscale, Aact, ldact,
+                                  act, dA, ldda, s, fold ? W1e : nullptr, fold ? emb->E : 0, fold ? emb->demb_ws : nullptr);
+            if (rc || !emb) return rc;
+            if (!fold) {
+                rc = gd_emb_bwd_demb(dA, ldda, W1e, emb->E, K, M, emb->demb_ws, s);
+                if (rc) return rc;
+            }
+            return gd_emb_bwd_w(emb->demb_ws, emb->temb, M, emb->E, emb->dWe, emb->dbe, s);
+        }
+    }
+    const int rc = tail ? gdmcf_linear_bwd_input_tail_f32(dZ, lddz, W, ldw, rowscale, Aact, ldact, act, M, N, K, dA, ldda, ws, ws_bytes, tail, stream)
+                        : gdmcf_linear_bwd_input_f32(dZ, lddz, W, ldw, rowscale, Aact, ldact, act, M, N, K, dA, ldda, ws, ws_bytes, stream);
+    if (rc || !emb) return rc;
+    return gdmcf_emb_bwd_f32(dA, ldda, emb->W1, emb->ldw, emb->I, emb->E, emb->temb, M, emb->N1, emb->demb_ws, emb->dWe, emb->dbe, stream);
 }
 
 int gdmcf_linear_bwd_weight_f32(const float* dZ, int64_t lddz, const float* A, int64_t lda, const float* rowscale,
diff --git a/gdmcf_amd/csrc/reduce.hip b/gdmcf_amd/csrc/reduce.hip
--- a/gdmcf_amd/csrc/reduce.hip
+++ b/gdmcf_amd/csrc/reduce.hip
@@ -2,16 +2,24 @@
 
 namespace {
 
+template <bool DEMB>
 __global__ __launch_bounds__(256) void splitk_reduce_kernel(const float* __restrict__ slabs, int64_t slab_stride,
                                                             int splits, int64_t ld_slab, int M, int N, int mode,
                                                             const float* __restrict__ bias,
                                                             const float* __restrict__ rowscale,
                                                             const float* __restrict__ aact, int64_t ldact, int act,
                                                             float* __restrict__ out, int64_t ldo,
-                                                            unsigned short* __restrict__ out16, int64_t ldo16, int vec) {
+                                                            unsigned short* __restrict__ out16, int64_t ldo16, int vec,
+                                                            const float* __restrict__ W1e, int E, float* __restrict__ demb) {
     const int m = blockIdx.y;
     const int n0 = (blockIdx.x * 256 + threadIdx.x) * 4;
-    if (n0 >= N) return;
+    float* row = nullptr;
+    if constexpr (DEMB) {
+        __shared__ float row_lds[GD_REDUCE_DEMB_MAX_N];
+        row = row_lds;
+    }
+    if (!DEMB && n0 >= N) return;
+    if (!DEMB || n0 < N) {
     float sv[4] = {0.f, 0.f, 0.f, 0.f};
     const float* p = slabs + (int64_t)m * ld_slab + n0;
     if (vec && n0 + 3 < N) {
@@ -48,6 +56,12 @@
         }
         out[(int64_t)m * ldo + n] = s;
         if (out16) out16[(int64_t)m * ldo16 + n] = gd_bf16_bits(s);
+        if constexpr (DEMB) row[n] = s;
+    }
+    }
+    if constexpr (DEMB) {
+        __syncthreads();
+        gd_emb_demb_row(row, W1e, E, N, demb + (int64_t)m * E);
     }
 }
 
@@ -131,13 +145,23 @@
 
 int gd_splitk_reduce(const float* slabs, int64_t slab_stride, int splits, int64_t ld_slab, int M, int N, int mode,
                      const float* bias, const float* rowscale, const float* aact, int64_t ldact, int act, float* out,
-                     int64_t ldo, hipStream_t s) {
+                     int64_t ldo, hipStream_t s, const float* W1e, int E, float* demb) {
     GdShadow sh;
     const bool has16 = gd_shadow_lookup(out, &sh) && sh.rows == M && sh.cols == N;
     const int vec = (ld_slab % 4 == 0) && (slab_stride % 4 == 0) && gd_aligned16(slabs);
-    hipLaunchKernelGGL(splitk_reduce_kernel, dim3(gd_cdiv(N, 1024), M), dim3(256), 0, s, slabs, slab_stride,
+    if (demb) {
+        if (!W1e || E <= 0 || mode != 1 || N > GD_REDUCE_DEMB_MAX_N) {
+            gdmcf_set_error("splitk_reduce: demb needs W1e, E > 0, mode 1 and N <= %d", GD_REDUCE_DEMB_MAX_N);
+            return GDMCF_E_ARG;
+        }
+        hipLaunchKernelGGL(splitk_reduce_kernel<true>, dim3(1, M), dim3(256), 0, s, slabs, slab_stride, splits, ld_slab, M, N, mode, bias,
+                           rowscale, aact, ldact, act, out, ldo, has16 ? (unsigned short*)sh.p16 : nullptr, has16 ? sh.ld16 : 0, vec,
+                           W1e, E, demb);
+        return gd_launch_status("splitk_reduce_demb");
+    }
+    hipLaunchKernelGGL(splitk_reduce_kernel<false>, dim3(gd_cdiv(N, 1024), M), dim3(256), 0, s, slabs, slab_stride,
                        splits, ld_slab, M, N, mode, bias, rowscale, aact, ldact, act, out, ldo,
-                       has16 ? (unsigned short*)sh.p16 : nullptr, has16 ? sh.ld16 : 0, vec);
+                       has16 ? (unsigned short*)sh.p16 : nullptr, has16 ? sh.ld16 : 0, vec, (const float*)nullptr, 0, (float*)nullptr);
     return gd_launch_status("splitk_reduce");
 }
 
diff --git a/gdmcf_amd/csrc/rows.hip b/gdmcf_amd/csrc/rows.hip
--- a/gdmcf_amd/csrc/rows.hip
+++ b/gdmcf_amd/csrc/rows.hip
@@ -1,4 +1,4 @@
-#include "common.h"
+#include "tail_job.h"
 
 namespace {
 
@@ -182,21 +182,14 @@
 
 __global__ __launch_bounds__(256) void emb_gather_w_kernel(const float* __restrict__ W1, int64_t ldw, int I, int E, int N,
                                                            float* __restrict__ W1e) {
-    const int idx = blockIdx.x * 256 + threadIdx.x;
-    if (idx < N * E) W1e[idx] = W1[(int64_t)(idx / E) * ldw + I + (idx % E)];
+    gd_emb_gather_w_cols<1>(W1, ldw, I, E, N, W1e, blockIdx.x, gridDim.x);
 }
 
 __global__ __launch_bounds__(256) void emb_bwd_demb_kernel(const float* __restrict__ dZ1, int64_t lddz,
                                                            const float* __restrict__ W1e, int E, int N,
                                                            float* __restrict__ demb) {
     const int m = blockIdx.x;
-    const int lane = threadIdx.x & 63, wave = threadIdx.x >> 6;
-    for (int e = wave; e < E; e += 4) {
-        float s = 0.f;
-        for (int n = lane; n < N; n += 64) s += dZ1[(int64_t)m * lddz + n] * W1e[(int64_t)n * E + e];
-        for (int o = 32; o > 0; o >>= 1) s += __shfl_xor(s, o);
-        if (lane == 0) demb[(int64_t)m * E + e] = s;
-    }
+    gd_emb_demb_row(dZ1 + (int64_t)m * lddz, W1e, E, N, demb + (int64_t)m * E);
 }
 
 __global__ __launch_bounds__(64) void emb_bwd_w_kernel(const float* __restrict__ demb, const float* __restrict__ temb,
@@ -326,9 +319,9 @@
     GD_CHECK_ARG(dZ1 && W1 && temb && demb_ws && dWe && dbe, "emb_bwd: null pointer");
     hipStream_t s = (hipStream_t)stream;
     float* W1e = demb_ws + (size_t)M * E;
-    hipLaunchKernelGGL(emb_gather_w_kernel, dim3(gd_cdiv(N * E, 256)), dim3(256), 0, s, W1, ldw, I, E, N, W1e);
-    hipLaunchKernelGGL(emb_bwd_demb_kernel, dim3(M), dim3(256), 0, s, dZ1, lddz, W1e, E, N, demb_ws);
-    hipLaunchKernelGGL(emb_bwd_w_kernel, dim3(E * E + E), dim3(64), 0, s, demb_ws, temb, M, E, dWe, dbe);
+    gd_emb_gather_w(W1, ldw, I, E, N, W1e, s);
+    gd_emb_bwd_demb(dZ1, lddz, W1e, E, N, M, demb_ws, s);
+    gd_emb_bwd_w(demb_ws, temb, M, E, dWe, dbe, s);
     return gd_launch_status("emb_bwd");
 }
 
@@ -350,3 +343,18 @@
 }
 
 }
+
+int gd_emb_gather_w(const float* W1, int64_t ldw, int I, int E, int N, float* W1e, hipStream_t s) {
+    hipLaunchKernelGGL(emb_gather_w_kernel, dim3(gd_cdiv(N * E, 256)), dim3(256), 0, s, W1, ldw, I, E, N, W1e);
+    return gd_launch_status("emb_gather_w");
+}
+
+int gd_emb_bwd_demb(const float* dZ1, int64_t lddz, const float* W1e, int E, int N, int M, float* demb, hipStream_t s) {
+    hipLaunchKernelGGL(emb_bwd_demb_kernel, dim3(M), dim3(256), 0, s, dZ1, lddz, W1e, E, N, demb);
+    return gd_launch_status("emb_bwd_demb");
+}
+
+int gd_emb_bwd_w(const float* demb, const float* temb, int M, int E, float* dWe, float* dbe, hipStream_t s) {
+    hipLaunchKernelGGL(emb_bwd_w_kernel, dim3(E * E + E), dim3(64), 0, s, demb, temb, M, E, dWe, dbe);
+    return gd_launch_status("emb_bwd_w");
+}
diff --git a/gdmcf_amd/csrc/tail_job.h b/gdmcf_amd/csrc/tail_job.h
--- a/gdmcf_amd/csrc/tail_job.h
+++ b/gdmcf_amd/csrc/tail_job.h
@@ -63,6 +63,65 @@
                         if (k + j < K) out16[(int64_t)m * ldo16 + k + j] = gd_bf16_bits(v[j]);
             }
         }
+    }
+}
+
+template <int U>
+__device__ __forceinline__ void gd_emb_gather_w_cols(const float* __restrict__ W1, int64_t ldw, int I, int E, int N,
+                                                     float* __restrict__ W1e, int blk, int nblk) {
+    const int total = N * E, step = nblk * 256;
+    for (int i0 = blk * 256 + (int)threadIdx.x; i0 < total; i0 += step * U) {
+        float v[U];
+#pragma unroll
+        for (int u = 0; u < U; ++u) {
+            const int idx = min(i0 + u * step, total - 1);
+            v[u] = W1[(int64_t)(idx / E) * ldw + I + (idx % E)];
+        }
+#pragma unroll
+        for (int u = 0; u < U; ++u)
+            if (i0 + u * step < total) W1e[i0 + u * step] = v[u];
+    }
+}
+
+template <int NU>
+__device__ __forceinline__ void gd_emb_demb_row_some(const float* row, const float* __restrict__ W1e, int E, int N, int e0,
+                                                     float* __restrict__ demb_row) {
+    const int lane = threadIdx.x & 63;
+    float s[NU];
+#pragma unroll
+    for (int u = 0; u < NU; ++u) s[u] = 0.f;
+    for (int n0 = lane; n0 < N; n0 += 256) {
+        float x[4], w[4][NU];
+#pragma unroll
+        for (int v = 0; v < 4; ++v) {
+            const int n = min(n0 + 64 * v, N - 1);
+            x[v] = row[n];
+#pragma unroll
+            for (int u = 0; u < NU; ++u) w[v][u] = W1e[(int64_t)n * E + e0 + 4 * u];
+        }
+#pragma unroll
+        for (int v = 0; v < 4; ++v) {
+            if (n0 + 64 * v >= N) break;
+#pragma unroll
+            for (int u = 0; u < NU; ++u) s[u] = __builtin_fmaf(x[v], w[v][u], s[u]);
+        }
+    }
+#pragma unroll
+    for (int u = 0; u < NU; ++u) {
+        for (int o = 32; o > 0; o >>= 1) s[u] += __shfl_xor(s[u], o);
+        if (lane == 0) demb_row[e0 + 4 * u] = s[u];
+    }
+}
+
+__device__ __forceinline__ void gd_emb_demb_row(const float* row, const float* __restrict__ W1e, int E, int N,
+                                                float* __restrict__ demb_row) {
+    const int wave = __builtin_amdgcn_readfirstlane(threadIdx.x >> 6);
+    for (int e0 = wave; e0 < E; e0 += 16) {
+        const int nu = (E - e0 + 3) >> 2;
+        if (nu >= 4) gd_emb_demb_row_some<4>(row, W1e, E, N, e0, demb_row);
+        else if (nu == 3) gd_emb_demb_row_some<3>(row, W1e, E, N, e0, demb_row);
+        else if (nu == 2) gd_emb_demb_row_some<2>(row, W1e, E, N, e0, demb_row);
+        else gd_emb_demb_row_some<1>(row, W1e, E, N, e0, demb_row);
     }
 }
 
@@ -161,6 +220,10 @@
     unsigned short* out16;
     int64_t ldo16;
     int bias_col;
+    const float* emb_W1;
+    int64_t emb_ldw;
+    int emb_I, emb_E, emb_N1;
+    float* emb_W1e;
 };
 
 namespace {
@@ -188,3 +251,14 @@
 }
 
 int gd_dr_kn_launch_tail(GdGemm& g, const GdTailJob& job, hipStream_t s);
+int gd_dr_kn_launch_jobs(GdGemm& g, const GdTailJob& job, hipStream_t s);
+int gd_dr_kn_idle_workgroups(const GdGemm& g);
+bool gd_dr_kn_tail_switch();
+
+constexpr int GD_REDUCE_DEMB_MAX_N = 1024;
+int gd_splitk_reduce(const float* slabs, int64_t slab_stride, int splits, int64_t ld_slab, int M, int N, int mode,
+                     const float* bias, const float* rowscale, const float* aact, int64_t ldact, int act, float* out,
+                     int64_t ldo, hipStream_t s, const float* W1e = nullptr, int E = 0, float* demb = nullptr);
+int gd_emb_gather_w(const float* W1, int64_t ldw, int I, int E, int N, float* W1e, hipStream_t s);
+int gd_emb_bwd_demb(const float* dZ1, int64_t lddz, const float* W1e, int E, int N, int M, float* demb, hipStream_t s);
+int gd_emb_bwd_w(const float* demb, const float* temb, int M, int E, float* dWe, float* dbe, hipStream_t s);
diff --git a/gdmcf_amd/engine.py b/gdmcf_amd/engine.py
--- a/gdmcf_amd/engine.py
+++ b/gdmcf_amd/engine.py
@@ -267,16 +267,25 @@
         dz, rs = dz_last, rowscale
         dw_queue = [] if (fused is not None and self.gemm_dtype == "f32" and os.environ.get("GDMCF_DW_MULTI", "1") != "0") else None
 
+        emb_rides = type(self) is DenoiserEngine and self.gemm_dtype == "f32" and self.grad_sink is None and L >= 2
+
         def input_grad(li, w, A_prev):
             nonlocal dWe, dbe
             N, K = w.shape
             if li > 0:
                 dprev = bufs.dzs[li - 1]
-                if tail is not None and li == L - 1:
+                if li == 1 and emb_rides:
+                    dWe = self._grad_like(m.emb_layer.weight)
+                    dbe = self._grad_like(m.emb_layer.bias)
+                    core.linear_bwd_input_jobs(lib, bufs, dz, w, rs, A_prev, layers[0][2], B, N, K, dprev,
+                                               tail if li == L - 1 else None, layers[0][0], self.I, self.E, dWe, dbe, st)
+                elif tail is not None and li == L - 1:
                     core.linear_bwd_input_tail(lib, bufs, dz, w, rs, A_prev, layers[li - 1][2], B, N, K, dprev, tail, st)
                 else:
                     self._input_grad(bufs, B, w, N, K, dz, rs, A_prev, layers[li - 1][2], dprev, st)
                 return dprev
+            if emb_rides:
+                return None
             dWe = self._grad_like(m.emb_layer.weight)
             dbe = self._grad_like(m.emb_layer.bias)
             core.emb_bwd(lib, bufs, dz, w, self.I, self.E, B, N, dWe, dbe, st)
diff --git a/gdmcf_amd/engine_core.py b/gdmcf_amd/engine_core.py
--- a/gdmcf_amd/engine_core.py
+++ b/gdmcf_amd/engine_core.py
@@ -307,6 +307,14 @@
     (z, ldz), (w, ldw), (a, lda), (d, ldd) = _pl(dz), _pl(W), _pl(A_prev), _pl(d_prev)
     _lib.check(lib.gdmcf_linear_bwd_input_tail_f32(z, ldz, w, ldw, _lib.ptr(rs), a, lda, act_prev, B, N, K, d, ldd,
                                                    bufs.ws.data_ptr(), bufs.ws_bytes, ctypes.byref(job), st))
+
+
+def linear_bwd_input_jobs(lib, bufs, dz, W, rs, A_prev, act_prev, B, N, K, d_prev, job, W1, I_cols, E, dWe, dbe, st):
+    (z, ldz), (w, ldw), (a, lda), (d, ldd), (w1, ldw1) = _pl(dz), _pl(W), _pl(A_prev), _pl(d_prev), _pl(W1)
+    emb = _lib.GdEmbBwd(w1, ldw1, I_cols, E, K, bufs.temb.data_ptr(), bufs.demb.data_ptr(), dWe.data_ptr(), dbe.data_ptr())
+    _lib.check(lib.gdmcf_linear_bwd_input_jobs_f32(z, ldz, w, ldw, _lib.ptr(rs), a, lda, act_prev, B, N, K, d, ldd,
+                                                   bufs.ws.data_ptr(), bufs.ws_bytes, None if job is None else ctypes.byref(job),
+                                                   ctypes.byref(emb), st))
 
 
 def posterior_fwd(lib, A, W, bias, x_t, c1, c2, r1, r2, sigma, z, B, N, K, x_next, pred, st):
diff --git a/include/gdmcf_hip.h b/include/gdmcf_hip.h
--- a/include/gdmcf_hip.h
+++ b/include/gdmcf_hip.h
@@ -150,6 +150,19 @@
 int gdmcf_kn_tail_run(const GdKnTail* tail, int M, void* stream);
 int gdmcf_loss_parts_last(void);
 int gdmcf_debug_kn_tail_rides(int M, int N, int K);
+typedef struct GdEmbBwd {
+    const float* W1;
+    int64_t ldw;
+    int I, E, N1;
+    const float* temb;
+    float* demb_ws;
+    float* dWe;
+    float* dbe;
+} GdEmbBwd;
+int gdmcf_linear_bwd_input_jobs_f32(const float* dZ, int64_t lddz, const float* W, int64_t ldw, const float* rowscale,
+                                    const float* Aact, int64_t ldact, int act, int M, int N, int K, float* dA, int64_t ldda,
+                                    void* ws, size_t ws_bytes, const GdKnTail* tail, const GdEmbBwd* emb, void* stream);
+int gdmcf_debug_kn_idle_workgroups(int M, int N, int K);
 int gdmcf_linear_bwd_weight_f32(const float* dZ, int64_t lddz, const float* A, int64_t lda,
                                 const float* rowscale, int a_scale_col, int M, int N, int K,
                                 float* dW, int64_t lddw, float* db, int accumulate, void* stream);
```

New measurement: 325,400 users/s (median of 4 runs). About the same (+0.2%).
